# WestlyPark/StyleRenderer

Measured on AMD Instinct MI355X. Metric: generator fwd+bwd images/sec at 256^2, higher is better.
Workload: dtype f32

## Files before the change

### include/stylerenderer_amd.h

```cpp
#ifndef STYLERENDERER_AMD_H_
#define STYLERENDERER_AMD_H_

#include <stddef.h>
#include <stdint.h>

#ifdef __cplusplus
extern "C" {
#endif

typedef void* sr_stream_t;

#define SR_OK 0
#define SR_EINVAL (-1)
#define SR_ERANGE (-2)

const char* sr_error_string(int code);
int sr_abi_version(void);

int sr_fused_bias_act(float* y, const float* x, const float* b, const float* ref, int act, int grad,
                      float alpha, float scale, int64_t size_x, int64_t step_b, int64_t size_b,
                      int use_bias, int use_ref, sr_stream_t stream);

int64_t sr_fused_act_bwd_scratch_floats(int64_t n, int64_t c, int64_t inner);
int sr_fused_act_bwd(float* gx, float* gb, const float* gy, const float* out, float alpha,
                     float scale, int64_t n, int64_t c, int64_t inner, float* partial,
                     sr_stream_t stream);

int sr_noise_bias_act(float* y, const float* x, const float* noise, const float* noise_w,
                      const float* bias, const float* ref, float alpha, float scale, int64_t n,
                      int64_t c, int64_t inner, int64_t noise_bstride, sr_stream_t stream);
int64_t sr_noise_bias_act_bwd_scratch_floats(int64_t n, int64_t c, int64_t inner);
int sr_noise_bias_act_bwd(float* gx, float* gbias, float* gnoise_w, const float* gy, const float* out,
                          const float* noise, float alpha, float scale, int64_t n, int64_t c,
                          int64_t inner, int64_t noise_bstride, float* scratch, sr_stream_t stream);
int64_t sr_noise_bias_act_bwd_dot_scratch_floats(int64_t n, int64_t c, int64_t inner);
int sr_noise_bias_act_bwd_dot(float* gx, float* gbias, float* gnoise_w, float* rowdot, const float* gy,
                              const float* out, const float* noise, const float* noise_w, const float* bias,
                              float alpha, float scale, int64_t n, int64_t c, int64_t inner,
                              int64_t noise_bstride, float* scratch, sr_stream_t stream);
int sr_noise_bias_act_affine(float* y, const float* x, const float* amap, const float* smap, int64_t map_bstride,
                             const float* noise, const float* noise_w, const float* bias, float alpha,
                             float scale, int64_t n, int64_t c, int64_t inner, int64_t noise_bstride,
                             sr_stream_t stream);
int64_t sr_noise_bias_act_affine_bwd_scratch_floats(int64_t n, int64_t c, int64_t inner);
int sr_noise_bias_act_affine_bwd(float* gx, float* gamap, float* gsmap, float* gbias, float* gnoise_w,
                                 const float* gy, const float* out, const float* x, const float* amap,
                                 int64_t map_bstride, const float* noise, float alpha, float scale, int64_t n,
                                 int64_t c, int64_t inner, int64_t noise_bstride, float* scratch,
                                 sr_stream_t stream);
int64_t sr_noise_bias_act_affine_bwd2_scratch_floats(int64_t n, int64_t c, int64_t inner);
int sr_noise_bias_act_affine_bwd2(float* d_gy, float* d_x, float* d_amap, int64_t d_amap_bstride, const float* Gx,
                                  const float* Gmap, int64_t gmap_bstride, const float* Gb, const float* Gnw,
                                  const float* gy, const float* out, const float* x, const float* amap,
                                  int64_t map_bstride, const float* noise, float alpha, float scale, int64_t n,
                                  int64_t c, int64_t inner, int64_t noise_bstride, float* scratch, sr_stream_t stream);

int sr_adam_flat(float* p, const float* g, float* m, float* v, int64_t n, float lr, float beta1, float beta2,
                 float eps, const float* step, sr_stream_t stream);
int sr_adam_flat_guarded(float* p, const float* g, float* m, float* v, int64_t n, float lr, float beta1, float beta2,
                         float eps, float* step, const int64_t* guard_offs, int n_guards,
                         int32_t* skipped_host, sr_stream_t stream);

int64_t sr_rowdot_scratch_floats(int64_t rows, int64_t inner);
int sr_rowdot(float* dots, float* out_scaled, const float* a, const float* b, const float* scale,
              int64_t rows, int64_t inner, float* scratch, sr_stream_t stream);
int sr_rowdot_div(float* dots, const float* a, const float* b, const float* rdiv, int64_t rows, int64_t inner,
                  float* scratch, sr_stream_t stream);
int sr_rowdot_bwd(float* ga, float* gb, float* gs, const float* a, const float* b, const float* gd, const float* go,
                  const float* scale, int64_t rows, int64_t inner, float* scratch, sr_stream_t stream);

int sr_smallconv_fwd(float* out, const float* x, const float* ws, const float* bias, int64_t B, int64_t C,
                     int64_t N, int64_t hw, sr_stream_t stream);
int sr_smallconv_dx(float* dx, const float* g, const float* ws, int64_t B, int64_t C, int64_t N, int64_t hw,
                    sr_stream_t stream);
int sr_smallconv_dx_add(float* dx, const float* g, const float* ws, const float* addend, int64_t B, int64_t C, int64_t N,
                        int64_t hw, sr_stream_t stream);
int64_t sr_smallconv_dw_scratch_floats(int64_t B, int64_t C, int64_t N, int64_t hw);
int sr_smallconv_dw(float* dws, const float* g, const float* x, int64_t B, int64_t C, int64_t N, int64_t hw,
                    float* scratch, sr_stream_t stream);
int sr_smallconv_dw_bias(float* dws, float* gb, const float* g, const float* x, int64_t B, int64_t C, int64_t N, int64_t hw,
                         float* scratch, sr_stream_t stream);
int sr_modrows_fwd(float* ws, const float* w, const float* s, float scale, int64_t B, int64_t N, int64_t C,
                   sr_stream_t stream);
int sr_modrows_bwd(float* gs, float* gw, const float* dws, const float* w, const float* s, float scale, int64_t B,
                   int64_t N, int64_t C, sr_stream_t stream);

int sr_vertex_normals_f32(float* vn, float* norm_out, const float* v, const int64_t* tri, const int32_t* adj_off,
                          const int32_t* adj, int64_t B, int64_t nv, int64_t nf, float eps, sr_stream_t stream);

int sr_affine3_fwd(float* out, const float* v, const float* m, const float* t, int64_t B, int64_t nv,
                   int64_t v_bstride, sr_stream_t stream);
int sr_affine3_bwd(float* gm, float* gt, const float* v, const float* g, int64_t B, int64_t nv, int64_t v_bstride,
                   sr_stream_t stream);

int sr_morph_fwd(float* v, float* vs, float* reg, const float* w, const float* bias, const float* coeff, const float* lin,
                 const float* pose, const float* sigma, float lam, int64_t B, int64_t nv, int64_t d, sr_stream_t stream);
int sr_vertex_normals_bwd_f32(float* gvs, const float* gv, const float* gn, const float* lin, const float* rot,
                              const float* v, const float* ns, const float* normc, const int64_t* tri,
                              const int32_t* adj_off, const int32_t* adj, int64_t B, int64_t nv, int64_t nf, float eps,
                              sr_stream_t stream);
int64_t sr_morph_gcoeff_scratch_floats(int64_t rows, int64_t B, int64_t d);
int sr_morph_gcoeff(float* gcoeff, float* scratch, const float* w, const float* gvs, const float* coeff,
                    const float* sigma, float lam, const float* greg, int64_t B, int64_t rows, int64_t d,
                    sr_stream_t stream);
int sr_morph_pose_bwd(float* gpose, const float* glin, const float* grot, const float* gt, const float* pose, int64_t B,
                      sr_stream_t stream);

int sr_skin_joints_fwd(float* cx, float* G, float* chain, float* reg, const float* coeff, const float* pose,
                       const float* j0, const float* js, const int32_t* parent, const float* sigma, const float* pose_inv,
                       float lam, int64_t B, int64_t nj, int64_t nroot, int64_t ds, sr_stream_t stream);
int sr_skin_fwd(float* v, float* vp, const float* st, const float* vt, const float* cx, const float* wts, const float* G,
                int64_t B, int64_t nv, int64_t D, int64_t nj, sr_stream_t stream);
int64_t sr_skin_bwd_scratch_floats(int64_t nv, int64_t B, int64_t nj);
int sr_skin_bwd(float* gvp, float* part, const float* gv, const float* gvn, const float* vp, const float* wts,
                const float* G, int64_t B, int64_t nv, int64_t nj, sr_stream_t stream);
int sr_skin_joints_bwd(float* gcoeff, float* gpose, const float* gcx, const float* part, const float* coeff,
                       const float* pose, const float* chain, const float* js, const int32_t* parent, const float* sigma,
                       const float* pose_inv, float lam, const float* greg, int64_t B, int64_t nblk, int64_t nj,
                       int64_t nroot, int64_t ds, sr_stream_t stream);

int64_t sr_blend_z_floats(int64_t B, int64_t ds, int64_t de);
int sr_blend_head(float* xs, float* xe, float* prior, float* z, const float* x, const float* beta, float lam, int64_t B,
                  int64_t ds, int64_t de, sr_stream_t stream);
int sr_blend_fwd(float* v, float* vs, float* reg, const float* w, const float* z, const float* prior, const float* lin,
                 const float* pose, int64_t B, int64_t nv, int64_t ds, int64_t de, sr_stream_t stream);
int sr_blend_gz(float* gz, const float* w, const float* gvs, int64_t B, int64_t nv, int64_t ds, int64_t de,
                sr_stream_t stream);
int sr_blend_tail(float* gcoeff, const float* gz, const float* xs, const float* xe, const float* beta, float lam,
                  const float* greg, int64_t B, int64_t ds, int64_t de, sr_stream_t stream);

int sr_pose_fwd(float* lin, float* rot, const float* pose, sr_stream_t stream);
int sr_pose_bwd(float* gpose, const float* glin, const float* grot, const float* pose, sr_stream_t stream);
int sr_pose_batch_fwd(float* lin, float* rot, const float* pose, int64_t B, sr_stream_t stream);

int sr_linear_fwd(float* y, const float* x, const float* w, const float* bias, int64_t B, int64_t K, int64_t N,
                  int64_t ldx, float wscale, float bscale, int act, float alpha, float gain, sr_stream_t stream);
int sr_linear_bwd_x(float* gx, const float* gy, const float* y, const float* w, int64_t B, int64_t K, int64_t N,
                    float wscale, int act, float alpha, float gain, sr_stream_t stream);
int sr_linear_bwd_w(float* gw, float* gbias, const float* gy, const float* y, const float* x, int64_t B,
                    int64_t K, int64_t N, int64_t ldx, float wscale, float bscale, int act, float alpha,
                    float gain, sr_stream_t stream);
int sr_demod_fwd(float* d, const float* s, const float* wsq, int64_t B, int64_t Ci, int64_t Co, float eps,
                 sr_stream_t stream);
int sr_demod_bwd(float* gs, float* gwsq, const float* gd, const float* gs_add, const float* s, const float* d,
                 const float* wsq, int64_t B, int64_t Ci, int64_t Co, sr_stream_t stream);

int sr_weight_prep(float* wt, float* wsq, const float* w, float scale, int64_t Co, int64_t Ci, int ksize,
                   int64_t ld, sr_stream_t stream);
int sr_weight_prep_bwd(float* gw, const float* gwt, const float* gwsq, const float* w, float scale,
                       int64_t Co, int64_t Ci, int ksize, int64_t ldg, sr_stream_t stream);
int sr_weight_adjoint(float* out, const float* in, int64_t taps, int64_t C, int64_t N, int64_t ldn,
                      int64_t ldc, int flip, sr_stream_t stream);

int sr_weight_prep_batch(int n, float* const* wt, float* const* wsq, const float* const* w, const float* scale,
                         const int64_t* Co, const int64_t* Ci, const int* ksize, const int64_t* ld, sr_stream_t stream);
int sr_weight_adjoint_batch(int n, float* const* out, const float* const* in, const int64_t* taps, const int64_t* C,
                            const int64_t* N, const int64_t* ldn, const int64_t* ldc, const int* flip,
                            sr_stream_t stream);

#define SR_BANK_MAX 48
int sr_bank_nt(int n, float* const* out, const float* const* A, const float* const* M, const float* const* bias,
               const int64_t* lda, const int64_t* ldo, const int64_t* K, const int64_t* N, int64_t B, float alpha,
               float bscale, sr_stream_t stream);
int sr_bank_nn(int n_out, float* const* out, const int64_t* ldo, const int64_t* J, const int* n_terms,
               const float* const* A, const float* const* M, const int64_t* lda, const int64_t* I, int64_t B,
               float alpha, sr_stream_t stream);
int sr_bank_tn(int n, float* const* out, float* const* col, const float* const* A, const float* const* C,
               const int64_t* lda, const int64_t* ldc, const int64_t* I, const int64_t* J, int64_t B, float alpha,
               float bscale, sr_stream_t stream);

int sr_upfirdn2d(float* out, const float* x, const float* k, int64_t major, int in_h, int in_w,
                 int out_h, int out_w, int kh, int kw, int up_x, int up_y, int down_x, int down_y,
                 int pad_x0, int pad_x1, int pad_y0, int pad_y1, sr_stream_t stream);

int sr_upsample2_add(float* out, const float* x, const float* k, const float* addend, int64_t major, int in_h,
                     int in_w, int out_h, int out_w, int pad0, int pad1, sr_stream_t stream);

int sr_blur_noise_bias_act(float* y, const float* x, const float* k, const float* noise, const float* noise_w,
                           const float* bias, float alpha, float gain, int64_t n, int64_t c, int in_h, int in_w,
                           int out_h, int out_w, int pad0, int pad1, int64_t noise_bstride, sr_stream_t stream);

int64_t sr_blur_nba_bwd_scratch_floats(int64_t n, int64_t c, int out_h, int out_w);
int sr_blur_nba_bwd(float* gx, float* gbias, float* gnoise_w, float* rowdot, const float* gy, const float* y,
                    const float* k_flipped, const float* noise, const float* noise_w, const float* bias, float alpha,
                    float gain, int64_t n, int64_t c, int in_h, int in_w, int out_h, int out_w, int pad0,
                    int64_t noise_bstride, float* scratch, sr_stream_t stream);


#define SR_RASTER_CHW 2
#define SR_RASTER_GRAD_ACC 4
int64_t sr_rasterize_scratch_bytes(int64_t b, int64_t nf, int64_t h, int64_t w, int is_double);
int sr_rasterize_forward_f32(int64_t b, int64_t nv, int64_t nf, int64_t h, int64_t w, int repeat_v,
                             int repeat_f, int perspective, const float* v, const int64_t* tri,
                             int64_t* index, float* coeff, float* zbuf, float eps,
                             const float* tex, int64_t tex_c, float* attr, int32_t* win, int32_t* big,
                             void* work, sr_stream_t stream);
int sr_rasterize_forward_f64(int64_t b, int64_t nv, int64_t nf, int64_t h, int64_t w, int repeat_v,
                             int repeat_f, int perspective, const double* v, const int64_t* tri,
                             int64_t* index, double* coeff, double* zbuf, double eps,
                             const double* tex, int64_t tex_c, double* attr, int32_t* win, int32_t* big,
                             void* work, sr_stream_t stream);

#define SR_RASTER_MAX_LEVELS 12
int sr_rasterize_levels_supported(int n, int64_t b, int64_t nf, const int64_t* h, const int64_t* w);
int sr_rasterize_forward_levels_f32(int n, int64_t b, int64_t nv, int64_t nf, const int64_t* h, const int64_t* w,
                                    int repeat_v, int repeat_f, int perspective, const float* v, const int64_t* tri,
                                    float eps, const float* tex, int64_t tex_c, float* const* attr, int32_t* const* win,
                                    int32_t* const* big, void* const* work, sr_stream_t stream);

int sr_rasterize_grad_levels_f32(int n, int64_t b, int64_t nv, int64_t nf, const int64_t* h, const int64_t* w, int repeat_f,
                                 int perspective, const float* v, const float* tex, int64_t tex_c, const int64_t* tri,
                                 const int32_t* const* win, int32_t* const* big, const float* const* grad_out,
                                 const int32_t* adj_off, const int32_t* adj, int64_t off_bstride, int64_t adj_bstride,
                                 const int32_t* adj_slot, float* grad_v, float* grad_tex, float eps, void* const* work,
                                 sr_stream_t stream);

int sr_rasterize_backward_f32(int64_t b, int64_t n, int64_t h, int64_t w, int repeat_v,
                              int perspective, const float* v, const int64_t* index, float* dcoeff,
                              float eps, sr_stream_t stream);
int sr_rasterize_backward_f64(int64_t b, int64_t n, int64_t h, int64_t w, int repeat_v,
                              int perspective, const double* v, const int64_t* index,
                              double* dcoeff, double eps, sr_stream_t stream);

int64_t sr_rasterize_grad_scratch_bytes(int64_t b, int64_t nf, int64_t tex_c, int is_double);
int sr_rasterize_grad_f32(int64_t b, int64_t nv, int64_t nf, int64_t h, int64_t w, int repeat_f,
                          int perspective, const float* v, const float* tex, int64_t tex_c,
                          const int64_t* tri, const int32_t* win, const int32_t* big, const float* grad_out,
                          const int32_t* adj_off, const int32_t* adj, int64_t adj_off_bstride,
                          int64_t adj_bstride, const int32_t* adj_slot, float* grad_v, float* grad_tex, float eps,
                          void* work, sr_stream_t stream);
int sr_rasterize_grad_f64(int64_t b, int64_t nv, int64_t nf, int64_t h, int64_t w, int repeat_f,
                          int perspective, const double* v, const double* tex, int64_t tex_c,
                          const int64_t* tri, const int32_t* win, const int32_t* big, const double* grad_out,
                          const int32_t* adj_off, const int32_t* adj, int64_t adj_off_bstride,
                          int64_t adj_bstride, const int32_t* adj_slot, double* grad_v, double* grad_tex, double eps,
                          void* work, sr_stream_t stream);

int sr_rasterize_forward_cpu_f32(int64_t b, int64_t nv, int64_t nf, int64_t h, int64_t w, int repeat_v,
                                 int repeat_f, int perspective, const float* v, const int64_t* tri,
                                 int64_t* index, float* coeff, float* zbuf, float eps);
int sr_rasterize_forward_cpu_f64(int64_t b, int64_t nv, int64_t nf, int64_t h, int64_t w, int repeat_v,
                                 int repeat_f, int perspective, const double* v, const int64_t* tri,
                                 int64_t* index, double* coeff, double* zbuf, double eps);
int sr_rasterize_backward_cpu_f32(int64_t b, int64_t n, int64_t h, int64_t w, int perspective,
                                  const float* v, const int64_t* index, float* dcoeff, float eps);
int sr_rasterize_backward_cpu_f64(int64_t b, int64_t n, int64_t h, int64_t w, int perspective,
                                  const double* v, const int64_t* index, double* dcoeff, double eps);

int64_t sr_conv2d_scratch_floats(int64_t B, int64_t C, int64_t N, int64_t IH, int64_t IW, int64_t OH,
                                 int64_t OW, int ksize, int stride, int pad, int transposed);
int sr_conv2d_mfma(float* out, const float* in, const float* wt, const float* iscale,
                   const float* oscale, const float* obias, int64_t B, int64_t C, int64_t N,
                   int64_t wt_ld, int64_t IH, int64_t IW, int64_t OH, int64_t OW, int ksize, int stride,
                   int pad, int transposed, float* scratch, sr_stream_t stream);
int sr_conv2d_nba(float* out, const float* in, const float* wt, const float* iscale, const float* oscale,
                  const float* noise, const float* noise_w, const float* abias, float alpha, float gain, int64_t B,
                  int64_t C, int64_t N, int64_t wt_ld, int64_t H, int64_t W, int64_t noise_bstride, float* scratch,
                  sr_stream_t stream);

#define SR_CONV_U_READY 1
int sr_conv2d_uses_winograd(int64_t B, int64_t C, int64_t N, int64_t IH, int64_t IW, const float* in, const float* out);

int sr_conv2d_generic(float* y, const float* x, const float* w, const float* bias, int64_t B, int64_t C, int64_t N,
                      int64_t IH, int64_t IW, int64_t OH, int64_t OW, int kh, int kw, int sy, int sx, int py, int px,
                      sr_stream_t stream);
int sr_conv2d_generic_dgrad(float* dx, const float* g, const float* w, int64_t B, int64_t C, int64_t N, int64_t IH,
                            int64_t IW, int64_t OH, int64_t OW, int kh, int kw, int sy, int sx, int py, int px,
                            sr_stream_t stream);
int sr_conv2d_generic_wgrad(float* dw, const float* x, const float* g, int64_t B, int64_t C, int64_t N, int64_t IH,
                            int64_t IW, int64_t OH, int64_t OW, int kh, int kw, int sy, int sx, int py, int px,
                            sr_stream_t stream);
int sr_conv2d_mfma_ex(float* out, const float* in, const float* wt, const float* iscale,
                      const float* oscale, const float* obias, int64_t B, int64_t C, int64_t N,
                      int64_t wt_ld, int64_t IH, int64_t IW, int64_t OH, int64_t OW, int ksize,
                      int stride, int pad, int transposed, int flags, float* scratch, sr_stream_t stream);
int sr_conv1x1_add_supported(int64_t B, int64_t C, int64_t N, int64_t wt_ld, int64_t P, const float* in, const float* wt,
                             const float* out, const float* addend);
int sr_conv1x1_add(float* out, const float* in, const float* wt, const float* oscale, const float* addend, int64_t B,
                   int64_t C, int64_t N, int64_t wt_ld, int64_t P, sr_stream_t stream);
int sr_conv2d_nba_ex(float* out, const float* in, const float* wt, const float* iscale, const float* oscale,
                     const float* noise, const float* noise_w, const float* abias, float alpha, float gain,
                     int64_t B, int64_t C, int64_t N, int64_t wt_ld, int64_t H, int64_t W, int64_t noise_bstride,
                     int flags, float* scratch, sr_stream_t stream);

int64_t sr_conv2d_wgrad_scratch_floats(int64_t B, int64_t C, int64_t N, int64_t IH, int64_t IW,
                                       int64_t OH, int64_t OW, int ksize, int stride, int pad,
                                       int transposed);
int sr_conv2d_wgrad_mfma(float* dwt, const float* x, const float* gy, const float* xscale,
                         const float* gscale, int64_t B, int64_t C, int64_t N, int64_t IH,
                         int64_t IW, int64_t OH, int64_t OW, int ksize, int stride, int pad,
                         int transposed, float* scratch, sr_stream_t stream);

int sr_signal_bump(uint32_t* counter, sr_stream_t stream);
int sr_signal_set(uint32_t* word, const uint32_t* epoch, sr_stream_t stream);
int sr_signal_wait(const uint32_t* counter, uint32_t at_least, sr_stream_t stream);
int sr_signal_wait_timeout(const uint32_t* counter, uint32_t at_least, uint64_t timeout_us, int32_t* status_host,
                           int32_t code, sr_stream_t stream);
int sr_signal_wait_poison(const uint32_t* counter, uint32_t at_least, uint64_t timeout_us, int32_t* status_host,
                          int32_t code, float* poison, sr_stream_t stream);
int sr_signal_set_host(uint32_t* word_host, const uint32_t* epoch, sr_stream_t stream);

int sr_graph_replace_memset_nodes(void* hip_graph, int* replaced);
int sr_graph_node_count(void* graph, int* kernel_nodes, int* all_nodes);

int64_t sr_lpips_layer_scratch_floats(int64_t b, int64_t hw);
int sr_lpips_layer_fwd(float* d, const float* f0, const float* t, const float* lin, int64_t b, int64_t c, int64_t hw,
                       int64_t t_bstride, float eps, float* scratch, sr_stream_t stream);
int sr_lpips_layer_bwd(float* gf, const float* gd, const float* f0, const float* t, const float* lin, int64_t b,
                       int64_t c, int64_t hw, int64_t t_bstride, float eps, sr_stream_t stream);
int sr_ppl_endpoints(float* out, const float* a, const float* b, int64_t in_stride, const float* t, int64_t npairs,
                     int64_t d, int mode, int n_ends, float eps, sr_stream_t stream);
int sr_ppl_prep(float* out, const float* img, const float* shift, const float* scale, int64_t n, int64_t h, int64_t w,
                int64_t y0, int64_t x0, int64_t ch, int64_t cw, int64_t oh, int64_t ow, sr_stream_t stream);
int64_t sr_lpips_pair_scratch_floats(int64_t npairs, int64_t n_layers, const int64_t* hw);
int sr_lpips_pair(float* d, const float* const* f, const float* const* lin, const int64_t* c, const int64_t* hw,
                  int64_t n_layers, int64_t npairs, float div, float* scratch, sr_stream_t stream);
int sr_incep_conv(const float* in, const float* wt, const float* bias, int64_t B, int64_t C, int64_t H, int64_t W,
                  int64_t M, int kh, int kw, int stride, int ph, int pw, int nseg, float* const* seg_out,
                  const int64_t* seg_m0, const int64_t* seg_coff, const int64_t* seg_ctot, sr_stream_t stream);
int sr_incep_pool(float* out, const float* in, int64_t B, int64_t C, int64_t H, int64_t W, int mode, int64_t coff,
                  int64_t ctot, sr_stream_t stream);
int sr_incep_gap(float* out, const float* in, int64_t planes, int64_t hw, sr_stream_t stream);
int sr_fstats_update(double* sum, double* gram, double* shift, const float* f, int64_t n, int64_t d, int first,
                     sr_stream_t stream);
int sr_fstats_finalize(double* mean, double* cov, const double* sum, const double* gram, const double* shift,
                       int64_t count, int64_t d, sr_stream_t stream);
int sr_mse_fwd(float* out, const float* a, const float* b, int64_t n, sr_stream_t stream);
int sr_mse_bwd(float* ga, const float* gout, const float* a, const float* b, int64_t n, sr_stream_t stream);
int64_t sr_mse_rows_scratch_floats(int64_t B, int64_t n);
int sr_mse_rows_fwd(float* out, const float* a, const float* t, int64_t B, int64_t n, float* scratch,
                    sr_stream_t stream);
int sr_mse_rows_bwd(float* ga, const float* gout, const float* a, const float* t, int64_t B, int64_t n,
                    sr_stream_t stream);
int sr_fit_loss_rows(float* rows, float* total, const float* d0, const float* d1, const float* d2, const float* d3,
                     const float* d4, const float* mse, float pixel_weight, const float* coeff, const float* sigma,
                     float shape_reg, int64_t B, int64_t d, sr_stream_t stream);
int sr_fit_loss_rows_bwd(float* gd, float* gmse, const float* gtotal, float pixel_weight, int64_t B, sr_stream_t stream);
int sr_maxpool2_fwd(float* out, const float* x, int64_t planes, int64_t ih, int64_t iw, sr_stream_t stream);
int sr_maxpool2_bwd(float* gx, const float* gy, const float* x, int64_t planes, int64_t ih, int64_t iw, sr_stream_t stream);

#define SR_ADA_NDRAW 11
#define SR_ADA_REC 28
int sr_ada_params(float* rec, const float* draws, int64_t B, const float* pose_p, const float* color_p, const double* p_dev,
                  double p_host, int64_t H, int64_t W, sr_stream_t stream);
int sr_ada_apply(float* out, const float* img, const float* rec, int64_t B, int64_t H, int64_t W, int with_bias,
                 sr_stream_t stream);
int sr_ada_apply_grad(float* gin, const float* gout, const float* rec, int64_t B, int64_t H, int64_t W, sr_stream_t stream);
int sr_ada_update(double* state, const float* stat, double target, double length, sr_stream_t stream);

int64_t sr_resample_u8_scratch_bytes(int64_t N, int64_t H, int64_t W, int64_t C, int64_t oh, int64_t ow,
                                     const int32_t* bounds_v_host, int64_t oy0, int64_t ox0, int64_t ohw, int64_t oww);
int sr_resample_u8(void* out, const uint8_t* in, int64_t N, int64_t H, int64_t W, int64_t C, int64_t oh, int64_t ow,
                   const int32_t* coeffs_h_t, const int32_t* bounds_h, const int32_t* bounds_h_host, int64_t ksize_h,
                   const int32_t* coeffs_v, const int32_t* bounds_v, const int32_t* bounds_v_host, int64_t ksize_v,
                   int64_t oy0, int64_t ox0, int64_t ohw, int64_t oww, int out_form, int mul24, uint8_t* scratch,
                   sr_stream_t stream);

int sr_warp_affine_u8(void* out, const uint8_t* in, const double* matrix, int64_t matrix_stride, int64_t N, int64_t H,
                      int64_t W, int64_t C, int64_t oh, int64_t ow, int border, int fill, int out_form,
                      sr_stream_t stream);

#ifdef __cplusplus
}
#endif
#endif
```

### stylerenderer_amd/_lib.py

```python
import ctypes
import os

_HERE = os.path.dirname(os.path.abspath(__file__))
LIB_PATH = os.environ.get("STYLERENDERER_AMD_LIB") or os.path.join(_HERE, "libstylerenderer_hip.so")

_i = ctypes.c_int
_l = ctypes.c_int64
_f = ctypes.c_float
_d = ctypes.c_double
_p = ctypes.c_void_p

SIGNATURES = {
    "sr_error_string": (ctypes.c_char_p, [_i]),
    "sr_abi_version": (_i, []),
    "sr_fused_bias_act": (_i, [_p, _p, _p, _p, _i, _i, _f, _f, _l, _l, _l, _i, _i, _p]),
    "sr_fused_act_bwd_scratch_floats": (_l, [_l, _l, _l]),
    "sr_fused_act_bwd": (_i, [_p, _p, _p, _p, _f, _f, _l, _l, _l, _p, _p]),
    "sr_noise_bias_act": (_i, [_p] * 6 + [_f, _f] + [_l] * 4 + [_p]),
    "sr_noise_bias_act_bwd_scratch_floats": (_l, [_l, _l, _l]),
    "sr_noise_bias_act_bwd": (_i, [_p] * 6 + [_f, _f] + [_l] * 4 + [_p, _p]),
    "sr_noise_bias_act_bwd_dot_scratch_floats": (_l, [_l, _l, _l]),
    "sr_noise_bias_act_bwd_dot": (_i, [_p] * 9 + [_f, _f] + [_l] * 4 + [_p, _p]),
    "sr_conv2d_nba": (_i, [_p] * 8 + [_f, _f] + [_l] * 7 + [_p, _p]),
    "sr_conv2d_nba_ex": (_i, [_p] * 8 + [_f, _f] + [_l] * 7 + [_i, _p, _p]),
    "sr_noise_bias_act_affine": (_i, [_p] * 4 + [_l] + [_p] * 3 + [_f, _f] + [_l] * 4 + [_p]),
    "sr_noise_bias_act_affine_bwd_scratch_floats": (_l, [_l, _l, _l]),
    "sr_noise_bias_act_affine_bwd": (_i, [_p] * 9 + [_l, _p, _f, _f] + [_l] * 4 + [_p, _p]),
    "sr_noise_bias_act_affine_bwd2_scratch_floats": (_l, [_l, _l, _l]),
    "sr_noise_bias_act_affine_bwd2": (_i, [_p, _p, _p, _l, _p, _p, _l] + [_p] * 6 + [_l, _p, _f, _f] + [_l] * 4 + [_p, _p]),
    "sr_adam_flat": (_i, [_p] * 4 + [_l] + [_f] * 4 + [_p, _p]),
    "sr_adam_flat_guarded": (_i, [_p] * 4 + [_l] + [_f] * 4 + [_p, ctypes.POINTER(_l), _i, _p, _p]),
    "sr_rowdot_scratch_floats": (_l, [_l, _l]),
    "sr_rowdot": (_i, [_p] * 5 + [_l, _l, _p, _p]),
    "sr_rowdot_div": (_i, [_p] * 4 + [_l, _l, _p, _p]),
    "sr_rowdot_bwd": (_i, [_p] * 8 + [_l, _l, _p, _p]),
    "sr_smallconv_fwd": (_i, [_p] * 4 + [_l] * 4 + [_p]),
    "sr_smallconv_dx": (_i, [_p] * 3 + [_l] * 4 + [_p]),
    "sr_smallconv_dx_add": (_i, [_p] * 4 + [_l] * 4 + [_p]),
    "sr_smallconv_dw_scratch_floats": (_l, [_l] * 4),
    "sr_smallconv_dw": (_i, [_p] * 3 + [_l] * 4 + [_p, _p]),
    "sr_smallconv_dw_bias": (_i, [_p] * 4 + [_l] * 4 + [_p, _p]),
    "sr_modrows_fwd": (_i, [_p] * 3 + [_f] + [_l] * 3 + [_p]),
    "sr_modrows_bwd": (_i, [_p] * 5 + [_f] + [_l] * 3 + [_p]),
    "sr_vertex_normals_f32": (_i, [_p] * 6 + [_l] * 3 + [_f, _p]),
    "sr_linear_fwd": (_i, [_p] * 4 + [_l] * 4 + [_f, _f, _i, _f, _f, _p]),
    "sr_linear_bwd_x": (_i, [_p] * 4 + [_l] * 3 + [_f, _i, _f, _f, _p]),
    "sr_linear_bwd_w": (_i, [_p] * 5 + [_l] * 4 + [_f, _f, _i, _f, _f, _p]),
    "sr_demod_fwd": (_i, [_p] * 3 + [_l] * 3 + [_f, _p]),
    "sr_demod_bwd": (_i, [_p] * 7 + [_l] * 3 + [_p]),
    "sr_weight_prep": (_i, [_p, _p, _p, _f, _l, _l, _i, _l, _p]),
    "sr_weight_prep_bwd": (_i, [_p, _p, _p, _p, _f, _l, _l, _i, _l, _p]),
    "sr_weight_adjoint": (_i, [_p, _p, _l, _l, _l, _l, _l, _i, _p]),
    "sr_bank_nt": (_i, [_i] + [_p] * 8 + [_l, _f, _f, _p]),
    "sr_bank_nn": (_i, [_i] + [_p] * 8 + [_l, _f, _p]),
    "sr_bank_tn": (_i, [_i] + [_p] * 8 + [_l, _f, _f, _p]),
    "sr_weight_prep_batch": (_i, [_i] + [_p] * 9),
    "sr_weight_adjoint_batch": (_i, [_i] + [_p] * 9),
    "sr_lpips_layer_scratch_floats": (_l, [_l, _l]),
    "sr_lpips_layer_fwd": (_i, [_p] * 4 + [_l] * 4 + [_f, _p, _p]),
    "sr_lpips_layer_bwd": (_i, [_p] * 5 + [_l] * 4 + [_f, _p]),
    "sr_ppl_endpoints": (_i, [_p, _p, _p, _l, _p, _l, _l, _i, _i, _f, _p]),
    "sr_ppl_prep": (_i, [_p] * 4 + [_l] * 9 + [_p]),
    "sr_lpips_pair_scratch_floats": (_l, [_l, _l, _p]),
    "sr_lpips_pair": (_i, [_p] * 5 + [_l, _l, _f, _p, _p]),
    "sr_incep_conv": (_i, [_p] * 3 + [_l] * 5 + [_i] * 6 + [_p] * 5),
    "sr_incep_pool": (_i, [_p] * 2 + [_l] * 4 + [_i, _l, _l, _p]),
    "sr_incep_gap": (_i, [_p] * 2 + [_l] * 2 + [_p]),
    "sr_fstats_update": (_i, [_p] * 4 + [_l, _l, _i, _p]),
    "sr_fstats_finalize": (_i, [_p] * 5 + [_l, _l, _p]),
    "sr_mse_fwd": (_i, [_p] * 3 + [_l, _p]),
    "sr_mse_bwd": (_i, [_p] * 4 + [_l, _p]),
    "sr_mse_rows_scratch_floats": (_l, [_l, _l]),
    "sr_mse_rows_fwd": (_i, [_p] * 3 + [_l, _l, _p, _p]),
    "sr_mse_rows_bwd": (_i, [_p] * 4 + [_l, _l, _p]),
    "sr_fit_loss_rows": (_i, [_p] * 8 + [_f, _p, _p, _f, _l, _l, _p]),
    "sr_fit_loss_rows_bwd": (_i, [_p] * 3 + [_f, _l, _p]),
    "sr_maxpool2_fwd": (_i, [_p] * 2 + [_l] * 3 + [_p]),
    "sr_maxpool2_bwd": (_i, [_p] * 3 + [_l] * 3 + [_p]),
    "sr_ada_params": (_i, [_p, _p, _l, _p, _p, _p, _d, _l, _l, _p]),
    "sr_ada_apply": (_i, [_p] * 3 + [_l] * 3 + [_i, _p]),
    "sr_ada_apply_grad": (_i, [_p] * 3 + [_l] * 3 + [_p]),
    "sr_ada_update": (_i, [_p, _p, _d, _d, _p]),
    "sr_upfirdn2d": (_i, [_p, _p, _p, _l] + [_i] * 14 + [_p]),
    "sr_upsample2_add": (_i, [_p] * 4 + [_l] + [_i] * 6 + [_p]),
    "sr_blur_noise_bias_act": (_i, [_p] * 6 + [_f, _f, _l, _l] + [_i] * 6 + [_l, _p]),
    "sr_conv2d_generic": (_i, [_p] * 4 + [_l] * 7 + [_i] * 6 + [_p]),
    "sr_conv2d_generic_dgrad": (_i, [_p] * 3 + [_l] * 7 + [_i] * 6 + [_p]),
    "sr_conv2d_generic_wgrad": (_i, [_p] * 3 + [_l] * 7 + [_i] * 6 + [_p]),
    "sr_blur_nba_bwd_scratch_floats": (_l, [_l, _l, _i, _i]),
    "sr_blur_nba_bwd": (_i, [_p] * 10 + [_f, _f, _l, _l] + [_i] * 5 + [_l, _p, _p]),
    "sr_rasterize_scratch_bytes": (_l, [_l, _l, _l, _l, _i]),
    "sr_rasterize_forward_f32": (_i, [_l] * 5 + [_i] * 3 + [_p] * 5 + [_f, _p, _l, _p, _p, _p, _p, _p]),
    "sr_rasterize_levels_supported": (_i, [_i, _l, _l, _p, _p]),
    "sr_rasterize_forward_levels_f32": (_i, [_i, _l, _l, _l, _p, _p, _i, _i, _i, _p, _p, _f, _p, _l, _p, _p, _p, _p, _p]),
    "sr_rasterize_grad_levels_f32": (_i, [_i, _l, _l, _l, _p, _p, _i, _i, _p, _p, _l] + [_p] * 6 + [_l, _l] + [_p] * 3 + [_f, _p, _p]),
    "sr_rasterize_forward_f64": (_i, [_l] * 5 + [_i] * 3 + [_p] * 5 + [_d, _p, _l, _p, _p, _p, _p, _p]),
    "sr_rasterize_grad_scratch_bytes": (_l, [_l, _l, _l, _i]),
    "sr_rasterize_forward_cpu_f32": (_i, [_l] * 5 + [_i] * 3 + [_p] * 5 + [_f]),
    "sr_rasterize_forward_cpu_f64": (_i, [_l] * 5 + [_i] * 3 + [_p] * 5 + [_d]),
    "sr_rasterize_backward_cpu_f32": (_i, [_l] * 4 + [_i] + [_p] * 3 + [_f]),
    "sr_rasterize_backward_cpu_f64": (_i, [_l] * 4 + [_i] + [_p] * 3 + [_d]),
    "sr_rasterize_backward_f32": (_i, [_l] * 4 + [_i] * 2 + [_p] * 3 + [_f, _p]),
    "sr_rasterize_backward_f64": (_i, [_l] * 4 + [_i] * 2 + [_p] * 3 + [_d, _p]),
    "sr_rasterize_grad_f32": (_i, [_l] * 5 + [_i] * 2 + [_p, _p, _l] + [_p] * 6 + [_l, _l, _p, _p, _p, _f, _p, _p]),
    "sr_conv2d_wgrad_scratch_floats": (_l, [_l] * 7 + [_i] * 4),
    "sr_conv2d_wgrad_mfma": (_i, [_p] * 5 + [_l] * 7 + [_i] * 4 + [_p, _p]),
    "sr_conv2d_scratch_floats": (_l, [_l] * 7 + [_i] * 4),
    "sr_conv2d_mfma": (_i, [_p] * 6 + [_l] * 8 + [_i] * 4 + [_p, _p]),
    "sr_conv2d_uses_winograd": (_i, [_l] * 5 + [_p, _p]),
    "sr_conv2d_mfma_ex": (_i, [_p] * 6 + [_l] * 8 + [_i] * 5 + [_p, _p]),
    "sr_conv1x1_add_supported": (_i, [_l] * 5 + [_p] * 4),
    "sr_conv1x1_add": (_i, [_p] * 5 + [_l] * 5 + [_p]),
    "sr_rasterize_grad_f64": (_i, [_l] * 5 + [_i] * 2 + [_p, _p, _l] + [_p] * 6 + [_l, _l, _p, _p, _p, _d, _p, _p]),
    "sr_pose_fwd": (_i, [_p, _p, _p, _p]),
    "sr_pose_bwd": (_i, [_p, _p, _p, _p, _p]),
    "sr_pose_batch_fwd": (_i, [_p, _p, _p, _l, _p]),
    "sr_affine3_fwd": (_i, [_p, _p, _p, _p, _l, _l, _l, _p]),
    "sr_affine3_bwd": (_i, [_p, _p, _p, _p, _l, _l, _l, _p]),
    "sr_morph_fwd": (_i, [_p] * 9 + [_f, _l, _l, _l, _p]),
    "sr_vertex_normals_bwd_f32": (_i, [_p] * 11 + [_l, _l, _l, _f, _p]),
    "sr_morph_gcoeff_scratch_floats": (_l, [_l, _l, _l]),
    "sr_morph_gcoeff": (_i, [_p] * 6 + [_f, _p, _l, _l, _l, _p]),
    "sr_morph_pose_bwd": (_i, [_p] * 5 + [_l, _p]),
    "sr_skin_joints_fwd": (_i, [_p] * 11 + [_f] + [_l] * 4 + [_p]),
    "sr_skin_fwd": (_i, [_p] * 7 + [_l] * 4 + [_p]),
    "sr_skin_bwd_scratch_floats": (_l, [_l, _l, _l]),
    "sr_skin_bwd": (_i, [_p] * 7 + [_l] * 3 + [_p]),
    "sr_skin_joints_bwd": (_i, [_p] * 11 + [_f, _p] + [_l] * 5 + [_p]),
    "sr_blend_z_floats": (_l, [_l, _l, _l]),
    "sr_blend_head": (_i, [_p] * 6 + [_f] + [_l] * 3 + [_p]),
    "sr_blend_fwd": (_i, [_p] * 8 + [_l] * 4 + [_p]),
    "sr_blend_gz": (_i, [_p] * 3 + [_l] * 4 + [_p]),
    "sr_blend_tail": (_i, [_p] * 5 + [_f, _p] + [_l] * 3 + [_p]),
    "sr_resample_u8_scratch_bytes": (_l, [_l] * 6 + [ctypes.POINTER(ctypes.c_int32)] + [_l] * 4),
    "sr_resample_u8": (_i, [_p, _p] + [_l] * 6 + [_p, _p, ctypes.POINTER(ctypes.c_int32), _l] * 2 + [_l] * 4
                       + [_i, _i, _p, _p]),
    "sr_warp_affine_u8": (_i, [_p, _p, _p] + [_l] * 7 + [_i, _i, _i, _p]),
    "sr_signal_bump": (_i, [_p, _p]),
    "sr_signal_wait": (_i, [_p, ctypes.c_uint32, _p]),
    "sr_signal_set": (_i, [_p, _p, _p]),
    "sr_signal_set_host": (_i, [_p, _p, _p]),
    "sr_signal_wait_timeout": (_i, [_p, ctypes.c_uint32, ctypes.c_uint64, _p, _i, _p]),
    "sr_signal_wait_poison": (_i, [_p, ctypes.c_uint32, ctypes.c_uint64, _p, _i, _p, _p]),
    "sr_graph_replace_memset_nodes": (_i, [_p, ctypes.POINTER(_i)]),
    "sr_graph_node_count": (_i, [_p, ctypes.POINTER(_i), ctypes.POINTER(_i)]),
}

_lib = None


class NativeLibraryError(RuntimeError):
    pass


def lib():
    global _lib
    if _lib is not None:
        return _lib
    if not os.path.isfile(LIB_PATH):
        raise NativeLibraryError(
            "stylerenderer_amd: %s not found. Build it with `python -c 'import __graft_entry__ as g; "
            "g.build()'` (hipcc --offload-arch=gfx950). There is no CPU/PyTorch fallback for device "
            "tensors." % LIB_PATH)
    try:
        handle = ctypes.CDLL(LIB_PATH)
    except OSError as e:
        raise NativeLibraryError("stylerenderer_amd: cannot load %s: %s" % (LIB_PATH, e))
    for name, (res, args) in SIGNATURES.items():
        try:
            fn = getattr(handle, name)
        except AttributeError:
            raise NativeLibraryError("stylerenderer_amd: %s does not export %s" % (LIB_PATH, name))
        fn.restype = res
        fn.argtypes = args
    _lib = handle
    return _lib


def check(rc, what=""):
    if rc != 0:
        msg = lib().sr_error_string(rc)
        raise RuntimeError("%s failed: %s (code %d)" % (what or "stylerenderer_amd call",
                                                        msg.decode() if msg else "?", rc))


def ptr(t):
    if t is None or t.numel() == 0:
        return None
    return t.data_ptr()


def current_stream(device=None):
    import torch

    return torch.cuda.current_stream(device).cuda_stream
```

### stylerenderer_amd/csrc/conv_mfma.hip

```cpp
#include "common.h"
#include "conv1x1_gemm.h"
#include "conv_s2_bf16x3.h"
#include "conv_wgrad_bf16x3.h"
#include "conv_wino.h"

#include <cstdlib>

namespace {

typedef float f32x16 __attribute__((ext_vector_type(16)));
typedef const void __attribute__((address_space(1)))* gptr_t;
typedef void __attribute__((address_space(3)))* lptr_t;

constexpr int BN = 128;
constexpr int BM = 128;

__device__ __attribute__((aligned(16))) const float g_zero_line[4] = {0.f, 0.f, 0.f, 0.f};
__device__ __attribute__((aligned(16))) const float g_ones_line[4] = {1.f, 1.f, 1.f, 1.f};

struct ConvParams {
    const float* in;
    const float* wt;
    const float* iscale;
    const float* oscale;
    const float* obias;
    float* out;
    int B, C, N, ldw;
    int IH, IW;
    int GH, GW;
    int gy_base, gx_base;
    int OH, OW;
    int osy, osx, ooy, oox;
    int dy0, dx0;
    int wmap[9];
    int tiles_x, tiles_y, tiles_b, tiles_n;
    float* partial;
    int64_t partial_floats;
    int ks, c_per_slice;
    int tap_first, tap_step, tap_count;
};

template <int IS, int TY, int TX, int PW, int PH, int PB, bool V4, bool TAP9 = false>
struct Geo {
    static constexpr bool ROT = V4 && IS == 2;
    static constexpr int NT = TY * TX;
    static constexpr int KC = NT >= 9 ? 4 : (NT >= 4 ? 8 : 16);
    static constexpr int EH = (PH - 1) * IS + TY;
    static constexpr int EW = (PW - 1) * IS + TX;
    static constexpr int LEAD = (V4 && !ROT) ? (TAP9 ? 4 : (TX > 1 ? 3 : 0)) : 0;
    static constexpr int EWP = ROT ? (EW + 3 + 3) / 4 * 4
                                   : (V4 ? (LEAD + EW + 3) / 4 * 4 : EW + ((EW % 2 == 0) ? 1 : 0));
    static constexpr int PLANE = PB * EH * EWP;
    static constexpr int W_FLOATS = NT * KC * BN;
    static constexpr int W_INSTR = W_FLOATS / 256;
    static constexpr int IMG_INSTR = V4 ? (KC * PLANE + 255) / 256 : 0;
    static constexpr int ST_INSTR = V4 ? (KC * PB + 63) / 64 : 0;
    static constexpr int IN_FLOATS = KC * PLANE + KC * PB;
    static constexpr int IN_INSTR = V4 ? IMG_INSTR + ST_INSTR : (IN_FLOATS + 63) / 64;
    static constexpr int S_BASE = V4 ? W_FLOATS + IMG_INSTR * 256 : W_FLOATS + KC * PLANE;
    static constexpr int BUF = V4 ? S_BASE + ST_INSTR * 64 : W_FLOATS + IN_INSTR * 64;
    static constexpr int W_PER_WAVE = (W_INSTR + 3) / 4;
    static constexpr int IN_PER_WAVE = (IN_INSTR + 3) / 4;
    static constexpr int LDS_BYTES = 2 * BUF * 4;
};

template <int IS, int TY, int TX, int PW, int PH, int PB, bool V4, bool FAST, bool TAP9 = false>
__global__ __launch_bounds__(256) void k_conv_mfma(const ConvParams p) {
    using G = Geo<IS, TY, TX, PW, PH, PB, V4, TAP9>;
    static_assert(PW * PH * PB == BM, "patch must hold 128 pixels");
    static_assert(!TAP9 || (IS == 1 && TY == 1 && TX == 1), "tap-split mode is a shifted 1x1 convolution");
    extern __shared__ __attribute__((aligned(16))) float smem[];

    const int nwg = gridDim.x;
    int bid = blockIdx.x;
    {
        const int q = nwg / SR_NUM_XCD, r = nwg % SR_NUM_XCD, xcd = bid % SR_NUM_XCD;
        bid = (xcd < r ? xcd * (q + 1) : r * (q + 1) + (xcd - r) * q) + bid / SR_NUM_XCD;
    }
    int tap = 0, g_dy0 = p.dy0, g_dx0 = p.dx0, g_gh = p.GH, g_gw = p.GW, g_ooy = p.ooy, g_oox = p.oox, g_slab = p.wmap[0];
    int tap_local = 0;
    if (TAP9) {
        tap_local = bid % p.tap_count;
        bid /= p.tap_count;
        tap = p.tap_first + tap_local * p.tap_step;
        const int ky = tap / 3, kx = tap - 3 * ky;
        g_dy0 = -(ky >> 1); g_dx0 = -(kx >> 1);
        g_ooy = ky & 1; g_oox = kx & 1;
        g_gh = min(g_ooy ? p.IH : p.IH + 1, p.GH); g_gw = min(g_oox ? p.IW : p.IW + 1, p.GW);
        g_slab = tap;
    }
    const int n_t = bid % p.tiles_n;
    bid /= p.tiles_n;
    const int tx_i = bid % p.tiles_x;
    bid /= p.tiles_x;
    const int ty_i = bid % p.tiles_y;
    bid /= p.tiles_y;
    const int tb_i = bid % p.tiles_b;
    const int slice = bid / p.tiles_b;
    const int c_beg = slice * p.c_per_slice;
    const int c_end = min(p.C, c_beg + p.c_per_slice);
    const int n0 = n_t * BN, gy0 = p.gy_base + ty_i * PH, gx0 = p.gx_base + tx_i * PW, b0 = tb_i * PB;
    const int iy0 = gy0 * IS + g_dy0, ix0 = gx0 * IS + g_dx0;

    const int tid = threadIdx.x, lane = tid & 63;
    const int wave = __builtin_amdgcn_readfirstlane(tid >> 6);
    const int half = lane >> 5, l31 = lane & 31;
    const int wco = wave & 1, wpx = wave >> 1;

    int a_off[2], b_off[2], s_off[2];
    int b_rot[2][4];
#pragma unroll
    for (int t = 0; t < 2; ++t) {
        a_off[t] = half * BN + wco * 64 + t * 32 + l31;
        const int m = wpx * 64 + t * 32 + l31;
        const int px = m % PW, py = (m / PW) % PH, pb = m / (PW * PH);
        b_off[t] = G::W_FLOATS + half * G::PLANE + (pb * G::EH + py * IS) * G::EWP + px * IS + G::LEAD +
                   ((TAP9 && V4) ? g_dx0 : 0);
        s_off[t] = G::S_BASE + pb * G::KC + half;
        const int l0 = half + iy0 + py * IS + ix0;
#pragma unroll
        for (int k = 0; k < 4; ++k) b_rot[t][k] = b_off[t] + ((l0 + k) & 3);
    }

    int w_src[G::W_PER_WAVE];
    int w_cl[G::W_PER_WAVE];
#pragma unroll
    for (int i = 0; i < G::W_PER_WAVE; ++i) {
        const int j = wave + 4 * i;
        const int row = 2 * j + half;
        const int t = row / G::KC, c = row % G::KC;
        const int col = min(n0 + l31 * 4, p.ldw - 4);
        w_cl[i] = (j < G::W_INSTR) ? c : -1;
        int slab = 0;
#pragma unroll
        for (int k = 0; k < G::NT; ++k)
            if (t == k) slab = p.wmap[k];
        if (TAP9) slab = g_slab;
        w_src[i] = (slab * p.C + c) * p.ldw + col;
    }
    int i_src[G::IN_PER_WAVE];
    int i_cl[G::IN_PER_WAVE];
#pragma unroll
    for (int i = 0; i < G::IN_PER_WAVE; ++i) {
        const int j = wave + 4 * i;
        int src = -1, c = 0, pb = 0;
        if (V4) {
            const int f = (j * 64 + lane) * 4;
            if (j < G::IMG_INSTR && f < G::KC * G::PLANE) {
                c = f / G::PLANE;
                const int q = f % G::PLANE;
                const int cola = q % G::EWP, r = (q / G::EWP) % G::EH;
                pb = q / (G::EWP * G::EH);
                const int gy = iy0 + r;
                int gx = ((TAP9 && V4) ? gx0 : ix0) - G::LEAD + cola;
                bool ok = gy >= 0 && gy < p.IH && b0 + pb < p.B;
                if (G::ROT) {
                    gx = ix0 - ((c * (p.IH * p.IW) + gy * p.IW + ix0) & 3) + cola;
                } else {
                    ok = ok && gx >= 0 && gx + 3 < p.IW;
                }
                if (ok) src = (pb * p.C + c) * p.IH * p.IW + gy * p.IW + gx;
            } else if (j >= G::IMG_INSTR && j < G::IN_INSTR) {
                const int e = (j - G::IMG_INSTR) * 64 + lane;
                if (e < G::KC * PB) {
                    pb = e / G::KC;
                    c = e % G::KC;
                    src = -2;
                }
            }
        } else {
            const int f = j * 64 + lane;
            if (j < G::IN_INSTR && f < G::KC * G::PLANE) {
                c = f / G::PLANE;
                const int q = f % G::PLANE;
                const int colp = q % G::EWP, r = (q / G::EWP) % G::EH;
                pb = q / (G::EWP * G::EH);
                const int gy = iy0 + r, gx = ix0 + colp;
                if (colp < G::EW && gy >= 0 && gy < p.IH && gx >= 0 && gx < p.IW && b0 + pb < p.B)
                    src = (pb * p.C + c) * p.IH * p.IW + gy * p.IW + gx;
            } else if (j < G::IN_INSTR && f < G::IN_FLOATS) {
                const int e = f - G::KC * G::PLANE;
                pb = e / G::KC;
                c = e % G::KC;
                src = -2;
            }
        }
        i_src[i] = src;
        i_cl[i] = c | (pb << 8);
    }
    const float* in_base = p.in + (int64_t)b0 * p.C * p.IH * p.IW;
    const int plane_in = p.IH * p.IW;

    const char* f_wp[G::W_PER_WAVE];
    const char* f_ip[G::IN_PER_WAVE];
    unsigned f_is[G::IN_PER_WAVE];
    if (FAST) {
#pragma unroll
        for (int i = 0; i < G::W_PER_WAVE; ++i) f_wp[i] = reinterpret_cast<const char*>(p.wt + w_src[i]);
#pragma unroll
        for (int i = 0; i < G::IN_PER_WAVE; ++i) {
            const int c = i_cl[i] & 255, pb = i_cl[i] >> 8;
            const char* ptr = reinterpret_cast<const char*>(g_zero_line);
            unsigned str = 0;
            if (i_src[i] >= 0) {
                ptr = reinterpret_cast<const char*>(in_base + i_src[i]);
                str = (unsigned)plane_in * 4u;
            } else if (i_src[i] == -2) {
                const bool ok = p.iscale && b0 + pb < p.B;
                ptr = ok ? reinterpret_cast<const char*>(p.iscale + (int64_t)(b0 + pb) * p.C + c)
                         : reinterpret_cast<const char*>(g_ones_line);
                str = ok ? 4u : 0u;
            }
            f_ip[i] = ptr;
            f_is[i] = str;
        }
    }
    const unsigned w_chunk_stride = (unsigned)p.ldw * 4u;

    auto dma = [&](int c0, int buf) {
        float* dst = smem + buf * G::BUF;
        if (FAST) {
#pragma unroll
            for (int i = 0; i < G::W_PER_WAVE; ++i) {
                const int j = wave + 4 * i;
                if (j < G::W_INSTR)
                    __builtin_amdgcn_global_load_lds((gptr_t)(f_wp[i] + (uint64_t)(unsigned)c0 * w_chunk_stride),
                                                     (lptr_t)(dst + j * 256), 16, 0, 0);
            }
#pragma unroll
            for (int i = 0; i < G::IN_PER_WAVE; ++i) {
                const int j = wave + 4 * i;
                if (j < G::IN_INSTR) {
                    const char* src = f_ip[i] + (uint64_t)(unsigned)c0 * f_is[i];
                    if (V4 && j < G::IMG_INSTR)
                        __builtin_amdgcn_global_load_lds((gptr_t)src, (lptr_t)(dst + G::W_FLOATS + j * 256), 16, 0, 0);
                    else if (V4)
                        __builtin_amdgcn_global_load_lds((gptr_t)src,
                                                         (lptr_t)(dst + G::S_BASE + (j - G::IMG_INSTR) * 64), 4, 0, 0);
                    else
                        __builtin_amdgcn_global_load_lds((gptr_t)src, (lptr_t)(dst + G::W_FLOATS + j * 64), 4, 0, 0);
                }
            }
            return;
        }
#pragma unroll
        for (int i = 0; i < G::W_PER_WAVE; ++i) {
            const int j = wave + 4 * i;
            if (j < G::W_INSTR) {
                const float* src = (c0 + w_cl[i] < p.C) ? p.wt + w_src[i] + (int64_t)c0 * p.ldw : g_zero_line;
                __builtin_amdgcn_global_load_lds((gptr_t)src, (lptr_t)(dst + j * 256), 16, 0, 0);
            }
        }
#pragma unroll
        for (int i = 0; i < G::IN_PER_WAVE; ++i) {
            const int j = wave + 4 * i;
            if (j < G::IN_INSTR) {
                const int c = i_cl[i] & 255, pb = i_cl[i] >> 8;
                const bool c_ok = c0 + c < p.C;
                const float* src = g_zero_line;
                if (i_src[i] >= 0 && c_ok) src = in_base + i_src[i] + (int64_t)c0 * plane_in;
                if (i_src[i] == -2)
                    src = (p.iscale && c_ok && b0 + pb < p.B) ? p.iscale + (int64_t)(b0 + pb) * p.C + c0 + c
                                                              : g_ones_line;
                if (V4 && j < G::IMG_INSTR)
                    __builtin_amdgcn_global_load_lds((gptr_t)src, (lptr_t)(dst + G::W_FLOATS + j * 256), 16, 0, 0);
                else if (V4)
                    __builtin_amdgcn_global_load_lds((gptr_t)src,
                                                     (lptr_t)(dst + G::S_BASE + (j - G::IMG_INSTR) * 64), 4, 0, 0);
                else
                    __builtin_amdgcn_global_load_lds((gptr_t)src, (lptr_t)(dst + G::W_FLOATS + j * 64), 4, 0, 0);
            }
        }
    };

    f32x16 acc[2][2];
#pragma unroll
    for (int i = 0; i < 2; ++i)
#pragma unroll
        for (int j = 0; j < 2; ++j)
#pragma unroll
            for (int r = 0; r < 16; ++r) acc[i][j][r] = 0.0f;

    dma(c_beg, 0);
    int buf = 0;
    for (int c0 = c_beg; c0 < c_end; c0 += G::KC) {
        __syncthreads();
        if (c0 + G::KC < c_end) dma(c0 + G::KC, buf ^ 1);
        const float* sb = smem + buf * G::BUF;
#pragma unroll
        for (int cp = 0; cp < G::KC / 2; ++cp) {
            const float sc0 = sb[s_off[0] + 2 * cp];
            const float sc1 = (PB > 1) ? sb[s_off[1] + 2 * cp] : sc0;
#pragma unroll
            for (int ty = 0; ty < TY; ++ty)
#pragma unroll
                for (int tx = 0; tx < TX; ++tx) {
                    const int w_tap = ((ty * TX + tx) * G::KC + 2 * cp) * BN;
                    const int i_tap = (2 * cp) * G::PLANE + ty * G::EWP + tx;
                    float a0 = sb[w_tap + a_off[0]];
                    float a1 = sb[w_tap + a_off[1]];
                    float x0 = sb[i_tap + (G::ROT ? b_rot[0][(2 * cp + ty) & 3] : b_off[0])];
                    float x1 = sb[i_tap + (G::ROT ? b_rot[1][(2 * cp + ty) & 3] : b_off[1])];
                    if (PB == 1) { a0 *= sc0; a1 *= sc0; }
                    else { x0 *= sc0; x1 *= sc1; }
                    acc[0][0] = __builtin_amdgcn_mfma_f32_32x32x2f32(a0, x0, acc[0][0], 0, 0, 0);
                    acc[0][1] = __builtin_amdgcn_mfma_f32_32x32x2f32(a0, x1, acc[0][1], 0, 0, 0);
                    acc[1][0] = __builtin_amdgcn_mfma_f32_32x32x2f32(a1, x0, acc[1][0], 0, 0, 0);
                    acc[1][1] = __builtin_amdgcn_mfma_f32_32x32x2f32(a1, x1, acc[1][1], 0, 0, 0);
                }
        }
        buf ^= 1;
    }

    const int64_t plane_out = (int64_t)p.OH * p.OW;
#pragma unroll
    for (int pt = 0; pt < 2; ++pt) {
        const int m = wpx * 64 + pt * 32 + l31;
        const int px = m % PW, py = (m / PW) % PH, pb = m / (PW * PH);
        const int gy = gy0 + py, gx = gx0 + px, b = b0 + pb;
        if (gy >= g_gh || gx >= g_gw || b >= p.B) continue;
        const int64_t pix = (int64_t)(gy * p.osy + g_ooy) * p.OW + (gx * p.osx + g_oox);
#pragma unroll
        for (int ct = 0; ct < 2; ++ct)
#pragma unroll
            for (int r = 0; r < 16; ++r) {
                const int n = n0 + wco * 64 + ct * 32 + (r & 3) + 8 * (r >> 2) + 4 * half;
                if (n < p.N) {
                    float v = acc[ct][pt][r];
                    if (TAP9) {
                        const int rw = p.GW - p.gx_base, rh = p.GH - p.gy_base;
                        p.partial[((((int64_t)slice * p.tap_count + tap_local) * p.B + b) * p.N + n) * (rh * rw) +
                                  (gy - p.gy_base) * rw + (gx - p.gx_base)] = v;
                    } else if (p.ks > 1) {
                        const int rw = p.GW - p.gx_base, rh = p.GH - p.gy_base;
                        p.partial[(((int64_t)slice * p.B + b) * p.N + n) * (rh * rw) +
                                  (gy - p.gy_base) * rw + (gx - p.gx_base)] = v;
                    } else {
                        if (p.oscale) v *= p.oscale[(int64_t)b * p.N + n];
                        if (p.obias) v += p.obias[n];
                        p.out[((int64_t)b * p.N + n) * plane_out + pix] = v;
                    }
                }
            }
    }
}

template <int IS, int TY, int TX, int PW, int PH, int PB, bool V4, bool FAST, bool TAP9 = false>
int launch_fast(const ConvParams& p, dim3 grid, hipStream_t st) {
    using G = Geo<IS, TY, TX, PW, PH, PB, V4, TAP9>;
    auto kern = k_conv_mfma<IS, TY, TX, PW, PH, PB, V4, FAST, TAP9>;
    static bool configured = false;
    if (!configured) {
        (void)hipFuncSetAttribute(reinterpret_cast<const void*>(kern),
                                  hipFuncAttributeMaxDynamicSharedMemorySize, G::LDS_BYTES);
        configured = true;
    }
    hipLaunchKernelGGL(kern, grid, dim3(256), G::LDS_BYTES, st, p);
    return sr_launch_status();
}

template <int IS, int TY, int TX, int PW, int PH, int PB, bool V4, bool TAP9 = false>
int launch_one(const ConvParams& p, dim3 grid, hipStream_t st) {
    using G = Geo<IS, TY, TX, PW, PH, PB, V4, TAP9>;
    if (p.C % G::KC == 0 && p.c_per_slice % G::KC == 0)
        return launch_fast<IS, TY, TX, PW, PH, PB, V4, true, TAP9>(p, grid, st);
    return launch_fast<IS, TY, TX, PW, PH, PB, V4, false, TAP9>(p, grid, st);
}

struct TFused {
    static constexpr int KC = 8;
    static constexpr int PW = 32, PH = 4;
    static constexpr int LEAD = 3;
    static constexpr int EWP = 36;
    static constexpr int EH = PH + 1;
    static constexpr int PLANE = EH * EWP;
    static constexpr int W_FLOATS = 9 * KC * BN;
    static constexpr int W_INSTR = W_FLOATS / 256;
    static constexpr int I_INSTR = (KC * PLANE / 4 + 63) / 64;
    static constexpr int I_FLOATS = I_INSTR * 256;
    static constexpr int BUF = W_FLOATS + I_FLOATS;
    static constexpr int W_PER_WAVE = 9, I_PER_WAVE = 2;
    static constexpr int PAD = 2 * BUF;
    static constexpr int STY = PAD + 4 * 256;
};

#ifdef CONVT_TIMING
__device__ long long g_convt_stamps[8 * 16384];
#define CONVT_STAMP(i) do { if (threadIdx.x == 0) { g_convt_stamps[(blockIdx.x & 16383) * 8 + (i)] = wall_clock64(); } } while (0)
#else
#define CONVT_STAMP(i)
#endif

template <bool KS>
__global__ __launch_bounds__(256) void k_convt_fused(const ConvParams p) {
#if __HIP_DEVICE_COMPILE__
    using G = TFused;
    CONVT_STAMP(0);
#ifdef CONVT_TIMING
    const long long convt_c0 = clock64();
#endif
    extern __shared__ __attribute__((aligned(16))) float smem[];
    float* const sty = smem + G::STY;

    const int nwg = gridDim.x;
    int bid = blockIdx.x;
    {
        const int q = nwg / SR_NUM_XCD, r = nwg % SR_NUM_XCD, xcd = bid % SR_NUM_XCD;
        bid = (xcd < r ? xcd * (q + 1) : r * (q + 1) + (xcd - r) * q) + bid / SR_NUM_XCD;
    }
    const int n_t = bid % p.tiles_n;
    bid /= p.tiles_n;
    const int tx_i = bid % p.tiles_x;
    bid /= p.tiles_x;
    const int ty_i = bid % p.tiles_y;
    bid /= p.tiles_y;
    const int b = KS ? bid % p.B : bid;
    const int slice = KS ? bid / p.B : 0;
    const int c_beg = KS ? slice * p.c_per_slice : 0;
    const int c_cnt = KS ? p.c_per_slice : p.C;
    const int n0 = n_t * BN, j0 = ty_i * G::PH, i0 = tx_i * G::PW;

    const int tid = threadIdx.x, lane = tid & 63;
    const int wave = __builtin_amdgcn_readfirstlane(tid >> 6);
    const int half = lane >> 5, l31 = lane & 31;
    const int wco = wave & 1, wpx = wave >> 1;

    constexpr int OOB = 0x7FFFFFF0;
    int w_off[G::W_PER_WAVE];
#pragma unroll
    for (int i = 0; i < G::W_PER_WAVE; ++i) {
        const int j = wave + 4 * i;
        const int row = 2 * j + half;
        const int t = row / G::KC, c = row % G::KC;
        const int col = min(n0 + l31 * 4, p.ldw - 4);
        w_off[i] = j < G::W_INSTR ? ((t * p.C + c) * p.ldw + col) * 4 : OOB;
    }
    int i_off[G::I_PER_WAVE];
#pragma unroll
    for (int i = 0; i < G::I_PER_WAVE; ++i) {
        const int j = wave + 4 * i;
        const int f = (j * 64 + lane) * 4;
        int off = OOB;
        if (j < G::I_INSTR && f < G::KC * G::PLANE) {
            const int c = f / G::PLANE, q = f % G::PLANE;
            const int r = q / G::EWP, cola = q % G::EWP;
            const int gy = j0 - 1 + r, gx = i0 - 4 + cola;
            if (gy >= 0 && gy < p.IH && gx >= 0 && gx + 3 < p.IW) off = ((c * p.IH + gy) * p.IW + gx) * 4;
        }
        i_off[i] = off;
    }
    const int plane_in = p.IH * p.IW;
    const __amdgpu_buffer_rsrc_t r_w = uniform_rsrc(p.wt + (int64_t)c_beg * p.ldw, (9 * p.C - c_beg) * p.ldw * 4);
    const __amdgpu_buffer_rsrc_t r_in = uniform_rsrc(p.in + ((int64_t)b * p.C + c_beg) * plane_in, c_cnt * plane_in * 4);
    const int nchunks = c_cnt / G::KC;

    auto dma1 = [&](int k, int i) {
        const int kc = min(k, nchunks - 1), c0 = kc * G::KC;
        float* dst = smem + (k & 1) * G::BUF;
        if (i < G::I_PER_WAVE) {
            const int j = wave + 4 * i;
            __builtin_amdgcn_raw_ptr_buffer_load_lds(
                r_in, (lptr_t)(j < G::I_INSTR ? dst + G::W_FLOATS + j * 256 : smem + G::PAD + wave * 256), 16, i_off[i],
                c0 * plane_in * 4, 0, 0);
        } else {
            const int ii = i - G::I_PER_WAVE, j = wave + 4 * ii;
            __builtin_amdgcn_raw_ptr_buffer_load_lds(r_w, (lptr_t)(j < G::W_INSTR ? dst + j * 256 : smem + G::PAD + wave * 256),
                                                     16, w_off[ii], c0 * p.ldw * 4, 0, 0);
        }
    };
    constexpr int N_DMA = G::W_PER_WAVE + G::I_PER_WAVE;

    f32x16 acc[4][2][2];
#pragma unroll
    for (int ph = 0; ph < 4; ++ph)
#pragma unroll
        for (int i = 0; i < 2; ++i)
#pragma unroll
            for (int j = 0; j < 2; ++j)
#pragma unroll
                for (int r = 0; r < 16; ++r) acc[ph][i][j][r] = 0.0f;

    int a_off[2], b_off[2];
#pragma unroll
    for (int t = 0; t < 2; ++t) {
        a_off[t] = half * BN + wco * 64 + t * 32 + l31;
        const int py = wpx * 2 + t;
        b_off[t] = G::W_FLOATS + half * G::PLANE + (py + 1) * G::EWP + l31 + G::LEAD + 1;
    }

#pragma unroll
    for (int i = 0; i < N_DMA; ++i) dma1(0, i);
#pragma unroll
    for (int i = 0; i < 4; ++i) dma1(1, i);
    for (int c = tid; c < c_cnt; c += 256) sty[c] = p.iscale ? p.iscale[(int64_t)b * p.C + c_beg + c] : 1.0f;
    __builtin_amdgcn_s_waitcnt(0x0F70);
    __syncthreads();

    float A[2][9][2], X[2][4][2];
    float sc_next;
    auto load_set = [&](const float* sb, int c0, int cp, int set) {
#pragma unroll
        for (int sh = 0; sh < 4; ++sh)
#pragma unroll
            for (int t = 0; t < 2; ++t)
                X[set][sh][t] = sb[(2 * cp) * G::PLANE + b_off[t] - (sh >> 1) * G::EWP - (sh & 1)];
#pragma unroll
        for (int tap = 0; tap < 9; ++tap)
#pragma unroll
            for (int t = 0; t < 2; ++t) A[set][tap][t] = sb[(tap * G::KC + 2 * cp) * BN + a_off[t]];
        sc_next = sty[c0 + 2 * cp + half];
    };
    load_set(smem, 0, 0, 0);
#pragma unroll
    for (int sh = 0; sh < 4; ++sh) { X[0][sh][0] *= sc_next; X[0][sh][1] *= sc_next; }
    CONVT_STAMP(1);

    for (int k = 0; k < nchunks; ++k) {
        const float* sb = smem + (k & 1) * G::BUF;
        const float* sbn = smem + ((k + 1) & 1) * G::BUF;
        const int c0 = k * G::KC, c0n = min(k + 1, nchunks - 1) * G::KC;
#pragma unroll
        for (int cp = 0; cp < G::KC / 2; ++cp) {
            const int cur = cp & 1, nxt = cur ^ 1;
            if (cp == G::KC / 2 - 1) {
                __builtin_amdgcn_s_waitcnt(0x0F70);
                __syncthreads();
                load_set(sbn, c0n, 0, nxt);
            } else {
                load_set(sb, c0, cp + 1, nxt);
            }
            __builtin_amdgcn_sched_barrier(0);
#pragma unroll
            for (int ky = 0; ky < 3; ++ky)
#pragma unroll
                for (int kx = 0; kx < 3; ++kx) {
                    const int tap = ky * 3 + kx, ph = (ky & 1) * 2 + (kx & 1), sh = (ky >> 1) * 2 + (kx >> 1);
                    acc[ph][0][0] = __builtin_amdgcn_mfma_f32_32x32x2f32(A[cur][tap][0], X[cur][sh][0], acc[ph][0][0], 0, 0, 0);
                    acc[ph][0][1] = __builtin_amdgcn_mfma_f32_32x32x2f32(A[cur][tap][0], X[cur][sh][1], acc[ph][0][1], 0, 0, 0);
                    acc[ph][1][0] = __builtin_amdgcn_mfma_f32_32x32x2f32(A[cur][tap][1], X[cur][sh][0], acc[ph][1][0], 0, 0, 0);
                    acc[ph][1][1] = __builtin_amdgcn_mfma_f32_32x32x2f32(A[cur][tap][1], X[cur][sh][1], acc[ph][1][1], 0, 0, 0);
                    if (tap >= 1) X[nxt][(tap - 1) >> 1][(tap - 1) & 1] *= sc_next;
                    if ((tap & 1) == 1) {
                        const int u = tap >> 1;
                        if (cp == 0) dma1(k + 1, 4 + u);
                        else if (cp == 1 && 8 + u < N_DMA) dma1(k + 1, 8 + u);
                        else if (cp == G::KC / 2 - 1) dma1(k + 2, u);
                    }
                    __builtin_amdgcn_sched_barrier(0);
                }
        }
    }
    __builtin_amdgcn_s_waitcnt(0x0F70);
    CONVT_STAMP(2);

    const int64_t plane_out = (int64_t)p.OH * p.OW;
#pragma unroll
    for (int pt = 0; pt < 2; ++pt) {
        const int j = j0 + wpx * 2 + pt, i = i0 + l31;
#pragma unroll
        for (int ct = 0; ct < 2; ++ct)
#pragma unroll
            for (int r = 0; r < 16; ++r) {
                const int n = n0 + wco * 64 + ct * 32 + (r & 3) + 8 * (r >> 2) + 4 * half;
                if (n < p.N) {
                    const float os = (!KS && p.oscale) ? p.oscale[(int64_t)b * p.N + n] : 1.0f;
                    const float ob = (!KS && p.obias) ? p.obias[n] : 0.0f;
                    float* o = (KS ? p.partial + (int64_t)slice * p.B * p.N * plane_out : p.out) +
                               ((int64_t)b * p.N + n) * plane_out + (int64_t)(2 * j) * p.OW + 2 * i;
                    o[0] = acc[0][ct][pt][r] * os + ob;
                    o[1] = acc[1][ct][pt][r] * os + ob;
                    o[p.OW] = acc[2][ct][pt][r] * os + ob;
                    o[p.OW + 1] = acc[3][ct][pt][r] * os + ob;
                }
            }
    }
    CONVT_STAMP(3);
#ifdef CONVT_TIMING
    if (threadIdx.x == 0) g_convt_stamps[(blockIdx.x & 16383) * 8 + 5] = clock64() - convt_c0;
#endif
#endif
}

#ifdef CONVT_TIMING
extern "C" int sr_debug_convt_stamps(long long* host, int n) {
    return (int)hipMemcpyFromSymbol(host, HIP_SYMBOL(g_convt_stamps), (size_t)n * sizeof(long long));
}
#endif

bool convt_fused_eligible(const ConvParams& p) {
    if ((int64_t)p.C * p.IH * p.IW >= (1LL << 29) - 4 || 9LL * p.C * p.ldw >= (1LL << 29) - 4) return false;
    return p.IH % TFused::PH == 0 && p.IW % TFused::PW == 0 && p.C % TFused::KC == 0 && p.C <= 2048 &&
           (reinterpret_cast<uintptr_t>(p.in) & 15) == 0;
}

__global__ __launch_bounds__(256) void k_convt_fused_reduce(const ConvParams p) {
    const int iw2 = 2 * p.IW, ih2 = 2 * p.IH;
    const int64_t plane_out = (int64_t)p.OH * p.OW, planes = (int64_t)p.B * p.N;
    const int64_t total = planes * ih2 * (iw2 / 4);
    for (int64_t i = (int64_t)blockIdx.x * blockDim.x + threadIdx.x; i < total; i += (int64_t)gridDim.x * blockDim.x) {
        const int64_t row = i / ((int64_t)ih2 * (iw2 / 4));
        const int q = (int)(i - row * (int64_t)ih2 * (iw2 / 4));
        const int Y = q / (iw2 / 4), X = (q - Y * (iw2 / 4)) * 4;
        const int64_t at = row * plane_out + (int64_t)Y * p.OW + X;
        float acc[4] = {0.0f, 0.0f, 0.0f, 0.0f};
        for (int s = 0; s < p.ks; ++s) {
            const float* src = p.partial + (int64_t)s * planes * plane_out + at;
#pragma unroll
            for (int k = 0; k < 4; ++k) acc[k] += src[k];
        }
        const float os = p.oscale ? p.oscale[row] : 1.0f, ob = p.obias ? p.obias[row % p.N] : 0.0f;
#pragma unroll
        for (int k = 0; k < 4; ++k) p.out[at + k] = acc[k] * os + ob;
    }
}

int convt_fused_slices(int64_t fused_blocks, int C) {
    for (int ks = 2; ks <= 4; ks *= 2)
        if (C % (ks * TFused::KC) == 0 && C / ks >= 64 && fused_blocks * ks >= 192) return ks;
    return 1;
}

int64_t convt_fused_split_floats(int64_t B, int64_t C, int64_t N, int64_t IH, int64_t IW) {
    const int64_t blocks = (IW / TFused::PW) * (IH / TFused::PH) * ((N + BN - 1) / BN) * B;
    if (IW % TFused::PW || IH % TFused::PH || blocks >= 192 || C <= 256) return 0;
    const int ks = convt_fused_slices(blocks, (int)C);
    return ks > 1 ? ks * B * N * (2 * IH + 1) * (2 * IW + 1) : 0;
}

int launch_convt_fused(ConvParams p, hipStream_t st) {
    p.tiles_x = p.IW / TFused::PW;
    p.tiles_y = p.IH / TFused::PH;
    p.tiles_n = (p.N + BN - 1) / BN;
    const int64_t blocks = (int64_t)p.tiles_x * p.tiles_y * p.tiles_n * p.B * p.ks;
    if (blocks > 0x7FFFFFFFLL) return SR_ERANGE;
    if (p.ks > 1) {
        const int lds = (TFused::STY + p.c_per_slice) * 4;
        hipLaunchKernelGGL(k_convt_fused<true>, dim3((unsigned)blocks), dim3(256), lds, st, p);
        const int64_t total = (int64_t)p.B * p.N * 2 * p.IH * (2 * p.IW / 4);
        hipLaunchKernelGGL(k_convt_fused_reduce, dim3(sr_stream_grid(total, 256)), dim3(256), 0, st, p);
        return sr_launch_status();
    }
    const int lds = (TFused::STY + p.C) * 4;
    hipLaunchKernelGGL(k_convt_fused<false>, dim3((unsigned)blocks), dim3(256), lds, st, p);
    return sr_launch_status();
}

void patch_shape(int GW, int& pw, int& ph, int& pb) {
    if (GW > 16) { pw = 32; ph = 4; pb = 1; }
    else if (GW > 8) { pw = 16; ph = 8; pb = 1; }
    else if (GW > 4) { pw = 8; ph = 8; pb = 2; }
    else { pw = 4; ph = 4; pb = 8; }
}

void choose_split(int GH, int GW, int B, int N, int C, int& ks, int& c_per_slice) {
    int pw, ph, pb;
    patch_shape(GW, pw, ph, pb);
    const int64_t blocks = (int64_t)((GW + pw - 1) / pw) * ((GH + ph - 1) / ph) * ((B + pb - 1) / pb) *
                           ((N + BN - 1) / BN);
    ks = 1;
    c_per_slice = (C + 15) / 16 * 16;
    if (blocks >= SR_NUM_CU || C < 64) return;
    int want = (int)((2 * SR_NUM_CU + blocks - 1) / blocks);
    if (want > 16) want = 16;
    int per = (C + want - 1) / want;
    per = (per + 15) / 16 * 16;
    if (per < 32) per = 32;
    c_per_slice = per;
    ks = (C + per - 1) / per;
}

__global__ __launch_bounds__(256) void k_conv_reduce(const ConvParams p, int rh, int rw) {
    const int64_t region = (int64_t)rh * rw, total = (int64_t)p.B * p.N * region;
    const int64_t plane_out = (int64_t)p.OH * p.OW;
    for (int64_t i = (int64_t)blockIdx.x * blockDim.x + threadIdx.x; i < total;
         i += (int64_t)gridDim.x * blockDim.x) {
        float acc = 0.0f;
#pragma unroll 8
        for (int s = 0; s < p.ks; ++s) acc += p.partial[s * total + i];
        const int64_t row = i / region;
        const int q = (int)(i - row * region);
        const int gy = p.gy_base + q / rw, gx = p.gx_base + q % rw;
        if (p.oscale) acc *= p.oscale[row];
        if (p.obias) acc += p.obias[row % p.N];
        p.out[row * plane_out + (int64_t)(gy * p.osy + p.ooy) * p.OW + (gx * p.osx + p.oox)] = acc;
    }
}

__global__ __launch_bounds__(256) void k_convt_tap_reduce(const ConvParams p) {
    const int rh = p.GH, rw = p.GW;
    const int64_t region = (int64_t)rh * rw, plane_out = (int64_t)p.OH * p.OW;
    const int64_t total = (int64_t)p.B * p.N * plane_out, slab = (int64_t)p.B * p.N * region;
    for (int64_t i = (int64_t)blockIdx.x * blockDim.x + threadIdx.x; i < total;
         i += (int64_t)gridDim.x * blockDim.x) {
        const int64_t row = i / plane_out;
        const int q = (int)(i - row * plane_out);
        const int Y = q / p.OW, X = q - Y * p.OW;
        const int py = Y & 1, px = X & 1;
        const int64_t at = row * region + (int64_t)(Y >> 1) * rw + (X >> 1);
        float acc = 0.0f;
        for (int s = 0; s < p.ks; ++s)
            for (int ky = py; ky < 3; ky += 2)
                for (int kx = px; kx < 3; kx += 2) acc += p.partial[((int64_t)s * 9 + ky * 3 + kx) * slab + at];
        if (p.oscale) acc *= p.oscale[row];
        if (p.obias) acc += p.obias[row % p.N];
        p.out[i] = acc;
    }
}

int convt_taps_mode() {
    const char* e = std::getenv("SR_CONVT_TAPS");
    return !e ? 2 : (e[0] == '0' ? 0 : 1);
}

void convt_taps_plan(int IH, int IW, int B, int N, int C, int& ks, int& c_per_slice) {
    if (sr_convt_taps_gemm_eligible(B, C, N, IW, 4, 16, nullptr)) {
        const int64_t tiles = sr_ceil_div((int64_t)B * (IH + 1) * (IW + 1), 128) * (N / 128) * 9;
        static const int per_cu = [] {
            const char* e = std::getenv("SR_TAPS_WGS");
            const int v = e ? std::atoi(e) : 0;
            return v >= 1 && v <= 8 ? v : 2;
        }();
        int want = (int)sr_ceil_div((int64_t)per_cu * SR_NUM_CU, tiles);
        if (want > 8) want = 8;
        if (want < 1) want = 1;
        int per = (C + want - 1) / want;
        per = (per + 15) / 16 * 16;
        if (per < 64) per = 64;
        if (per > C) per = C;
        c_per_slice = per;
        ks = (C + per - 1) / per;
        return;
    }
    int pw, ph, pb;
    patch_shape(IW + 1, pw, ph, pb);
    const int64_t blocks = (int64_t)((IW + pw) / pw) * ((IH + ph) / ph) * ((B + pb - 1) / pb) * ((N + BN - 1) / BN) * 9;
    ks = 1;
    c_per_slice = (C + 15) / 16 * 16;
    if (blocks >= 2 * SR_NUM_CU || C < 64) return;
    int want = (int)((2 * SR_NUM_CU + blocks - 1) / blocks);
    if (want > 8) want = 8;
    int per = (C + want - 1) / want;
    per = (per + 15) / 16 * 16;
    if (per < 32) per = 32;
    c_per_slice = per;
    ks = (C + per - 1) / per;
}

int64_t convt_taps_floats(int64_t B, int64_t C, int64_t N, int64_t IH, int64_t IW) {
    int ks, per;
    convt_taps_plan((int)IH, (int)IW, (int)B, (int)N, (int)C, ks, per);
    return (int64_t)ks * 9 * B * N * (IH + 1) * (IW + 1);
}

bool convt_taps_wanted(int64_t B, int64_t C, int64_t N, int64_t IH, int64_t IW) {
    const int mode = convt_taps_mode();
    return mode == 1 || (mode == 2 && 18.0 * (double)B * (double)C * (double)N * (double)IH * (double)IW < 1.05e10);
}

bool taps_v4(const ConvParams& p) {
    const char* e = std::getenv("SR_CONVT_TAPS_V4");
    return !(e && e[0] == '0') && p.IW % 4 == 0 && p.gx_base % 4 == 0 && (reinterpret_cast<uintptr_t>(p.in) & 15) == 0;
}

int launch_convt_taps(ConvParams p, hipStream_t st) {
    p.GH = p.IH + 1; p.GW = p.IW + 1;
    p.gy_base = p.gx_base = 0;
    p.osy = p.osx = 2; p.ooy = p.oox = 0;
    p.dy0 = p.dx0 = 0;
    p.tap_first = 0; p.tap_step = 1; p.tap_count = 9;
    convt_taps_plan(p.IH, p.IW, p.B, p.N, p.C, p.ks, p.c_per_slice);
    int pw, ph, pb;
    patch_shape(p.GW, pw, ph, pb);
    p.tiles_x = (p.GW + pw - 1) / pw;
    p.tiles_y = (p.GH + ph - 1) / ph;
    p.tiles_b = (p.B + pb - 1) / pb;
    p.tiles_n = (p.N + BN - 1) / BN;
    const int64_t blocks = (int64_t)p.tiles_x * p.tiles_y * p.tiles_b * p.tiles_n * p.ks * 9;
    if (blocks > 0x7FFFFFFFLL) return SR_ERANGE;
    const dim3 grid((unsigned)blocks);
    const bool v4 = taps_v4(p);
    int rc;
    if (sr_convt_taps_gemm_eligible(p.B, p.C, p.N, p.IW, p.ldw, p.c_per_slice, p.wt))
        rc = sr_convt_taps_gemm_launch(p.partial, p.in, p.wt, p.ldw, p.iscale, p.B, p.C, p.N, p.IH, p.IW, p.ks, p.c_per_slice, st);
    else if (pw == 32) rc = v4 ? launch_one<1, 1, 1, 32, 4, 1, true, true>(p, grid, st)
                          : launch_one<1, 1, 1, 32, 4, 1, false, true>(p, grid, st);
    else if (pw == 16) rc = v4 ? launch_one<1, 1, 1, 16, 8, 1, true, true>(p, grid, st)
                               : launch_one<1, 1, 1, 16, 8, 1, false, true>(p, grid, st);
    else if (pw == 8) rc = launch_one<1, 1, 1, 8, 8, 2, false, true>(p, grid, st);
    else rc = launch_one<1, 1, 1, 4, 4, 8, false, true>(p, grid, st);
    if (rc != SR_OK) return rc;
    const int64_t total = (int64_t)p.B * p.N * p.OH * p.OW;
    hipLaunchKernelGGL(k_convt_tap_reduce, dim3(sr_stream_grid(total, 256)), dim3(256), 0, st, p);
    return sr_launch_status();
}

__global__ __launch_bounds__(256) void k_convt_strip_reduce(const ConvParams p, const float* __restrict__ prow,
                                                            const float* __restrict__ pcol, int ks_row, int ks_col) {
    const int rw = p.IW + 1, ch = p.IH, OW = p.OW, OH = p.OH;
    const int per_row = OW + OH - 1;
    const int64_t planes = (int64_t)p.B * p.N, total = planes * per_row;
    for (int64_t i = (int64_t)blockIdx.x * blockDim.x + threadIdx.x; i < total;
         i += (int64_t)gridDim.x * blockDim.x) {
        const int64_t row = i / per_row;
        const int q = (int)(i - row * per_row);
        float acc;
        int64_t o;
        acc = 0.0f;
        if (q < OW) {
            const int g = q >> 1;
            const float* t = prow + row * rw + g;
            for (int s = 0; s < ks_row; ++s, t += 3 * planes * rw)
                acc += (q & 1) ? t[planes * rw] : t[0] + t[2 * planes * rw];
            o = (int64_t)(OH - 1) * OW + q;
        } else {
            const int Y = q - OW, g = Y >> 1;
            const float* t = pcol + row * ch + g;
            for (int s = 0; s < ks_col; ++s, t += 3 * planes * ch)
                acc += (Y & 1) ? t[planes * ch] : t[0] + t[2 * planes * ch];
            o = (int64_t)Y * OW + (OW - 1);
        }
        if (p.oscale) acc *= p.oscale[row];
        if (p.obias) acc += p.obias[row % p.N];
        p.out[row * (int64_t)OH * OW + o] = acc;
    }
}

constexpr int STRIP_KS = 4;
int64_t convt_strip_floats(int64_t B, int64_t N, int64_t IH, int64_t IW) { return STRIP_KS * 3 * B * N * (IW + 1 + IH); }

template <int PW, int PH, int PB>
int launch_strip_part(ConvParams& p, hipStream_t st) {
    p.tiles_x = (p.GW - p.gx_base + PW - 1) / PW;
    p.tiles_y = (p.GH - p.gy_base + PH - 1) / PH;
    p.tiles_b = (p.B + PB - 1) / PB;
    p.tiles_n = (p.N + BN - 1) / BN;
    int64_t blocks = (int64_t)p.tiles_x * p.tiles_y * p.tiles_b * p.tiles_n * p.tap_count;
    p.ks = 1; p.c_per_slice = (p.C + 15) / 16 * 16;
    for (int ks = STRIP_KS; ks >= 2; ks /= 2)
        if (p.C % (16 * ks) == 0 && p.C / ks >= 64 && blocks * ks <= 4 * SR_NUM_CU) {
            p.ks = ks;
            p.c_per_slice = p.C / ks;
            break;
        }
    blocks *= p.ks;
    if (blocks > 0x7FFFFFFFLL) return SR_ERANGE;
    if (PB == 1 && taps_v4(p)) return launch_one<1, 1, 1, PW, PH, PB, PB == 1, true>(p, dim3((unsigned)blocks), st);
    return launch_one<1, 1, 1, PW, PH, PB, false, true>(p, dim3((unsigned)blocks), st);
}

int launch_convt_strips(ConvParams p, hipStream_t st) {
    float* prow = p.partial;
    float* pcol = p.partial + STRIP_KS * 3 * (int64_t)p.B * p.N * (p.IW + 1);
    p.osy = p.osx = 2; p.ooy = p.oox = 0;
    p.dy0 = p.dx0 = 0;
    p.ks = 1; p.c_per_slice = (p.C + 15) / 16 * 16;
    p.gy_base = p.IH; p.GH = p.IH + 1; p.gx_base = 0; p.GW = p.IW + 1;
    p.tap_first = 6; p.tap_step = 1; p.tap_count = 3;
    p.partial = prow;
    int rc = launch_strip_part<32, 4, 1>(p, st);
    if (rc != SR_OK) return rc;
    const int ks_row = p.ks;
    p.gy_base = 0; p.GH = p.IH; p.gx_base = p.IW; p.GW = p.IW + 1;
    p.tap_first = 2; p.tap_step = 3; p.tap_count = 3;
    p.partial = pcol;
    rc = launch_strip_part<4, 4, 8>(p, st);
    if (rc != SR_OK) return rc;
    const int ks_col = p.ks;
    const int64_t total = (int64_t)p.B * p.N * (p.OW + p.OH - 1);
    hipLaunchKernelGGL(k_convt_strip_reduce, dim3(sr_stream_grid(total, 256)), dim3(256), 0, st, p, prow, pcol, ks_row,
                       ks_col);
    return sr_launch_status();
}

bool wino_enabled() {
    const char* e = std::getenv("SR_WINOGRAD");
    return !(e && e[0] == '0');
}

bool rot_enabled() {
    const char* e = std::getenv("SR_CONV_ROT");
    return !(e && e[0] == '0');
}

template <int IS, int TY, int TX>
int launch_by_patch(ConvParams& p, hipStream_t st) {
    int pw, ph, pb;
    const int ext_w = p.GW - p.gx_base, ext_h = p.GH - p.gy_base;
    if (ext_w <= 0 || ext_h <= 0) return SR_OK;
    choose_split(ext_h, ext_w, p.B, p.N, p.C, p.ks, p.c_per_slice);
    if (!p.partial || (int64_t)p.ks * p.B * p.N * ext_h * ext_w > p.partial_floats) {
        p.ks = 1;
        p.c_per_slice = (p.C + 15) / 16 * 16;
    }
    patch_shape(ext_w, pw, ph, pb);
    p.tiles_x = (ext_w + pw - 1) / pw;
    p.tiles_y = (ext_h + ph - 1) / ph;
    p.tiles_b = (p.B + pb - 1) / pb;
    p.tiles_n = (p.N + BN - 1) / BN;
    const int64_t blocks = (int64_t)p.tiles_x * p.tiles_y * p.tiles_b * p.tiles_n * p.ks;
    if (blocks <= 0) return SR_OK;
    if (blocks > 0x7FFFFFFFLL) return SR_ERANGE;
    const dim3 grid((unsigned)blocks);
    const bool v4 = IS == 1 && pb == 1 && p.IW % 4 == 0 && (reinterpret_cast<uintptr_t>(p.in) & 15) == 0 &&
                    p.gx_base % 4 == 0 && p.dx0 == (TX > 1 ? -1 : 0);
    const bool rot = IS == 2 && pb == 1 && (p.IW & 3) == 1 && ((p.IH * p.IW) & 3) == 1 && p.C % 4 == 0 &&
                     (reinterpret_cast<uintptr_t>(p.in) & 15) == 0 && p.dx0 >= 0 && p.dy0 >= 0 && p.gx_base == 0 &&
                     p.gy_base == 0 && (p.GW - 1) * 2 + p.dx0 + TX <= p.IW && (p.GH - 1) * 2 + p.dy0 + TY <= p.IH &&
                     ext_w % pw == 0 && ext_h % ph == 0 && rot_enabled();
    int rc;
    if (IS == 1 && v4) {
        if (pw == 32) rc = launch_one<1, TY, TX, 32, 4, 1, true>(p, grid, st);
        else rc = launch_one<1, TY, TX, 16, 8, 1, true>(p, grid, st);
    } else if (IS == 2 && rot && TY == 3 && TX == 3) {
        if (pw == 32) rc = launch_one<2, 3, 3, 32, 4, 1, true>(p, grid, st);
        else rc = launch_one<2, 3, 3, 16, 8, 1, true>(p, grid, st);
    } else if (pw == 32) rc = launch_one<IS, TY, TX, 32, 4, 1, false>(p, grid, st);
    else if (pw == 16) rc = launch_one<IS, TY, TX, 16, 8, 1, false>(p, grid, st);
    else if (pw == 8) rc = launch_one<IS, TY, TX, 8, 8, 2, false>(p, grid, st);
    else rc = launch_one<IS, TY, TX, 4, 4, 8, false>(p, grid, st);
    if (rc != SR_OK || p.ks <= 1) return rc;
    const int64_t total = (int64_t)p.B * p.N * ext_h * ext_w;
    hipLaunchKernelGGL(k_conv_reduce, dim3(sr_stream_grid(total, 256)), dim3(256), 0, st, p, ext_h, ext_w);
    return sr_launch_status();
}

}

extern "C" int64_t sr_conv2d_scratch_floats(int64_t B, int64_t C, int64_t N, int64_t IH, int64_t IW,
                                            int64_t OH, int64_t OW, int ksize, int stride, int pad,
                                            int transposed) {
    (void)ksize; (void)stride; (void)pad;
    if (B <= 0 || C <= 0 || N <= 0 || OH <= 0 || OW <= 0) return 0;
    int ks, per;
    int64_t need = 0;
    auto consider = [&](int64_t gh, int64_t gw) {
        if (gh <= 0 || gw <= 0) return;
        choose_split((int)gh, (int)gw, (int)B, (int)N, (int)C, ks, per);
        if (ks > 1) need = need > ks * B * N * gh * gw ? need : ks * B * N * gh * gw;
    };
    if (!transposed) {
        consider(OH, OW);
        if (ksize == 3 && stride == 2 && pad == 0 && sr_wgrad_bf16x3_enabled('c') &&
            sr_conv_s2_bf16x3_eligible(B, C, N, IH, IW, OH, OW)) {
            const int64_t w = sr_conv_s2_bf16x3_scratch_floats(C, N);
            need = need > w ? need : w;
        }
        if (ksize == 3 && stride == 1 && pad == 1 && wino_enabled() &&
            sr_wino_eligible(B, C, N, IH, IW, nullptr, nullptr)) {
            const int64_t w = sr_wino_scratch_floats(C, N) + sr_wino_partial_floats(B, C, N, IH, IW);
            need = need > w ? need : w;
        }
    } else {
        consider(IH + 1, IW + 1);
        consider(IH, IW);
        consider(1, IW + 1);
        consider(IH, 1);
        if (ksize == 3 && stride == 2 && pad == 0 && convt_taps_wanted(B, C, N, IH, IW)) {
            const int64_t w = convt_taps_floats(B, C, N, IH, IW);
            need = need > w ? need : w;
        }
        if (ksize == 3 && stride == 2 && pad == 0) {
            const int64_t w = convt_strip_floats(B, N, IH, IW), f = convt_fused_split_floats(B, C, N, IH, IW);
            need = need > w ? need : w;
            need = need > f ? need : f;
        }
        if (ksize == 3 && stride == 2 && pad == 0 && sr_wgrad_bf16x3_enabled('t') && sr_convt_bf16x3_eligible(B, C, N, IH, IW)) {
            const int64_t w = sr_convt_bf16x3_scratch_floats(C, N);
            need = need > w ? need : w;
        }
    }
    return need;
}

extern "C" int sr_conv2d_uses_winograd(int64_t B, int64_t C, int64_t N, int64_t IH, int64_t IW, const float* in,
                                       const float* out) {
    return (wino_enabled() && sr_wino_eligible(B, C, N, IH, IW, in, out)) ? 1 : 0;
}

extern "C" int sr_conv2d_mfma_ex(float* out, const float* in, const float* wt, const float* iscale,
                              const float* oscale, const float* obias, int64_t B, int64_t C,
                              int64_t N, int64_t wt_ld, int64_t IH, int64_t IW, int64_t OH, int64_t OW,
                              int ksize, int stride, int pad, int transposed, int flags, float* scratch,
                              sr_stream_t stream) {
    if (B < 0 || C <= 0 || N <= 0 || IH <= 0 || IW <= 0 || OH <= 0 || OW <= 0) return SR_EINVAL;
    if (wt_ld < N || wt_ld % 4 != 0 || (reinterpret_cast<uintptr_t>(wt) & 15)) return SR_EINVAL;
    if (B == 0) return SR_OK;
    if (!out || !in || !wt) return SR_EINVAL;
    if (B * C * IH * IW >= (1LL << 31) || B * N * OH * OW >= (1LL << 40) ||
        (int64_t)ksize * ksize * C * wt_ld >= (1LL << 31))
        return SR_ERANGE;
    hipStream_t st = sr_stream(stream);
    ConvParams p;
    p.in = in; p.wt = wt; p.iscale = iscale; p.oscale = oscale; p.obias = obias; p.out = out;
    p.B = (int)B; p.C = (int)C; p.N = (int)N; p.ldw = (int)wt_ld;
    p.IH = (int)IH; p.IW = (int)IW; p.OH = (int)OH; p.OW = (int)OW;
    p.partial = scratch;
    p.partial_floats = scratch ? sr_conv2d_scratch_floats(B, C, N, IH, IW, OH, OW, ksize, stride, pad, transposed) : 0;
    for (int i = 0; i < 9; ++i) p.wmap[i] = 0;
    p.ks = 1; p.c_per_slice = (p.C + 15) / 16 * 16;
    p.tap_first = 0; p.tap_step = 1; p.tap_count = 9;
    if (!transposed) {
        if (OH != (IH + 2 * pad - ksize) / stride + 1 || OW != (IW + 2 * pad - ksize) / stride + 1)
            return SR_EINVAL;
        p.GH = p.OH; p.GW = p.OW;
        p.gy_base = p.gx_base = 0;
        p.osy = p.osx = 1; p.ooy = p.oox = 0;
        p.dy0 = p.dx0 = -pad;
        for (int i = 0; i < ksize * ksize; ++i) p.wmap[i] = i;
        int rc;
        if (ksize == 3 && stride == 1 && pad == 1 && scratch && wino_enabled() &&
            sr_wino_eligible(B, C, N, IH, IW, in, out))
            return sr_wino_conv3x3(out, in, wt, wt_ld, iscale, oscale, obias, B, C, N, IH, IW, scratch, st, nullptr,
                                   (flags & SR_CONV_U_READY) != 0);
        if (ksize == 3 && stride == 2 && pad == 0 && scratch && sr_wgrad_bf16x3_enabled('c') &&
            sr_conv_s2_bf16x3_eligible(B, C, N, IH, IW, OH, OW))
            return sr_conv_s2_bf16x3_launch(out, in, wt, wt_ld, iscale, oscale, obias, B, C, N, IH, IW, OH, OW, scratch, st);
        if (ksize == 3 && stride == 1) rc = launch_by_patch<1, 3, 3>(p, st);
        else if (ksize == 3 && stride == 2) rc = launch_by_patch<2, 3, 3>(p, st);
        else if (ksize == 1 && stride == 1) {
            if (pad == 0 && sr_conv1x1_gemm_eligible(B, C, N, wt_ld, IH * IW, in, wt, out))
                return sr_conv1x1_gemm_launch(out, in, wt, wt_ld, iscale, oscale, obias, B, C, N, IH * IW, st);
            rc = launch_by_patch<1, 1, 1>(p, st);
        }
        else if (ksize == 1 && stride == 2) rc = launch_by_patch<2, 1, 1>(p, st);
        else return SR_EINVAL;
        return rc;
    }
    if (ksize != 3 || stride != 2 || pad != 0 || OH != 2 * IH + 1 || OW != 2 * IW + 1) return SR_EINVAL;
    if (scratch && convt_taps_wanted(B, C, N, IH, IW) && convt_taps_floats(B, C, N, IH, IW) <= p.partial_floats &&
        !(sr_wgrad_bf16x3_enabled('t') && sr_convt_bf16x3_eligible(B, C, N, IH, IW)))
        return launch_convt_taps(p, st);
    bool fused_ok = false;
    {
        const char* e = std::getenv("SR_CONVT_FUSED");
        const int64_t fused_blocks = (int64_t)(p.IW / TFused::PW) * (p.IH / TFused::PH) * ((p.N + BN - 1) / BN) * p.B;
        bool fused_pays = fused_blocks >= 192 || p.C <= 256;
        if (!fused_pays && scratch && !(e && e[0] == '0')) {
            const char* k = std::getenv("SR_CONVT_FUSED_KS");
            const int ks = (k && k[0] == '0') ? 1 : convt_fused_slices(fused_blocks, p.C);
            if (ks > 1 && convt_fused_eligible(p) && (int64_t)ks * B * N * OH * OW <= p.partial_floats) {
                p.ks = ks;
                p.c_per_slice = p.C / ks;
                fused_pays = true;
            }
        }
        if (scratch && sr_wgrad_bf16x3_enabled('t') && sr_convt_bf16x3_eligible(B, C, N, IH, IW)) {
            const int rc = sr_convt_bf16x3_launch(out, in, wt, wt_ld, iscale, oscale, obias, B, C, N, IH, IW, scratch, st);
            if (rc != SR_OK) return rc;
            fused_ok = true;
        } else if (!(e && e[0] == '0') && p.IW >= 16 && convt_fused_eligible(p) && (fused_pays || (e && e[0] == '1'))) {
            for (int i = 0; i < 9; ++i) p.wmap[i] = i;
            const int rc = launch_convt_fused(p, st);
            p.ks = 1; p.c_per_slice = (p.C + 15) / 16 * 16;
            if (rc != SR_OK) return rc;
            fused_ok = true;
        }
    }
    if (fused_ok && scratch && convt_strip_floats(B, N, IH, IW) <= p.partial_floats) {
        const char* e = std::getenv("SR_CONVT_STRIPS");
        if (!(e && e[0] == '0')) return launch_convt_strips(p, st);
    }
    for (int py = 0; py < 2; ++py)
        for (int px = 0; px < 2; ++px) {
            const int TYp = py == 0 ? 2 : 1, TXp = px == 0 ? 2 : 1;
            p.osy = p.osx = 2; p.ooy = py; p.oox = px;
            p.dy0 = -(TYp - 1); p.dx0 = -(TXp - 1);
            for (int ty = 0; ty < TYp; ++ty)
                for (int tx = 0; tx < TXp; ++tx) {
                    const int ky = py + 2 * (TYp - 1 - ty), kx = px + 2 * (TXp - 1 - tx);
                    p.wmap[ty * TXp + tx] = ky * 3 + kx;
                }
            const int gh_full = py == 0 ? p.IH + 1 : p.IH, gw_full = px == 0 ? p.IW + 1 : p.IW;
            int regions[3][4] = {{0, p.IH, 0, p.IW},
                                 {p.IH, gh_full, 0, gw_full},
                                 {0, p.IH, p.IW, gw_full}};
            const bool split_border = p.IW >= 16;
            if (!split_border) {
                regions[0][1] = gh_full;
                regions[0][3] = gw_full;
            }
            const bool fused = split_border && fused_ok;
            for (int rg = fused ? 1 : 0; rg < (split_border ? 3 : 1); ++rg) {
                p.gy_base = regions[rg][0]; p.GH = regions[rg][1];
                p.gx_base = regions[rg][2]; p.GW = regions[rg][3];
                if (p.GH <= p.gy_base || p.GW <= p.gx_base) continue;
                int rc;
                if (py == 0 && px == 0) rc = launch_by_patch<1, 2, 2>(p, st);
                else if (py == 0) rc = launch_by_patch<1, 2, 1>(p, st);
                else if (px == 0) rc = launch_by_patch<1, 1, 2>(p, st);
                else rc = launch_by_patch<1, 1, 1>(p, st);
                if (rc != SR_OK) return rc;
            }
        }
    return SR_OK;
}

extern "C" int sr_conv2d_mfma(float* out, const float* in, const float* wt, const float* iscale,
                              const float* oscale, const float* obias, int64_t B, int64_t C,
                              int64_t N, int64_t wt_ld, int64_t IH, int64_t IW, int64_t OH, int64_t OW,
                              int ksize, int stride, int pad, int transposed, float* scratch,
                              sr_stream_t stream) {
    return sr_conv2d_mfma_ex(out, in, wt, iscale, oscale, obias, B, C, N, wt_ld, IH, IW, OH, OW, ksize, stride, pad,
                             transposed, 0, scratch, stream);
}

extern "C" int sr_conv2d_nba_ex(float* out, const float* in, const float* wt, const float* iscale, const float* oscale,
                                const float* noise, const float* noise_w, const float* abias, float alpha, float gain,
                                int64_t B, int64_t C, int64_t N, int64_t wt_ld, int64_t H, int64_t W,
                                int64_t noise_bstride, int flags, float* scratch, sr_stream_t stream) {
    if (B < 0 || C <= 0 || N <= 0 || H <= 0 || W <= 0) return SR_EINVAL;
    if (wt_ld < N || wt_ld % 4 != 0 || (reinterpret_cast<uintptr_t>(wt) & 15)) return SR_EINVAL;
    if (B == 0) return SR_OK;
    if (!out || !in || !wt || !scratch || (noise && !noise_w)) return SR_EINVAL;
    if (!wino_enabled() || !sr_wino_eligible(B, C, N, H, W, in, out)) return SR_EINVAL;
    const WinoNba nba{noise, noise_w, abias, noise_bstride, alpha, gain};
    return sr_wino_conv3x3(out, in, wt, wt_ld, iscale, oscale, nullptr, B, C, N, H, W, scratch, sr_stream(stream), &nba,
                           (flags & SR_CONV_U_READY) != 0);
}

extern "C" int sr_conv2d_nba(float* out, const float* in, const float* wt, const float* iscale, const float* oscale,
                             const float* noise, const float* noise_w, const float* abias, float alpha, float gain,
                             int64_t B, int64_t C, int64_t N, int64_t wt_ld, int64_t H, int64_t W,
                             int64_t noise_bstride, float* scratch, sr_stream_t stream) {
    return sr_conv2d_nba_ex(out, in, wt, iscale, oscale, noise, noise_w, abias, alpha, gain, B, C, N, wt_ld, H, W,
                            noise_bstride, 0, scratch, stream);
}
```

### stylerenderer_amd/csrc/conv_wino.h

```cpp
#pragma once
#include <hip/hip_runtime.h>
#include <stdint.h>

struct WinoParams {
    const float* in;
    const float* u;
    const float* iscale;
    const float* oscale;
    const float* obias;
    float* out;
    int B, C, N, H, W;
    int tiles_x, tiles_y, tiles_n;
    int nba;
    const float* nz;
    const float* nz_w;
    const float* abias;
    int64_t nz_bstride;
    float alpha, gain;
    int ks, kchunks;
    float* partial;
};

struct WinoNba {
    const float* nz;
    const float* nz_w;
    const float* abias;
    int64_t nz_bstride;
    float alpha, gain;
};

bool sr_wino_eligible(int64_t B, int64_t C, int64_t N, int64_t H, int64_t W, const void* in, const void* out);
int64_t sr_wino_scratch_floats(int64_t C, int64_t N);
int sr_wino_split(int64_t B, int64_t C, int64_t N, int64_t H, int64_t W);
int64_t sr_wino_partial_floats(int64_t B, int64_t C, int64_t N, int64_t H, int64_t W);
int sr_wino_conv3x3(float* out, const float* in, const float* wt, int64_t ldw, const float* iscale,
                    const float* oscale, const float* obias, int64_t B, int64_t C, int64_t N, int64_t H, int64_t W,
                    float* u_scratch, hipStream_t st, const WinoNba* nba = nullptr, bool u_ready = false);

bool sr_wgrad_wino_eligible(int64_t B, int64_t C, int64_t N, int64_t H, int64_t W, const void* x, const void* gy);
int64_t sr_wgrad_wino_scratch_floats(int64_t B, int64_t C, int64_t N, int64_t H, int64_t W);
int sr_wgrad_wino_3x3(float* dwt, const float* x, const float* gy, const float* xscale, const float* gscale,
                      int64_t B, int64_t C, int64_t N, int64_t H, int64_t W, float* scratch, hipStream_t st);
```

### stylerenderer_amd/csrc/conv_wino.hip

```cpp
#include <type_traits>
#include "common.h"
#include "conv_wino.h"
#include <cstdlib>

namespace {

typedef float f32x16 __attribute__((ext_vector_type(16)));
typedef const void __attribute__((address_space(1)))* gptr_t;
typedef void __attribute__((address_space(3)))* lptr_t;

__device__ __attribute__((aligned(16))) const float g_wino_zero[4] = {0.f, 0.f, 0.f, 0.f};

constexpr int TW = 16, TH = 4;
constexpr int NB = 64;
constexpr int EH = 2 * TH + 2;
constexpr int LEAD = 3;
constexpr int EWP = 40;
constexpr int PLANE = EH * EWP;

#ifdef WINO_TIMING
__device__ long long g_wino_stamps[8 * 16384];
#define WINO_STAMP(i) do { if (tid == 0) { g_wino_stamps[(blockIdx.x & 16383) * 8 + (i)] = wall_clock64(); } } while (0)
#else
#define WINO_STAMP(i)
#endif

template <int KC>
struct WG {
    static constexpr int CQ = KC / 4;
    static constexpr int PPS = CQ * 512;
    static constexpr int UV = 8 * PPS;
    static constexpr int U_INSTR = UV / 256;
    static constexpr int D_FLOATS = KC * PLANE;
    static constexpr int D_INSTR = (D_FLOATS / 4 + 63) / 64;
    static constexpr int D_BUF = D_INSTR * 256;
    static constexpr int D_PER_WAVE = (D_INSTR + 3) / 4;
    static constexpr int PAD = 4 * UV + 2 * D_BUF;
    static constexpr int STY = PAD + 3 * 256;
};

template <int KC>
__global__ __launch_bounds__(256) void k_conv_wino(const WinoParams p) {
#if __HIP_DEVICE_COMPILE__
    using G = WG<KC>;
    extern __shared__ __attribute__((aligned(16))) float smem[];
    float* const ubuf = smem;
    float* const vbuf = smem + 2 * G::UV;
    float* const dbuf = smem + 4 * G::UV + 1;
    float* const sty = smem + G::STY;

    const int nwg = gridDim.x;
    int bid = blockIdx.x;
    {
        const int q = nwg / SR_NUM_XCD, r = nwg % SR_NUM_XCD, xcd = bid % SR_NUM_XCD;
        bid = (xcd < r ? xcd * (q + 1) : r * (q + 1) + (xcd - r) * q) + bid / SR_NUM_XCD;
    }
    const int slice = bid % p.ks;
    bid /= p.ks;
    const int n_t = bid % p.tiles_n;
    bid /= p.tiles_n;
    const int tx_i = bid % p.tiles_x;
    bid /= p.tiles_x;
    const int ty_i = bid % p.tiles_y;
    const int b = bid / p.tiles_y;
    const int oy0 = ty_i * (2 * TH), ox0 = tx_i * (2 * TW), n0 = n_t * NB;

    const int tid = threadIdx.x, lane = tid & 63;
    const int wave = __builtin_amdgcn_readfirstlane(tid >> 6);
    const int half = lane >> 5, l31 = lane & 31;
    const int wn = wave & 1, wt = wave >> 1;
    const int nchunks = p.kchunks;
    const int k_lo = slice * p.kchunks;
    const int all_chunks = p.C / KC;
    WINO_STAMP(0);
#ifdef WINO_TIMING
    const long long wino_c0 = clock64();
    if (tid == 0) {
        g_wino_stamps[(blockIdx.x & 16383) * 8 + 6] = __builtin_amdgcn_s_getreg((31 << 11) | 4);
        g_wino_stamps[(blockIdx.x & 16383) * 8 + 7] = __builtin_amdgcn_s_getreg((31 << 11) | 20);
    }
#endif

    int d_off[G::D_PER_WAVE];
#pragma unroll
    for (int i = 0; i < G::D_PER_WAVE; ++i) {
        const int j = wave + 4 * i;
        const int f = (j * 64 + lane) * 4;
        int off = 0x7FFFFFF0;
        if (j < G::D_INSTR && f < G::D_FLOATS) {
            const int c = f / PLANE, q = f % PLANE;
            const int r = q / EWP, cola = q % EWP;
            const int gy = oy0 - 1 + r, gx = ox0 - 4 + cola;
            if (gy >= 0 && gy < p.H && gx >= 0 && gx + 3 < p.W) off = ((c * p.H + gy) * p.W + gx) * 4;
        }
        d_off[i] = off;
    }
    const int chunk_in_bytes = KC * p.H * p.W * 4;
    const __amdgpu_buffer_rsrc_t r_in = __builtin_amdgcn_make_buffer_rsrc(
        const_cast<float*>(p.in + ((int64_t)b * p.C + (int64_t)k_lo * KC) * p.H * p.W), 0, nchunks * chunk_in_bytes,
        0x00020000);
    const __amdgpu_buffer_rsrc_t r_u = __builtin_amdgcn_make_buffer_rsrc(
        const_cast<float*>(p.u + ((int64_t)n_t * all_chunks + k_lo) * G::UV), 0, nchunks * G::UV * 4, 0x00020000);
    const int u_voff = lane * 16;

    auto dma_d1 = [&](int k, int buf, int i) {
        const int j = wave + 4 * i;
        float* dst = j < G::D_INSTR ? dbuf + buf * G::D_BUF + j * 256 : smem + G::PAD + (wave - 1) * 256;
        __builtin_amdgcn_raw_ptr_buffer_load_lds(r_in, (lptr_t)dst, 16, d_off[i], k * chunk_in_bytes, 0, 0);
    };
    auto dma_u1 = [&](int k, int buf, int i) {
        const int j = wave + 4 * i;
        __builtin_amdgcn_raw_ptr_buffer_load_lds(r_u, (lptr_t)(ubuf + buf * G::UV + j * 256), 16, u_voff,
                                                 (k * G::UV + j * 256) * 4, 0, 0);
    };
    auto dma_d = [&](int k, int buf) {
#pragma unroll
        for (int i = 0; i < G::D_PER_WAVE; ++i) dma_d1(k, buf, i);
    };
    auto dma_u = [&](int k, int buf) {
#pragma unroll
        for (int i = 0; i < G::U_INSTR / 4; ++i) dma_u1(k, buf, i);
    };

    static_assert(KC == 8, "two channel quads per chunk");
    const int t_cq = wave & 1, t_h = wave >> 1;
    const int t_ca = 4 * t_cq + t_h;
    const int t_rd = t_ca * PLANE + (2 * (lane >> 4)) * EWP + LEAD + 2 * (lane & 15);
    const int t_wr = t_cq * 512 + t_h * 128 + lane * 2;

    typedef float f2 __attribute__((ext_vector_type(2)));
    auto ld2 = [](const float* q) { return *reinterpret_cast<const f2*>(q); };
    auto st2 = [](float* q, f2 v) { *reinterpret_cast<f2*>(q) = v; };
    auto pk_add = [](f2 x, f2 y) { f2 r; asm("v_pk_add_f32 %0, %1, %2" : "=v"(r) : "v"(x), "v"(y)); return r; };
    auto pk_sub = [](f2 x, f2 y) {
        f2 r;
        asm("v_pk_add_f32 %0, %1, %2 neg_lo:[0,1] neg_hi:[0,1]" : "=v"(r) : "v"(x), "v"(y));
        return r;
    };
    auto pk_mul_s = [](f2 x, f2 sv, int ch) {
        f2 r;
        if (ch == 0) asm("v_pk_mul_f32 %0, %1, %2 op_sel:[0,0] op_sel_hi:[1,0]" : "=v"(r) : "v"(x), "v"(sv));
        else asm("v_pk_mul_f32 %0, %1, %2 op_sel:[0,1] op_sel_hi:[1,1]" : "=v"(r) : "v"(x), "v"(sv));
        return r;
    };
    auto pk_fms_s = [](f2 x, f2 sv, f2 y, int ch) {
        f2 r;
        if (ch == 0)
            asm("v_pk_fma_f32 %0, %1, %2, %3 op_sel:[0,0,0] op_sel_hi:[1,0,1] neg_lo:[0,0,1] neg_hi:[0,0,1]"
                : "=v"(r) : "v"(x), "v"(sv), "v"(y));
        else
            asm("v_pk_fma_f32 %0, %1, %2, %3 op_sel:[0,1,0] op_sel_hi:[1,1,1] neg_lo:[0,0,1] neg_hi:[0,0,1]"
                : "=v"(r) : "v"(x), "v"(sv), "v"(y));
        return r;
    };
    auto pk_fnma_s = [](f2 x, f2 sv, f2 y, int ch) {
        f2 r;
        if (ch == 0)
            asm("v_pk_fma_f32 %0, %1, %2, %3 op_sel:[0,0,0] op_sel_hi:[1,0,1] neg_lo:[1,0,0] neg_hi:[1,0,0]"
                : "=v"(r) : "v"(x), "v"(sv), "v"(y));
        else
            asm("v_pk_fma_f32 %0, %1, %2, %3 op_sel:[0,1,0] op_sel_hi:[1,1,1] neg_lo:[1,0,0] neg_hi:[1,0,0]"
                : "=v"(r) : "v"(x), "v"(sv), "v"(y));
        return r;
    };
    auto col01 = [](f2 tp, f2 tq) {
        f2 r;
        asm("v_pk_add_f32 %0, %1, %2 op_sel:[0,0] op_sel_hi:[1,0] neg_lo:[0,1] neg_hi:[0,0]" : "=v"(r) : "v"(tp), "v"(tq));
        return r;
    };
    auto col23 = [](f2 tp, f2 tq) {
        f2 r;
        asm("v_pk_add_f32 %0, %1, %2 op_sel:[0,1] op_sel_hi:[1,1] neg_lo:[0,1] neg_hi:[1,0]" : "=v"(r) : "v"(tq), "v"(tp));
        return r;
    };
    struct XF {
        f2 P[2][4], Q[2][4];
        f2 sp[2][2], sq[2][2];
        f2 tp[2][4], tq[2][4];
        f2 o01[2][4], o23[2][4];
    };
    auto xf_read = [&](XF& x, const float* d0, int r) {
#pragma unroll
        for (int ch = 0; ch < 2; ++ch) {
            x.P[ch][r] = ld2(d0 + ch * 2 * PLANE + r * EWP);
            x.Q[ch][r] = ld2(d0 + ch * 2 * PLANE + r * EWP + 2);
        }
    };
    auto xf_step = [&](XF& x, int step, f2 sv) {
#pragma unroll
        for (int ch = 0; ch < 2; ++ch) {
            if (step == 0) {
                x.sp[ch][0] = pk_mul_s(x.P[ch][1], sv, ch);
                x.sp[ch][1] = pk_mul_s(x.P[ch][2], sv, ch);
                x.sq[ch][0] = pk_mul_s(x.Q[ch][1], sv, ch);
                x.sq[ch][1] = pk_mul_s(x.Q[ch][2], sv, ch);
                x.tp[ch][0] = pk_fms_s(x.P[ch][0], sv, x.sp[ch][1], ch);
                x.tq[ch][0] = pk_fms_s(x.Q[ch][0], sv, x.sq[ch][1], ch);
            } else if (step == 1) {
                x.tp[ch][1] = pk_add(x.sp[ch][0], x.sp[ch][1]);
                x.tq[ch][1] = pk_add(x.sq[ch][0], x.sq[ch][1]);
                x.tp[ch][2] = pk_sub(x.sp[ch][1], x.sp[ch][0]);
                x.tq[ch][2] = pk_sub(x.sq[ch][1], x.sq[ch][0]);
                x.tp[ch][3] = pk_fnma_s(x.P[ch][3], sv, x.sp[ch][0], ch);
                x.tq[ch][3] = pk_fnma_s(x.Q[ch][3], sv, x.sq[ch][0], ch);
            } else {
#pragma unroll
                for (int q = 2 * (step - 2); q < 2 * (step - 2) + 2; ++q) {
                    x.o01[ch][q] = col01(x.tp[ch][q], x.tq[ch][q]);
                    x.o23[ch][q] = col23(x.tp[ch][q], x.tq[ch][q]);
                }
            }
        }
    };
    auto xf_write = [&](const XF& x, float* vout, int q) {
#pragma unroll
        for (int ch = 0; ch < 2; ++ch) {
            st2(vout + (2 * q) * G::PPS + ch * 256, x.o01[ch][q]);
            st2(vout + (2 * q + 1) * G::PPS + ch * 256, x.o23[ch][q]);
        }
    };
    auto transform = [&](int k, int dsel, int vsel) {
        const float* d0 = dbuf + dsel * G::D_BUF + t_rd;
        float* v = vbuf + vsel * G::UV + t_wr;
        f2 sv;
        sv.x = sty[k * KC + t_ca];
        sv.y = sty[k * KC + t_ca + 2];
        XF x;
#pragma unroll
        for (int r = 0; r < 4; ++r) xf_read(x, d0, r);
#pragma unroll
        for (int st = 0; st < 4; ++st) xf_step(x, st, sv);
#pragma unroll
        for (int q = 0; q < 4; ++q) xf_write(x, v, q);
    };

    f32x16 acc[16];
#pragma unroll
    for (int pos = 0; pos < 16; ++pos)
#pragma unroll
        for (int r = 0; r < 16; ++r) acc[pos][r] = 0.0f;

    const int a_off = (half * 64 + wn * 32 + l31) * 2;
    const int b_off = (half * 64 + wt * 32 + l31) * 2;

    dma_d(0, 0);
    dma_u(0, 0);
    if (nchunks > 1) dma_d(1, 1);
    for (int c = tid; c < nchunks * KC; c += 256)
        sty[c] = p.iscale ? p.iscale[(int64_t)b * p.C + k_lo * KC + c] : 1.0f;
    __builtin_amdgcn_s_waitcnt(0x0F70);
    __syncthreads();
    WINO_STAMP(1);
    transform(0, 0, 0);
    WINO_STAMP(2);

    static_assert(KC == 8, "the slot schedule below is written for two channel quads per chunk");
    f2 au[2][2][8], bv[2][2][8];
    auto mfma_step = [&](int cq, int m) {
        const int e = m >> 4, pos = m & 15, pp = pos >> 1;
        if (pos & 1) acc[pos] = __builtin_amdgcn_mfma_f32_32x32x2f32(au[cq][e][pp].y, bv[cq][e][pp].y, acc[pos], 0, 0, 0);
        else acc[pos] = __builtin_amdgcn_mfma_f32_32x32x2f32(au[cq][e][pp].x, bv[cq][e][pp].x, acc[pos], 0, 0, 0);
    };
    auto body = [&](int k, auto first_tag) {
        constexpr bool FIRST = decltype(first_tag)::value;
        __builtin_amdgcn_s_waitcnt(0x0F70);
        __syncthreads();
        const int kd = min(k + 2, nchunks - 1), ku = min(k + 1, nchunks - 1);
        const float* ub = ubuf + (k & 1) * G::UV + a_off;
        const float* vb_ = vbuf + (k & 1) * G::UV + b_off;
        const int kn = (k + 1 < nchunks) ? k + 1 : k;
        const float* d0 = dbuf + ((k + 1) & 1) * G::D_BUF + t_rd;
        float* vout = vbuf + ((k + 1) & 1) * G::UV + t_wr;
        f2 sab;
        sab.x = sty[kn * KC + t_ca];
        sab.y = sty[kn * KC + t_ca + 2];
        XF x;
        auto load_ops = [&](int cq, int pp) {
#pragma unroll
            for (int e = 0; e < 2; ++e) {
                au[cq][e][pp] = ld2(ub + pp * G::PPS + cq * 512 + e * 256);
                bv[cq][e][pp] = ld2(vb_ + pp * G::PPS + cq * 512 + e * 256);
            }
        };
#ifndef WINO_RD
#define WINO_RD "0123"
#define WINO_ST "4567"
#define WINO_WR "CDEF"
#define WINO_L0 "4567"
#define WINO_L1 "89AB"
#define WINO_DD "45"
#define WINO_DU "89AB"
#endif
        constexpr char RD[] = WINO_RD, ST[] = WINO_ST, WR[] = WINO_WR, L0[] = WINO_L0, L1[] = WINO_L1, DD[] = WINO_DD,
                       DU[] = WINO_DU;
        static_assert(sizeof(RD) == 5 && sizeof(ST) == 5 && sizeof(WR) == 5 && sizeof(L0) == 5 && sizeof(L1) == 5 &&
                      sizeof(DD) == 3 && sizeof(DU) == 5, "schedule strings");
        static_assert(G::D_PER_WAVE == 4 && G::U_INSTR / 4 == 8, "4 halo + 8 weight DMA instructions per wave");
#pragma unroll
        for (int s = 0; s < 16; ++s) {
            const int cq = (s < 8) ? 1 : 0, j = s & 7;
            const char d = s < 10 ? '0' + s : 'A' + (s - 10);
            if (!(FIRST && s < 8)) {
#pragma unroll
                for (int u = 0; u < 4; ++u) mfma_step(cq, 4 * j + u);
            }
#pragma unroll
            for (int i = 0; i < 4; ++i) {
                if (L0[i] == d) { load_ops(0, 2 * i); load_ops(0, 2 * i + 1); }
                if (L1[i] == d) { load_ops(1, 2 * i); load_ops(1, 2 * i + 1); }
            }
#ifndef WINO_NO_DMA
#pragma unroll
            for (int i = 0; i < 4; ++i) {
                if (i < 2 && DD[i] == d) { dma_d1(kd, k & 1, 2 * i); dma_d1(kd, k & 1, 2 * i + 1); }
                if (DU[i] == d) { dma_u1(ku, (k + 1) & 1, 2 * i); dma_u1(ku, (k + 1) & 1, 2 * i + 1); }
            }
#endif
#ifndef WINO_NO_XFORM
#pragma unroll
            for (int i = 0; i < 4; ++i) if (RD[i] == d) xf_read(x, d0, i);
#pragma unroll
            for (int i = 0; i < 4; ++i) if (ST[i] == d) xf_step(x, i, sab);
#pragma unroll
            for (int i = 0; i < 4; ++i) if (WR[i] == d) xf_write(x, vout, i);
#endif
            __builtin_amdgcn_sched_barrier(0);
        }
    };
    body(0, std::true_type{});
    for (int k = 1; k < nchunks; ++k) body(k, std::false_type{});
#pragma unroll
    for (int m = 0; m < 32; ++m) mfma_step(1, m);

    __builtin_amdgcn_s_waitcnt(0x0F70);
    WINO_STAMP(3);

    const int tile = wt * 32 + l31;
    const int oy = oy0 + 2 * (tile >> 4), ox = ox0 + 2 * (tile & 15);
    const int64_t plane = (int64_t)p.H * p.W;
    float nzv[2][2] = {{0.0f, 0.0f}, {0.0f, 0.0f}};
    if (p.nba && p.nz) {
#pragma clang fp contract(off)
        const float nw = p.nz_w[0];
        const float* nzp = p.nz + b * p.nz_bstride + (int64_t)oy * p.W + ox;
#pragma unroll
        for (int a = 0; a < 2; ++a) {
            nzv[a][0] = nw * nzp[a * p.W];
            nzv[a][1] = nw * nzp[a * p.W + 1];
        }
    }
#pragma unroll
    for (int r = 0; r < 16; ++r) {
        const int n = n0 + wn * 32 + (r & 3) + 8 * (r >> 2) + 4 * half;
        float s[2][4];
#pragma unroll
        for (int j = 0; j < 4; ++j) {
            const float m0 = acc[j][r], m1 = acc[4 + j][r], m2 = acc[8 + j][r], m3 = acc[12 + j][r];
            s[0][j] = (m0 + m1) + m2;
            s[1][j] = (m1 - m2) - m3;
        }
        if (p.ks > 1) {
            float* o = p.partial + (((int64_t)slice * p.B + b) * p.N + n) * plane + (int64_t)oy * p.W + ox;
            *reinterpret_cast<float2*>(o) = make_float2((s[0][0] + s[0][1]) + s[0][2], (s[0][1] - s[0][2]) - s[0][3]);
            *reinterpret_cast<float2*>(o + p.W) = make_float2((s[1][0] + s[1][1]) + s[1][2], (s[1][1] - s[1][2]) - s[1][3]);
            continue;
        }
        const float os = p.oscale ? p.oscale[(int64_t)b * p.N + n] : 1.0f;
        const float ob = p.obias ? p.obias[n] : 0.0f;
        float* o = p.out + ((int64_t)b * p.N + n) * plane + (int64_t)oy * p.W + ox;
        const float ab = (p.nba && p.abias) ? p.abias[n] : 0.0f;
        float y[2][2];
#pragma unroll
        for (int a = 0; a < 2; ++a) {
            const float y0 = (s[a][0] + s[a][1]) + s[a][2];
            const float y1 = (s[a][1] - s[a][2]) - s[a][3];
            float v0 = y0 * os + ob, v1 = y1 * os + ob;
            if (p.nba) {
#pragma clang fp contract(off)
                v0 = v0 + nzv[a][0];
                v1 = v1 + nzv[a][1];
                v0 = v0 + ab;
                v1 = v1 + ab;
                v0 = ((v0 > 0.0f) ? v0 : v0 * p.alpha) * p.gain;
                v1 = ((v1 > 0.0f) ? v1 : v1 * p.alpha) * p.gain;
            }
            y[a][0] = v0;
            y[a][1] = v1;
        }
        *reinterpret_cast<float2*>(o) = make_float2(y[0][0], y[0][1]);
        *reinterpret_cast<float2*>(o + p.W) = make_float2(y[1][0], y[1][1]);
    }
    WINO_STAMP(4);
#ifdef WINO_TIMING
    if (tid == 0) g_wino_stamps[(blockIdx.x & 16383) * 8 + 5] = clock64() - wino_c0;
#endif
#endif
}

__global__ __launch_bounds__(256) void k_wino_reduce(const WinoParams p) {
    const int64_t plane = (int64_t)p.H * p.W, total4 = (int64_t)p.B * p.N * plane / 4;
    const int64_t slab4 = total4;
    for (int64_t i = (int64_t)blockIdx.x * 256 + threadIdx.x; i < total4; i += (int64_t)gridDim.x * 256) {
        const float4* src = reinterpret_cast<const float4*>(p.partial) + i;
        float4 a = src[0];
        for (int s = 1; s < p.ks; ++s) {
            const float4 q = src[s * slab4];
            a.x += q.x; a.y += q.y; a.z += q.z; a.w += q.w;
        }
        const int64_t row = (i * 4) / plane;
        const int n = (int)(row % p.N), b = (int)(row / p.N);
        const int64_t pix = i * 4 - row * plane;
        const float os = p.oscale ? p.oscale[row] : 1.0f;
        const float ob = p.obias ? p.obias[n] : 0.0f;
        float v[4] = {a.x * os + ob, a.y * os + ob, a.z * os + ob, a.w * os + ob};
        if (p.nba) {
#pragma clang fp contract(off)
            const float ab = p.abias ? p.abias[n] : 0.0f;
            float nz[4] = {0.0f, 0.0f, 0.0f, 0.0f};
            if (p.nz) {
                const float nw = p.nz_w[0];
                const float4 q = *reinterpret_cast<const float4*>(p.nz + b * p.nz_bstride + pix);
                nz[0] = nw * q.x; nz[1] = nw * q.y; nz[2] = nw * q.z; nz[3] = nw * q.w;
            }
#pragma unroll
            for (int j = 0; j < 4; ++j) {
                float t = v[j] + nz[j];
                t = t + ab;
                v[j] = ((t > 0.0f) ? t : t * p.alpha) * p.gain;
            }
        }
        reinterpret_cast<float4*>(p.out)[i] = make_float4(v[0], v[1], v[2], v[3]);
    }
}

template <int KC>
__global__ __launch_bounds__(64) void k_wino_weights(float* __restrict__ u, const float* __restrict__ wt, int C,
                                                     int N, int ldw) {
    using G = WG<KC>;
    const int n = blockIdx.x * 64 + threadIdx.x, c = blockIdx.y;
    float g[3][3];
#pragma unroll
    for (int t = 0; t < 9; ++t) g[t / 3][t % 3] = wt[((int64_t)t * C + c) * ldw + n];
    float h[4][3];
#pragma unroll
    for (int j = 0; j < 3; ++j) {
        h[0][j] = g[0][j];
        h[1][j] = 0.5f * ((g[0][j] + g[2][j]) + g[1][j]);
        h[2][j] = 0.5f * ((g[0][j] + g[2][j]) - g[1][j]);
        h[3][j] = g[2][j];
    }
    const int cl = c % KC, cq = cl / 4, e = (cl % 4) / 2, hh = cl % 2;
    float* dst = u + ((int64_t)blockIdx.x * (C / KC) + c / KC) * G::UV + cq * 512 + e * 256 + hh * 128 + threadIdx.x * 2;
#pragma unroll
    for (int i = 0; i < 4; ++i) {
        *reinterpret_cast<float2*>(dst + (2 * i) * G::PPS) = make_float2(h[i][0], 0.5f * ((h[i][0] + h[i][2]) + h[i][1]));
        *reinterpret_cast<float2*>(dst + (2 * i + 1) * G::PPS) = make_float2(0.5f * ((h[i][0] + h[i][2]) - h[i][1]), h[i][2]);
    }
}

template <int KC>
int launch(const WinoParams& p, float* u, const float* wt, int ldw, hipStream_t st, bool u_ready) {
    using G = WG<KC>;
    const int lds = (G::STY + p.kchunks * KC) * 4;
    auto kern = k_conv_wino<KC>;
    static bool configured = false;
    if (!configured) {
        if (hipFuncSetAttribute(reinterpret_cast<const void*>(kern), hipFuncAttributeMaxDynamicSharedMemorySize,
                                160 * 1024) != hipSuccess) {
            (void)hipGetLastError();
            return SR_EINVAL;
        }
        configured = true;
    }
    if (!u_ready) hipLaunchKernelGGL(k_wino_weights<KC>, dim3(p.N / 64, p.C), dim3(64), 0, st, u, wt, p.C, p.N, ldw);
    const int64_t blocks = (int64_t)p.tiles_n * p.tiles_x * p.tiles_y * p.B * p.ks;
    hipLaunchKernelGGL(kern, dim3((unsigned)blocks), dim3(256), lds, st, p);
    if (p.ks > 1) {
        const int64_t total4 = (int64_t)p.B * p.N * p.H * p.W / 4;
        int64_t grid = (total4 + 255) / 256;
        if (grid > 8192) grid = 8192;
        hipLaunchKernelGGL(k_wino_reduce, dim3((unsigned)grid), dim3(256), 0, st, p);
    }
    return sr_launch_status();
}

}

#ifdef WINO_TIMING
extern "C" int sr_debug_wino_stamps(long long* host, int n) {
    return (int)hipMemcpyFromSymbol(host, HIP_SYMBOL(g_wino_stamps), (size_t)n * sizeof(long long));
}
#endif

bool sr_wino_eligible(int64_t B, int64_t C, int64_t N, int64_t H, int64_t W, const void* in, const void* out) {
    if (B <= 0 || C % 8 != 0 || N % 64 != 0 || H % 8 != 0 || W % 32 != 0) return false;
    if (C > 512 || B * ((W / 32) * (H / 8)) * (N / 64) > 0x7FFFFFFFLL) return false;
    if (C * H * W >= (1LL << 29) - 4 || 16 * C * 64 >= (1LL << 29)) return false;
    return ((reinterpret_cast<uintptr_t>(in) | reinterpret_cast<uintptr_t>(out)) & 15) == 0;
}

int64_t sr_wino_scratch_floats(int64_t C, int64_t N) { return 16 * C * N; }

int sr_wino_split(int64_t B, int64_t C, int64_t N, int64_t H, int64_t W) {
    const char* e = std::getenv("SR_WINO_SPLIT");
    if (e && e[0] == '0') return 1;
    const int64_t blocks = B * (W / (2 * TW)) * (H / (2 * TH)) * (N / NB), nchunks = C / 8;
    int ks = 1;
    while (blocks * ks < 192 && ks < 8 && nchunks % (2 * ks) == 0 && nchunks / (2 * ks) >= 8) ks *= 2;
    return ks;
}
int64_t sr_wino_partial_floats(int64_t B, int64_t C, int64_t N, int64_t H, int64_t W) {
    const int ks = sr_wino_split(B, C, N, H, W);
    return ks > 1 ? (int64_t)ks * B * N * H * W : 0;
}

int sr_wino_conv3x3(float* out, const float* in, const float* wt, int64_t ldw, const float* iscale,
                    const float* oscale, const float* obias, int64_t B, int64_t C, int64_t N, int64_t H, int64_t W,
                    float* u_scratch, hipStream_t st, const WinoNba* nba, bool u_ready) {
    WinoParams p;
    p.in = in; p.u = u_scratch; p.iscale = iscale; p.oscale = oscale; p.obias = obias; p.out = out;
    p.nba = nba ? 1 : 0;
    p.nz = nba ? nba->nz : nullptr; p.nz_w = nba ? nba->nz_w : nullptr; p.abias = nba ? nba->abias : nullptr;
    p.nz_bstride = nba ? nba->nz_bstride : 0; p.alpha = nba ? nba->alpha : 0.0f; p.gain = nba ? nba->gain : 1.0f;
    p.B = (int)B; p.C = (int)C; p.N = (int)N; p.H = (int)H; p.W = (int)W;
    p.tiles_x = (int)(W / (2 * TW)); p.tiles_y = (int)(H / (2 * TH)); p.tiles_n = (int)(N / NB);
    p.ks = sr_wino_split(B, C, N, H, W);
    p.kchunks = (int)(C / 8) / p.ks;
    p.partial = u_scratch + sr_wino_scratch_floats(C, N);
    return launch<8>(p, u_scratch, wt, (int)ldw, st, u_ready);
}
```

### stylerenderer_amd/op/conv.py

```python
import os

import torch

from .. import _lib
from ._dispatch import hold_for_capture, mark_inputs, on_device_of, require_f32, stream_of, wanted
from . import weight_prep as _wp
from .fused_elem import rowdot, rowdot_div


PROFILE = None


def _timed(kind, geom, flops, launch):
    if PROFILE is None:
        return launch()
    e0, e1 = torch.cuda.Event(enable_timing=True), torch.cuda.Event(enable_timing=True)
    e0.record()
    rc = launch()
    e1.record()
    PROFILE.append((kind, geom, flops, e0, e1))
    return rc


def conv_out_size(ih, iw, ksize, stride, pad, transposed):
    if transposed:
        return (ih - 1) * stride + ksize - 2 * pad, (iw - 1) * stride + ksize - 2 * pad
    return (ih + 2 * pad - ksize) // stride + 1, (iw + 2 * pad - ksize) // stride + 1


def conv2d_mfma(x, wt, iscale=None, oscale=None, obias=None, ksize=3, stride=1, pad=1,
                transposed=False):
    require_f32(x, "conv2d_mfma")
    require_f32(wt, "conv2d_mfma weight")
    x = x.contiguous()
    b, c, ih, iw = x.shape
    taps, cw, n = wt.shape
    if (wt.stride(2) == 1 and wt.stride(1) % 4 == 0 and wt.stride(1) >= n and wt.stride(0) == cw * wt.stride(1)
            and wt.data_ptr() % 16 == 0):
        ldw = wt.stride(1)
    else:
        ldw = (n + 3) // 4 * 4
        wt = torch.nn.functional.pad(wt, (0, ldw - n)) if ldw != n else wt.contiguous()
    if taps != ksize * ksize or cw != c:
        raise RuntimeError("conv2d_mfma: weight must be [k*k, C, N]; got %s for C=%d k=%d"
                           % (tuple(wt.shape), c, ksize))
    oh, ow = conv_out_size(ih, iw, ksize, stride, pad, transposed)
    for t, shape, name in ((iscale, (b, c), "iscale"), (oscale, (b, n), "oscale"), (obias, (n,), "obias")):
        if t is not None:
            require_f32(t, "conv2d_mfma " + name)
            if tuple(t.shape) != shape or not t.is_contiguous():
                raise RuntimeError("conv2d_mfma: %s must be contiguous %s" % (name, shape))
    out = torch.empty((b, n, oh, ow), dtype=x.dtype, device=x.device)
    gh, gw = (ih, iw) if transposed else (oh, ow)
    flops = 2.0 * b * gh * gw * c * n * ksize * ksize
    L = _lib.lib()
    nscr = L.sr_conv2d_scratch_floats(b, c, n, ih, iw, oh, ow, ksize, stride, pad, int(bool(transposed)))
    scratch, flags, entry = _conv_scratch(wt, nscr, (b, c, n, ih, iw, ksize, stride, pad, bool(transposed)), x)
    with on_device_of(x):
        rc = _timed("conv", (ksize, stride, int(bool(transposed)), b, c, n, gh, gw), flops,
                    lambda: L.sr_conv2d_mfma_ex(
                        _lib.ptr(out), _lib.ptr(x), _lib.ptr(wt), _lib.ptr(iscale), _lib.ptr(oscale),
                        _lib.ptr(obias), b, c, n, ldw, ih, iw, oh, ow, ksize, stride, pad,
                        int(bool(transposed)), flags, _lib.ptr(scratch), stream_of(x)))
    _lib.check(rc, "sr_conv2d_mfma")
    _scratch_written(entry, b, c, n, ih, iw, x, out)
    return out


class _Scratch:
    __slots__ = ("buf", "ready")

    def __init__(self, buf):
        self.buf, self.ready = buf, False


def _conv_scratch(wt, nscr, key, like):
    if nscr <= 0:
        return None, 0, None
    if not (getattr(wt, "_sr_frozen", False) and key[5:] == (3, 1, 1, False)) or os.environ.get("SR_U_CACHE", "1") == "0":
        return torch.empty(nscr, dtype=like.dtype, device=like.device), 0, None
    cache = wt.__dict__.setdefault("_sr_scratch", {})
    k = key + (os.environ.get("SR_WINOGRAD", "1"), os.environ.get("SR_WINO_SPLIT", "1"), wt._version, wt.data_ptr())
    hit = cache.get(k)
    if hit is None or hit.buf.numel() < nscr:
        if len(cache) >= 6:
            cache.clear()
        hit = cache[k] = _Scratch(torch.empty(nscr, dtype=like.dtype, device=like.device))
    hold_for_capture(hit.buf)
    return hit.buf, (1 if hit.ready else 0), hit


def _scratch_written(entry, b, c, n, h, w, x, out):
    if entry is None or entry.ready:
        return
    if x.is_cuda and torch.cuda.is_current_stream_capturing():
        return
    if _lib.lib().sr_conv2d_uses_winograd(b, c, n, h, w, _lib.ptr(x), _lib.ptr(out)):
        entry.ready = True


def conv2d_wgrad_mfma(x, gy, xscale=None, gscale=None, ksize=3, stride=1, pad=1, transposed=False):
    require_f32(x, "conv2d_wgrad_mfma")
    require_f32(gy, "conv2d_wgrad_mfma grad")
    x = x.contiguous()
    gy = gy.contiguous()
    b, c, ih, iw = x.shape
    b2, n, oh, ow = gy.shape
    if b2 != b or (oh, ow) != conv_out_size(ih, iw, ksize, stride, pad, transposed):
        raise RuntimeError("conv2d_wgrad_mfma: shape mismatch x %s gy %s" % (tuple(x.shape), tuple(gy.shape)))
    for t, shape, name in ((xscale, (b, c), "xscale"), (gscale, (b, n), "gscale")):
        if t is not None and (tuple(t.shape) != shape or not t.is_contiguous() or t.dtype != torch.float32):
            raise RuntimeError("conv2d_wgrad_mfma: %s must be contiguous float32 %s" % (name, shape))
    if (ksize == 1 and stride == 1 and pad == 0 and not transposed and c <= 4 and xscale is None and gscale is None
            and (ih * iw) % 4 == 0 and b * n <= 65535 and n <= 4096 and os.environ.get("SR_WGRAD_SMALL", "1") != "0"):
        from .smallconv import _dw

        return _dw(x, gy).sum(0).view(1, c, n)
    L = _lib.lib()
    nfl = L.sr_conv2d_wgrad_scratch_floats(b, c, n, ih, iw, oh, ow, ksize, stride, pad, int(bool(transposed)))
    if nfl < 0:
        raise RuntimeError("conv2d_wgrad_mfma: unsupported geometry")
    scratch = torch.empty(nfl, dtype=torch.float32, device=x.device)
    dwt = torch.empty((ksize * ksize, c, n), dtype=torch.float32, device=x.device)
    gh, gw = (ih, iw) if transposed else (oh, ow)
    flops = 2.0 * b * gh * gw * c * n * ksize * ksize
    with on_device_of(x):
        rc = _timed("wgrad", (ksize, stride, int(bool(transposed)), b, c, n, gh, gw), flops,
                    lambda: L.sr_conv2d_wgrad_mfma(
                        _lib.ptr(dwt), _lib.ptr(x), _lib.ptr(gy), _lib.ptr(xscale), _lib.ptr(gscale),
                        b, c, n, ih, iw, oh, ow, ksize, stride, pad, int(bool(transposed)),
                        _lib.ptr(scratch), stream_of(x)))
    _lib.check(rc, "sr_conv2d_wgrad_mfma")
    return dwt


_ADJOINT = {"c3": "c3", "c3s2": "t3s2", "t3s2": "c3s2", "c1": "c1"}
_GEOM = {
    "c3": (3, 1, 1, False), "c3s2": (3, 2, 0, False), "t3s2": (3, 2, 0, True), "c1": (1, 1, 0, False),
    "c1s2": (1, 2, 0, False),
}


def adjoint_weight(wt, geom, frozen=False, banked=None):
    if banked is not None and banked[0] == (geom == "c3") and not torch.is_grad_enabled():
        return banked[1]
    if frozen and not wt.requires_grad and not torch.is_grad_enabled():
        return _wp.adjoint_cached(wt, geom == "c3")
    return _wp.adjoint(wt, geom == "c3")


def _bc(s):
    return s[:, :, None, None]


class ConvFn(torch.autograd.Function):
    @staticmethod
    def forward(ctx, x, wt, iscale, oscale, bias, geom):
        mark_inputs(ctx, x, wt, iscale, oscale, bias, geom)
        k, stride, pad, tr = _GEOM[geom]
        out = conv2d_mfma(x, wt, iscale, oscale, bias, k, stride, pad, tr)
        ctx.frozen = bool(getattr(wt, "_sr_frozen", False))
        ctx.adj = getattr(wt, "_sr_adj", None)
        ctx.geom = geom
        ctx.has = (iscale is not None, oscale is not None, bias is not None)
        ctx.save_for_backward(x, wt, iscale, oscale, bias, out if oscale is not None else None)
        return out

    @staticmethod
    def backward(ctx, g):
        x, wt, iscale, oscale, bias, out = ctx.saved_tensors
        need_x, need_w, need_is, need_os, need_b = wanted(ctx)[:5]
        geom = ctx.geom
        g = g.contiguous()
        gx = gw = gis = gos = gb = None
        if need_x or need_is:
            if geom == "c1s2":
                inner = ConvFn.apply(g, adjoint_weight(wt, "c1", ctx.frozen, ctx.adj), oscale, None, None, "c1")
                dxu = torch.zeros_like(x)
                dxu[:, :, ::2, ::2] = inner
            else:
                dxu = ConvFn.apply(g, adjoint_weight(wt, geom, ctx.frozen, ctx.adj), oscale, None, None, _ADJOINT[geom])
            if need_is and need_x and iscale is not None:
                gis, gx = rowdot(x, dxu, iscale)
            else:
                if need_is:
                    gis = rowdot(x, dxu)
                if need_x:
                    gx = dxu * _bc(iscale) if iscale is not None else dxu
        if need_w:
            gw = WgradFn.apply(x, g, iscale, oscale, geom)
        if need_os:
            y0 = out - bias[None, :, None, None] if bias is not None else out
            gos = rowdot_div(g, y0, oscale)
        if need_b:
            gb = g.sum((0, 2, 3))
        return gx, gw, gis, gos, gb, None


class WgradFn(torch.autograd.Function):
    @staticmethod
    def forward(ctx, x, g, iscale, oscale, geom):
        mark_inputs(ctx, x, g, iscale, oscale, geom)
        k, stride, pad, tr = _GEOM[geom]
        ctx.geom = geom
        ctx.save_for_backward(x, g, iscale, oscale)
        return conv2d_wgrad_mfma(x, g, iscale, oscale, k, stride, pad, tr)

    @staticmethod
    def backward(ctx, gg):
        x, g, iscale, oscale = ctx.saved_tensors
        need_x, need_g, need_is, need_os = wanted(ctx)[:4]
        geom = ctx.geom
        gg = gg.contiguous()
        gx = g_g = gis = gos = None
        if need_x or need_is:
            if geom == "c1s2":
                inner = ConvFn.apply(g, adjoint_weight(gg, "c1"), oscale, None, None, "c1")
                dxu = torch.zeros_like(x)
                dxu[:, :, ::2, ::2] = inner
            else:
                dxu = ConvFn.apply(g, adjoint_weight(gg, geom), oscale, None, None, _ADJOINT[geom])
            if need_is:
                gis = rowdot(x, dxu)
            if need_x:
                gx = dxu * _bc(iscale) if iscale is not None else dxu
        if need_g or need_os:
            dgu = ConvFn.apply(x, gg, iscale, None, None, geom)
            if need_os:
                gos = rowdot(g, dgu)
            if need_g:
                g_g = dgu * _bc(oscale) if oscale is not None else dgu
        return gx, g_g, gis, gos, None


def _aliases(*tensors):
    return [t.view_as(t) if t is not None else None for t in tensors]


def conv_nba_shape_ok(x, n, noise):
    import os

    if os.environ.get("SR_WINOGRAD", "1") == "0" or x.device.type != "cuda" or x.dtype != torch.float32:
        return False
    b, c, h, w = x.shape
    ok = (h % 8 == 0 and w % 32 == 0 and c % 8 == 0 and c <= 512 and n % 64 == 0
          and b * n <= 65535 and x.is_contiguous() and x.data_ptr() % 16 == 0)
    if noise is not None:
        ok = ok and noise.dtype == torch.float32 and noise.numel() in (h * w, b * h * w) and noise.data_ptr() % 16 == 0
    return ok


def conv_nba_supported(x, wt, noise):
    return wt.shape[0] == 9 and conv_nba_shape_ok(x, wt.shape[2], noise)


def _wt_pitch(wt):
    taps, cw, n = wt.shape
    if (wt.stride(2) == 1 and wt.stride(1) % 4 == 0 and wt.stride(1) >= n and wt.stride(0) == cw * wt.stride(1)
            and wt.data_ptr() % 16 == 0):
        return wt, wt.stride(1)
    ldw = (n + 3) // 4 * 4
    return (torch.nn.functional.pad(wt, (0, ldw - n)) if ldw != n else wt.contiguous()), ldw


class ConvNBAFn(torch.autograd.Function):
    @staticmethod
    def forward(ctx, x, wt, iscale, oscale, noise, noise_w, abias, slope, gain):
        mark_inputs(ctx, x, wt, iscale, oscale, noise, noise_w, abias, slope, gain)
        b, c, h, w = x.shape
        n = wt.shape[2]
        wtp, ldw = _wt_pitch(wt)
        out = torch.empty((b, n, h, w), dtype=x.dtype, device=x.device)
        L = _lib.lib()
        nscr = L.sr_conv2d_scratch_floats(b, c, n, h, w, h, w, 3, 1, 1, 0)
        scratch, flags, entry = _conv_scratch(wt if wtp is wt else wtp, max(nscr, 1), (b, c, n, h, w, 3, 1, 1, False), x)
        bstride = 0 if noise is None or noise.numel() == h * w else h * w
        flops = 2.0 * b * h * w * c * n * 9
        with on_device_of(x):
            rc = _timed("conv", (3, 1, 0, b, c, n, h, w), flops,
                        lambda: L.sr_conv2d_nba_ex(_lib.ptr(out), _lib.ptr(x), _lib.ptr(wtp), _lib.ptr(iscale),
                                                   _lib.ptr(oscale), _lib.ptr(noise), _lib.ptr(noise_w), _lib.ptr(abias),
                                                   float(slope), float(gain), b, c, n, ldw, h, w, bstride, flags,
                                                   _lib.ptr(scratch), stream_of(x)))
        _lib.check(rc, "sr_conv2d_nba")
        _scratch_written(entry, b, c, n, h, w, x, out)
        ctx.save_for_backward(x, wt, iscale, oscale, noise, noise_w, abias, out)
        ctx.cfg = (float(slope), float(gain))
        ctx.frozen = bool(getattr(wt, "_sr_frozen", False))
        ctx.adj = getattr(wt, "_sr_adj", None)
        return out

    @staticmethod
    def backward(ctx, gy):
        from .fused_elem import _NBA

        x, wt, iscale, oscale, noise, noise_w, abias, out = ctx.saved_tensors
        slope, gain = ctx.cfg
        needs = wanted(ctx)
        if torch.is_grad_enabled() and oscale is not None:
            with torch.enable_grad():
                xa, wa, sa, da, nwa, aba = _aliases(x, wt, iscale, oscale, noise_w, abias)
                y0 = ConvFn.apply(xa, wa, sa, da, None, "c3")
                y = _NBA.apply(y0, noise, nwa, aba, slope, gain, out.detach())
                ins = (xa, wa, sa, da, None, nwa, aba)
                sel = [t for t, nd in zip(ins, needs[:7]) if nd and t is not None]
                got = iter(torch.autograd.grad(y, sel, gy, create_graph=True, allow_unused=True)) if sel else iter(())
                grads = [next(got) if (nd and t is not None) else None for t, nd in zip(ins, needs[:7])]
            return tuple(grads) + (None, None)
        want_p = bool(needs[6] or (noise is not None and needs[5]))
        if oscale is None:
            from .fused_elem import _NBABackward

            g, gb, gnw = _NBABackward.apply(gy, out, noise, slope, gain, want_p)
            rdot = None
        else:
            g, gb, gnw, rdot = _nba_bwd_dot(gy, out, noise, noise_w, abias, slope, gain, want_p)
        gx = gw = gis = gos = None
        if needs[0] or needs[2]:
            dxu = ConvFn.apply(g, adjoint_weight(wt, "c3", ctx.frozen, ctx.adj), oscale, None, None, "c3")
            if needs[2] and needs[0] and iscale is not None:
                gis, gx = rowdot(x, dxu, iscale)
            else:
                if needs[2] and iscale is not None:
                    gis = rowdot(x, dxu)
                if needs[0]:
                    gx = dxu * _bc(iscale) if iscale is not None else dxu
        if needs[1]:
            gw = WgradFn.apply(x, g, iscale, oscale, "c3")
        if needs[3] and oscale is not None:
            gos = rdot / oscale
        return (gx, gw, gis, gos, None, (gnw if noise is not None and want_p and needs[5] else None),
                (gb if want_p and needs[6] else None), None, None)


def _nba_bwd_dot(gy, out, noise, noise_w, abias, slope, gain, want_params=True):
    gy = gy.contiguous()
    b, n, h, w = out.shape
    inner = h * w
    L = _lib.lib()
    g = torch.empty_like(out)
    gb = (torch.zeros if out.numel() == 0 else torch.empty)(n if want_params else 0, dtype=out.dtype, device=out.device)
    gnw = (torch.empty if (noise is not None and out.numel() > 0) else torch.zeros)(1 if want_params else 0,
                                                                                        dtype=out.dtype, device=out.device)
    rdot = torch.empty((b, n), dtype=out.dtype, device=out.device)
    scratch = torch.empty(L.sr_noise_bias_act_bwd_dot_scratch_floats(b, n, inner), dtype=out.dtype, device=out.device)
    bstride = 0 if noise is None or noise.numel() == inner else inner
    with on_device_of(out):
        rc = L.sr_noise_bias_act_bwd_dot(_lib.ptr(g), _lib.ptr(gb) if want_params else None,
                                         _lib.ptr(gnw) if want_params else None, _lib.ptr(rdot), _lib.ptr(gy),
                                         _lib.ptr(out), _lib.ptr(noise), _lib.ptr(noise_w), _lib.ptr(abias), slope, gain,
                                         b, n, inner, bstride, _lib.ptr(scratch), stream_of(out))
    _lib.check(rc, "sr_noise_bias_act_bwd_dot")
    return g, gb, gnw, rdot


def _blur_bwd_fused():
    import os

    return os.environ.get("SR_BLUR_BWD_FUSED", "1") != "0"


def _blur_nba_bwd(gy, out, k_flipped, p0, shape257, noise, noise_w, abias, slope, gain, want_params=True):
    gy = gy.contiguous()
    b, n, oh, ow = out.shape
    L = _lib.lib()
    g257 = torch.empty(shape257, dtype=out.dtype, device=out.device)
    gb = torch.empty(n if want_params else 0, dtype=out.dtype, device=out.device)
    gnw = (torch.empty if noise is not None else torch.zeros)(1 if want_params else 0, dtype=out.dtype, device=out.device)
    rdot = torch.empty((b, n), dtype=out.dtype, device=out.device)
    scratch = torch.empty(L.sr_blur_nba_bwd_scratch_floats(b, n, shape257[2], shape257[3]), dtype=out.dtype,
                          device=out.device)
    bstride = 0 if noise is None or noise.numel() == oh * ow else oh * ow
    with on_device_of(out):
        rc = L.sr_blur_nba_bwd(_lib.ptr(g257), _lib.ptr(gb) if want_params else None,
                               _lib.ptr(gnw) if want_params else None, _lib.ptr(rdot), _lib.ptr(gy), _lib.ptr(out),
                               _lib.ptr(k_flipped), _lib.ptr(noise), _lib.ptr(noise_w), _lib.ptr(abias), slope, gain, b, n,
                               oh, ow, shape257[2], shape257[3], p0, bstride, _lib.ptr(scratch), stream_of(out))
    _lib.check(rc, "sr_blur_nba_bwd")
    return g257, gb, gnw, rdot


def upconv_nba_supported(x, wt, noise, oh, ow):
    b = x.shape[0]
    n = wt.shape[2]
    ok = (x.device.type == "cuda" and x.dtype == torch.float32 and wt.shape[0] == 9 and (oh * ow) % 4 == 0
          and b * n <= 65535)
    if noise is not None:
        ok = ok and noise.dtype == torch.float32 and noise.numel() in (oh * ow, b * oh * ow) and noise.data_ptr() % 16 == 0
    return ok


class UpConvNBAFn(torch.autograd.Function):

    @staticmethod
    def forward(ctx, x, wt, iscale, oscale, kernel, pad, noise, noise_w, abias, slope, gain):
        from .fused_elem import _BlurNBA

        mark_inputs(ctx, x, wt, iscale, oscale, kernel, pad, noise, noise_w, abias, slope, gain)
        y257 = conv2d_mfma(x, wt, iscale, oscale, None, 3, 2, 0, True)
        out = _BlurNBA.forward(_NoCtx(), y257, kernel, pad, noise, noise_w, abias, slope, gain)
        ctx.save_for_backward(x, wt, iscale, oscale, kernel, noise, noise_w, abias, out)
        ctx.cfg = (tuple(pad), float(slope), float(gain), tuple(y257.shape))
        ctx.frozen = bool(getattr(wt, "_sr_frozen", False))
        ctx.adj = getattr(wt, "_sr_adj", None)
        return out

    @staticmethod
    def backward(ctx, gy):
        from .fused_elem import _BlurNBA
        from .upfirdn2d import flipped, upfirdn2d_op

        x, wt, iscale, oscale, kernel, noise, noise_w, abias, out = ctx.saved_tensors
        pad, slope, gain, shape257 = ctx.cfg
        needs = wanted(ctx)
        if torch.is_grad_enabled():
            with torch.enable_grad():
                xa, wa, sa, da, nwa, aba = _aliases(x, wt, iscale, oscale, noise_w, abias)
                y = ConvFn.apply(xa, wa, sa, da, None, "t3s2")
                o = _BlurNBA.apply(y, kernel, pad, noise, nwa, aba, slope, gain, out.detach())
                ins = (xa, wa, sa, da, None, None, None, nwa, aba)
                sel = [t for t, nd in zip(ins, needs[:9]) if nd and t is not None]
                got = iter(torch.autograd.grad(o, sel, gy, create_graph=True, allow_unused=True)) if sel else iter(())
                grads = [next(got) if (nd and t is not None) else None for t, nd in zip(ins, needs[:9])]
            return tuple(grads) + (None, None)
        want_p = bool(needs[8] or (noise is not None and needs[7]))
        p0 = pad[0]
        oh, ow = out.shape[2], out.shape[3]
        if (_blur_bwd_fused() and pad[0] == pad[1] and shape257[2] == oh + 3 - 2 * p0 and shape257[3] == ow + 3 - 2 * p0
                and tuple(kernel.shape) == (4, 4)):
            g257, gb, gnw, rdot = _blur_nba_bwd(gy, out, flipped(kernel), p0, shape257, noise, noise_w, abias, slope,
                                                gain, want_p)
        else:
            g, gb, gnw, rdot = _nba_bwd_dot(gy, out, noise, noise_w, abias, slope, gain, want_p)
            g257 = upfirdn2d_op(g.reshape(-1, oh, ow, 1), flipped(kernel), 1, 1, 1, 1, 3 - p0,
                                shape257[3] - ow + p0, 3 - p0, shape257[2] - oh + p0).view(shape257)
        gx = gw = gis = gos = None
        if needs[0] or needs[2]:
            dxu = ConvFn.apply(g257, adjoint_weight(wt, "t3s2", ctx.frozen, ctx.adj), oscale, None, None, "c3s2")
            if needs[2] and needs[0] and iscale is not None:
                gis, gx = rowdot(x, dxu, iscale)
            else:
                if needs[2] and iscale is not None:
                    gis = rowdot(x, dxu)
                if needs[0]:
                    gx = dxu * _bc(iscale) if iscale is not None else dxu
        if needs[1]:
            gw = WgradFn.apply(x, g257, iscale, oscale, "t3s2")
        if needs[3] and oscale is not None:
            gos = rdot / oscale
        return (gx, gw, gis, gos, None, None, None, (gnw if noise is not None and want_p and needs[7] else None),
                (gb if want_p and needs[8] else None), None, None)


class _NoCtx:

    def save_for_backward(self, *a):
        pass


def upconv_nba(x, wt, iscale, oscale, kernel, pad, noise, noise_w, abias, slope=0.2, gain=2 ** 0.5):
    return UpConvNBAFn.apply(x, wt, iscale, oscale, kernel, tuple(pad), noise, noise_w, abias, slope, gain)


def conv2d_nba(x, wt, iscale, oscale, noise, noise_w, abias, slope=0.2, gain=2 ** 0.5):
    return ConvNBAFn.apply(x, wt, iscale, oscale, noise, noise_w, abias, slope, gain)


class Conv1x1AddFn(torch.autograd.Function):

    @staticmethod
    def forward(ctx, x, wt, oscale, addend):
        mark_inputs(ctx, x, wt, oscale, addend)
        b, c, h, w = x.shape
        n = wt.shape[2]
        out = torch.empty((b, n, h, w), dtype=x.dtype, device=x.device)
        with on_device_of(x):
            rc = _lib.lib().sr_conv1x1_add(_lib.ptr(out), _lib.ptr(x), _lib.ptr(wt), _lib.ptr(oscale), _lib.ptr(addend),
                                           b, c, n, wt.stride(1), h * w, stream_of(x))
        _lib.check(rc, "sr_conv1x1_add")
        ctx.frozen = bool(getattr(wt, "_sr_frozen", False))
        ctx.adj = getattr(wt, "_sr_adj", None)
        ctx.save_for_backward(x, wt, oscale)
        return out

    @staticmethod
    def backward(ctx, g):
        x, wt, oscale = ctx.saved_tensors
        need_x, need_w, _, need_a = wanted(ctx)[:4]
        g = g.contiguous()
        gx = gw = None
        if need_x:
            gx = ConvFn.apply(g, adjoint_weight(wt, "c1", ctx.frozen, ctx.adj), oscale, None, None, "c1")
        if need_w:
            gw = WgradFn.apply(x, g, None, oscale, "c1")
        return gx, gw, None, (g if need_a else None)


def conv1x1_add(x, wt, oscale, addend):
    ok = (x.device.type == "cuda" and x.dtype == torch.float32 and addend.dtype == torch.float32 and x.is_contiguous()
          and addend.is_contiguous() and wt.dim() == 3 and wt.shape[0] == 1 and wt.stride(2) == 1
          and wt.stride(1) % 4 == 0 and (oscale is None or (oscale.is_contiguous() and not oscale.requires_grad))
          and tuple(addend.shape) == (x.shape[0], wt.shape[2], x.shape[2], x.shape[3]))
    if ok:
        b, c, h, w = x.shape
        ok = bool(_lib.lib().sr_conv1x1_add_supported(b, c, wt.shape[2], wt.stride(1), h * w, _lib.ptr(x), _lib.ptr(wt),
                                                      _lib.ptr(addend), _lib.ptr(addend)))
    if not ok:
        return ConvFn.apply(x, wt, None, oscale, None, "c1") + addend
    return Conv1x1AddFn.apply(x, wt, oscale, addend)


def conv2d(x, wt, iscale=None, oscale=None, bias=None, geom="c3"):
    return ConvFn.apply(x, wt, iscale, oscale, bias, geom)
```

Before: 550.1.

## Fuse input-scale gradient dot product into conv data-gradient epilogue

Adds a fused dgrad+rowdot path in which the conv backward-data kernels (MFMA direct, Winograd, and the split-K reduce) compute the per-(batch,channel) dot with the input activation in their epilogue. They write partial sums per tile, and a small finish kernel reduces those into the modulation-scale gradient. This avoids materialising the unscaled dx and re-reading it plus x in a separate rowdot kernel. The cost is extra register and LDS pressure in the epilogue, more template instantiations, and a fallback path when a shape is unsupported.

Result: no change. 553.2 (median of 6 runs) (+0.6%).

```diff
diff --git a/include/stylerenderer_amd.h b/include/stylerenderer_amd.h
--- a/include/stylerenderer_amd.h
+++ b/include/stylerenderer_amd.h
@@ -260,6 +260,16 @@
 
 #define SR_CONV_U_READY 1
 int sr_conv2d_uses_winograd(int64_t B, int64_t C, int64_t N, int64_t IH, int64_t IW, const float* in, const float* out);
+
+int sr_conv2d_dgrad_dot_supported(int64_t B, int64_t C, int64_t N, int64_t IH, int64_t IW, int64_t OH, int64_t OW,
+                                  int ksize, int stride, int pad, int transposed, const float* in, const float* out,
+                                  const float* dot_x);
+int64_t sr_conv2d_dgrad_dot_scratch_floats(int64_t B, int64_t C, int64_t N, int64_t IH, int64_t IW, int64_t OH,
+                                           int64_t OW, int ksize, int stride, int pad, int transposed);
+int sr_conv2d_dgrad_dot(float* out, float* gis, const float* in, const float* wt, const float* iscale,
+                        const float* dot_x, const float* dot_scale, int64_t B, int64_t C, int64_t N, int64_t wt_ld,
+                        int64_t IH, int64_t IW, int64_t OH, int64_t OW, int ksize, int stride, int pad, int flags,
+                        float* scratch, float* dot_scratch, sr_stream_t stream);
 
 int sr_conv2d_generic(float* y, const float* x, const float* w, const float* bias, int64_t B, int64_t C, int64_t N,
                       int64_t IH, int64_t IW, int64_t OH, int64_t OW, int kh, int kw, int sy, int sx, int py, int px,
diff --git a/stylerenderer_amd/_lib.py b/stylerenderer_amd/_lib.py
--- a/stylerenderer_amd/_lib.py
+++ b/stylerenderer_amd/_lib.py
@@ -109,6 +109,9 @@
     "sr_conv2d_mfma": (_i, [_p] * 6 + [_l] * 8 + [_i] * 4 + [_p, _p]),
     "sr_conv2d_uses_winograd": (_i, [_l] * 5 + [_p, _p]),
     "sr_conv2d_mfma_ex": (_i, [_p] * 6 + [_l] * 8 + [_i] * 5 + [_p, _p]),
+    "sr_conv2d_dgrad_dot_supported": (_i, [_l] * 7 + [_i] * 4 + [_p] * 3),
+    "sr_conv2d_dgrad_dot_scratch_floats": (_l, [_l] * 7 + [_i] * 4),
+    "sr_conv2d_dgrad_dot": (_i, [_p] * 7 + [_l] * 8 + [_i] * 4 + [_p] * 3),
     "sr_conv1x1_add_supported": (_i, [_l] * 5 + [_p] * 4),
     "sr_conv1x1_add": (_i, [_p] * 5 + [_l] * 5 + [_p]),
     "sr_rasterize_grad_f64": (_i, [_l] * 5 + [_i] * 2 + [_p, _p, _l] + [_p] * 6 + [_l, _l, _p, _p, _p, _d, _p, _p]),
diff --git a/stylerenderer_amd/csrc/conv_mfma.hip b/stylerenderer_amd/csrc/conv_mfma.hip
--- a/stylerenderer_amd/csrc/conv_mfma.hip
+++ b/stylerenderer_amd/csrc/conv_mfma.hip
@@ -38,6 +38,10 @@
     int64_t partial_floats;
     int ks, c_per_slice;
     int tap_first, tap_step, tap_count;
+    const float* dot_x;
+    const float* dot_scale;
+    float* dot_partial;
+    int dot_tiles;
 };
 
 template <int IS, int TY, int TX, int PW, int PH, int PB, bool V4, bool TAP9 = false>
@@ -64,10 +68,11 @@
     static constexpr int LDS_BYTES = 2 * BUF * 4;
 };
 
-template <int IS, int TY, int TX, int PW, int PH, int PB, bool V4, bool FAST, bool TAP9 = false>
+template <int IS, int TY, int TX, int PW, int PH, int PB, bool V4, bool FAST, bool TAP9 = false, bool DOT = false>
 __global__ __launch_bounds__(256) void k_conv_mfma(const ConvParams p) {
     using G = Geo<IS, TY, TX, PW, PH, PB, V4, TAP9>;
     static_assert(PW * PH * PB == BM, "patch must hold 128 pixels");
+    static_assert(!DOT || (!TAP9 && PB <= 2), "dot epilogue: a wave's 64 pixels belong to one sample");
     static_assert(!TAP9 || (IS == 1 && TY == 1 && TX == 1), "tap-split mode is a shifted 1x1 convolution");
     extern __shared__ __attribute__((aligned(16))) float smem[];
 
@@ -313,6 +318,63 @@
     }
 
     const int64_t plane_out = (int64_t)p.OH * p.OW;
+    if constexpr (DOT) {
+        constexpr int RP = 72;
+        static_assert(BN * RP <= 2 * G::BUF, "reduction matrix fits the operand buffers");
+        float* const red = smem;
+        const int pb = (wpx * 64) / (PW * PH), b = b0 + pb;
+        bool ok[2];
+        int64_t pix[2];
+#pragma unroll
+        for (int pt = 0; pt < 2; ++pt) {
+            const int m = wpx * 64 + pt * 32 + l31;
+            const int px = m % PW, py = (m / PW) % PH;
+            const int gy = gy0 + py, gx = gx0 + px;
+            ok[pt] = gy < g_gh && gx < g_gw && b < p.B;
+            pix[pt] = (int64_t)(gy * p.osy + g_ooy) * p.OW + (gx * p.osx + g_oox);
+        }
+        __syncthreads();
+#pragma unroll
+        for (int ct = 0; ct < 2; ++ct) {
+            float xv[2][16];
+#pragma unroll
+            for (int r = 0; r < 16; ++r) {
+                const int n = n0 + wco * 64 + ct * 32 + (r & 3) + 8 * (r >> 2) + 4 * half;
+#pragma unroll
+                for (int pt = 0; pt < 2; ++pt)
+                    xv[pt][r] = (ok[pt] && n < p.N) ? p.dot_x[((int64_t)b * p.N + n) * plane_out + pix[pt]] : 0.0f;
+            }
+#pragma unroll
+            for (int r = 0; r < 16; ++r) {
+                const int cl = wco * 64 + ct * 32 + (r & 3) + 8 * (r >> 2) + 4 * half, n = n0 + cl;
+                const bool n_ok = n < p.N && b < p.B;
+                const float ds = (n_ok && p.dot_scale) ? p.dot_scale[(int64_t)b * p.N + n] : 1.0f;
+                float d = 0.0f;
+#pragma unroll
+                for (int pt = 0; pt < 2; ++pt)
+                    if (ok[pt] && n_ok) {
+                        float v = acc[ct][pt][r];
+                        if (p.oscale) v *= p.oscale[(int64_t)b * p.N + n];
+                        if (p.obias) v += p.obias[n];
+                        d += xv[pt][r] * v;
+                        p.out[((int64_t)b * p.N + n) * plane_out + pix[pt]] = v * ds;
+                    }
+                red[cl * RP + wpx * 32 + l31] = d;
+            }
+        }
+        __syncthreads();
+        {
+            const int cl = tid >> 1, part = tid & 1;
+            float sum = 0.0f;
+#pragma unroll
+            for (int i = 0; i < 32; ++i) sum += red[cl * RP + part * 32 + i];
+            if (PB == 1) sum += __shfl_xor(sum, 1, SR_WAVE);
+            const int bo = b0 + (PB == 2 ? part : 0);
+            if ((PB == 2 || part == 0) && bo < p.B && n0 + cl < p.N)
+                p.dot_partial[((int64_t)bo * p.N + n0 + cl) * p.dot_tiles + ty_i * p.tiles_x + tx_i] = sum;
+        }
+        return;
+    }
 #pragma unroll
     for (int pt = 0; pt < 2; ++pt) {
         const int m = wpx * 64 + pt * 32 + l31;
@@ -345,10 +407,10 @@
     }
 }
 
-template <int IS, int TY, int TX, int PW, int PH, int PB, bool V4, bool FAST, bool TAP9 = false>
+template <int IS, int TY, int TX, int PW, int PH, int PB, bool V4, bool FAST, bool TAP9 = false, bool DOT = false>
 int launch_fast(const ConvParams& p, dim3 grid, hipStream_t st) {
     using G = Geo<IS, TY, TX, PW, PH, PB, V4, TAP9>;
-    auto kern = k_conv_mfma<IS, TY, TX, PW, PH, PB, V4, FAST, TAP9>;
+    auto kern = k_conv_mfma<IS, TY, TX, PW, PH, PB, V4, FAST, TAP9, DOT>;
     static bool configured = false;
     if (!configured) {
         (void)hipFuncSetAttribute(reinterpret_cast<const void*>(kern),
@@ -359,12 +421,12 @@
     return sr_launch_status();
 }
 
-template <int IS, int TY, int TX, int PW, int PH, int PB, bool V4, bool TAP9 = false>
+template <int IS, int TY, int TX, int PW, int PH, int PB, bool V4, bool TAP9 = false, bool DOT = false>
 int launch_one(const ConvParams& p, dim3 grid, hipStream_t st) {
     using G = Geo<IS, TY, TX, PW, PH, PB, V4, TAP9>;
     if (p.C % G::KC == 0 && p.c_per_slice % G::KC == 0)
-        return launch_fast<IS, TY, TX, PW, PH, PB, V4, true, TAP9>(p, grid, st);
-    return launch_fast<IS, TY, TX, PW, PH, PB, V4, false, TAP9>(p, grid, st);
+        return launch_fast<IS, TY, TX, PW, PH, PB, V4, true, TAP9, DOT>(p, grid, st);
+    return launch_fast<IS, TY, TX, PW, PH, PB, V4, false, TAP9, DOT>(p, grid, st);
 }
 
 struct TFused {
@@ -684,6 +746,47 @@
         if (p.obias) acc += p.obias[row % p.N];
         p.out[row * plane_out + (int64_t)(gy * p.osy + p.ooy) * p.OW + (gx * p.osx + p.oox)] = acc;
     }
+}
+
+constexpr int DOT_SEG = 1024;
+__global__ __launch_bounds__(256) void k_dgrad_reduce_dot(float* __restrict__ out, const float* __restrict__ partial, int ks,
+                                                          int64_t slab, int plane, const float* __restrict__ dot_x,
+                                                          const float* __restrict__ dot_scale,
+                                                          float* __restrict__ dot_partial) {
+    __shared__ float wsum[4];
+    const int64_t row = blockIdx.y;
+    const float ds = dot_scale ? dot_scale[row] : 1.0f;
+    float d = 0.0f;
+#pragma unroll
+    for (int j = 0; j < DOT_SEG / 256; ++j) {
+        const int q = blockIdx.x * DOT_SEG + j * 256 + threadIdx.x;
+        if (q < plane) {
+            const int64_t at = row * plane + q;
+            float acc = 0.0f;
+#pragma unroll 8
+            for (int s = 0; s < ks; ++s) acc += partial[s * slab + at];
+            d += dot_x[at] * acc;
+            out[at] = acc * ds;
+        }
+    }
+    d = sr_wave_sum(d);
+    if ((threadIdx.x & 63) == 0) wsum[threadIdx.x >> 6] = d;
+    __syncthreads();
+    if (threadIdx.x == 0) dot_partial[row * gridDim.x + blockIdx.x] = (wsum[0] + wsum[1]) + (wsum[2] + wsum[3]);
+}
+
+__global__ __launch_bounds__(64) void k_dgrad_dot_finish(float* __restrict__ gis, const float* __restrict__ partial,
+                                                         int tiles) {
+    const int64_t row = blockIdx.x;
+    float acc = 0.0f;
+    for (int i = threadIdx.x; i < tiles; i += 64) acc += partial[row * tiles + i];
+    acc = sr_wave_sum(acc);
+    if (threadIdx.x == 0) gis[row] = acc;
+}
+
+bool dgrad_dot_enabled() {
+    const char* e = std::getenv("SR_DGRAD_DOT");
+    return !(e && e[0] == '0');
 }
 
 __global__ __launch_bounds__(256) void k_convt_tap_reduce(const ConvParams p) {
@@ -908,6 +1011,23 @@
                      p.gy_base == 0 && (p.GW - 1) * 2 + p.dx0 + TX <= p.IW && (p.GH - 1) * 2 + p.dy0 + TY <= p.IH &&
                      ext_w % pw == 0 && ext_h % ph == 0 && rot_enabled();
     int rc;
+    if (p.dot_x) {
+        if (p.osy != 1 || p.osx != 1 || ext_h != p.OH || ext_w != p.OW || p.oscale || p.obias) return SR_EINVAL;
+        if (p.ks == 1) {
+            if constexpr (IS == 2 && TY == 3 && TX == 3) {
+                if (pb > 2) return SR_EINVAL;
+                p.dot_tiles = p.tiles_x * p.tiles_y;
+                if (rot) rc = pw == 32 ? launch_one<2, 3, 3, 32, 4, 1, true, false, true>(p, grid, st)
+                                       : launch_one<2, 3, 3, 16, 8, 1, true, false, true>(p, grid, st);
+                else if (pw == 32) rc = launch_one<2, 3, 3, 32, 4, 1, false, false, true>(p, grid, st);
+                else if (pw == 16) rc = launch_one<2, 3, 3, 16, 8, 1, false, false, true>(p, grid, st);
+                else rc = launch_one<2, 3, 3, 8, 8, 2, false, false, true>(p, grid, st);
+                return rc;
+            } else {
+                return SR_EINVAL;
+            }
+        }
+    }
     if (IS == 1 && v4) {
         if (pw == 32) rc = launch_one<1, TY, TX, 32, 4, 1, true>(p, grid, st);
         else rc = launch_one<1, TY, TX, 16, 8, 1, true>(p, grid, st);
@@ -919,6 +1039,9 @@
     else if (pw == 8) rc = launch_one<IS, TY, TX, 8, 8, 2, false>(p, grid, st);
     else rc = launch_one<IS, TY, TX, 4, 4, 8, false>(p, grid, st);
     if (rc != SR_OK || p.ks <= 1) return rc;
+    if (p.dot_x)
+        return sr_dgrad_reduce_dot_launch(p.out, p.partial, p.ks, (int64_t)p.B * p.N, (int64_t)ext_h * ext_w, p.dot_x,
+                                          p.dot_scale, p.dot_partial, st);
     const int64_t total = (int64_t)p.B * p.N * ext_h * ext_w;
     hipLaunchKernelGGL(k_conv_reduce, dim3(sr_stream_grid(total, 256)), dim3(256), 0, st, p, ext_h, ext_w);
     return sr_launch_status();
@@ -977,11 +1100,71 @@
     return (wino_enabled() && sr_wino_eligible(B, C, N, IH, IW, in, out)) ? 1 : 0;
 }
 
-extern "C" int sr_conv2d_mfma_ex(float* out, const float* in, const float* wt, const float* iscale,
-                              const float* oscale, const float* obias, int64_t B, int64_t C,
-                              int64_t N, int64_t wt_ld, int64_t IH, int64_t IW, int64_t OH, int64_t OW,
-                              int ksize, int stride, int pad, int transposed, int flags, float* scratch,
-                              sr_stream_t stream) {
+int sr_dgrad_dot_segments(int64_t plane) { return (int)sr_ceil_div(plane, DOT_SEG); }
+
+int sr_dgrad_reduce_dot_launch(float* out, const float* partial, int ks, int64_t rows, int64_t plane, const float* dot_x,
+                               const float* dot_scale, float* dot_partial, hipStream_t st) {
+    if (rows <= 0 || rows > 65535 || plane <= 0 || plane >= (1LL << 31) - DOT_SEG) return SR_ERANGE;
+    hipLaunchKernelGGL(k_dgrad_reduce_dot, dim3((unsigned)sr_dgrad_dot_segments(plane), (unsigned)rows), dim3(256), 0, st, out,
+                       partial, ks, rows * plane, (int)plane, dot_x, dot_scale, dot_partial);
+    return sr_launch_status();
+}
+
+static int dgrad_dot_plan(int64_t B, int64_t C, int64_t N, int64_t IH, int64_t IW, int64_t OH, int64_t OW, int ksize,
+                          int stride, int pad, int transposed, const void* in, const void* out, const void* dot_x,
+                          bool has_scratch, int* tiles) {
+    *tiles = 0;
+    if (!dgrad_dot_enabled() || transposed || B <= 0 || C <= 0 || N <= 0 || B * N > 65535 || ksize != 3) return 0;
+    if (OH * OW >= (1LL << 31) - DOT_SEG) return 0;
+    if (stride == 1 && pad == 1) {
+        if (OH != IH || OW != IW) return 0;
+        if (has_scratch && wino_enabled() && sr_wino_eligible(B, C, N, IH, IW, in, out)) {
+            if (reinterpret_cast<uintptr_t>(dot_x) & 15) return 0;
+            *tiles = sr_wino_dot_tiles(B, C, N, IH, IW);
+            return sr_wino_split(B, C, N, IH, IW) > 1 ? 2 : 1;
+        }
+    } else if (stride == 2 && pad == 0) {
+        if (OH != (IH - 3) / 2 + 1 || OW != (IW - 3) / 2 + 1 || OH <= 0 || OW <= 0) return 0;
+        if (sr_wgrad_bf16x3_enabled('c') && sr_conv_s2_bf16x3_eligible(B, C, N, IH, IW, OH, OW)) return 0;
+    } else {
+        return 0;
+    }
+    int ks, per, pw, ph, pb;
+    choose_split((int)OH, (int)OW, (int)B, (int)N, (int)C, ks, per);
+    if (ks > 1 && has_scratch) {
+        *tiles = sr_dgrad_dot_segments(OH * OW);
+        return 2;
+    }
+    patch_shape((int)OW, pw, ph, pb);
+    if (stride != 2 || pb > 2) return 0;
+    *tiles = (int)(sr_ceil_div(OW, pw) * sr_ceil_div(OH, ph));
+    return 1;
+}
+
+extern "C" int sr_conv2d_dgrad_dot_supported(int64_t B, int64_t C, int64_t N, int64_t IH, int64_t IW, int64_t OH,
+                                             int64_t OW, int ksize, int stride, int pad, int transposed, const float* in,
+                                             const float* out, const float* dot_x) {
+    int tiles;
+    return dgrad_dot_plan(B, C, N, IH, IW, OH, OW, ksize, stride, pad, transposed, in, out, dot_x, true, &tiles);
+}
+
+extern "C" int64_t sr_conv2d_dgrad_dot_scratch_floats(int64_t B, int64_t C, int64_t N, int64_t IH, int64_t IW, int64_t OH,
+                                                      int64_t OW, int ksize, int stride, int pad, int transposed) {
+    int with = 0, without = 0;
+    const int a = dgrad_dot_plan(B, C, N, IH, IW, OH, OW, ksize, stride, pad, transposed, nullptr, nullptr, nullptr, true, &with);
+    const int b = dgrad_dot_plan(B, C, N, IH, IW, OH, OW, ksize, stride, pad, transposed, nullptr, nullptr, nullptr, false, &without);
+    if (!a && !b) return 0;
+    int64_t tiles = sr_dgrad_dot_segments(OH * OW);
+    if (with > tiles) tiles = with;
+    if (without > tiles) tiles = without;
+    return B * N * tiles;
+}
+
+static int conv2d_run(float* out, const float* in, const float* wt, const float* iscale,
+                      const float* oscale, const float* obias, int64_t B, int64_t C,
+                      int64_t N, int64_t wt_ld, int64_t IH, int64_t IW, int64_t OH, int64_t OW,
+                      int ksize, int stride, int pad, int transposed, int flags, float* scratch,
+                      sr_stream_t stream, const WinoDot* dot) {
     if (B < 0 || C <= 0 || N <= 0 || IH <= 0 || IW <= 0 || OH <= 0 || OW <= 0) return SR_EINVAL;
     if (wt_ld < N || wt_ld % 4 != 0 || (reinterpret_cast<uintptr_t>(wt) & 15)) return SR_EINVAL;
     if (B == 0) return SR_OK;
@@ -999,6 +1182,8 @@
     for (int i = 0; i < 9; ++i) p.wmap[i] = 0;
     p.ks = 1; p.c_per_slice = (p.C + 15) / 16 * 16;
     p.tap_first = 0; p.tap_step = 1; p.tap_count = 9;
+    p.dot_x = dot ? dot->x : nullptr; p.dot_scale = dot ? dot->scale : nullptr; p.dot_partial = dot ? dot->partial : nullptr;
+    p.dot_tiles = 0;
     if (!transposed) {
         if (OH != (IH + 2 * pad - ksize) / stride + 1 || OW != (IW + 2 * pad - ksize) / stride + 1)
             return SR_EINVAL;
@@ -1011,8 +1196,9 @@
         if (ksize == 3 && stride == 1 && pad == 1 && scratch && wino_enabled() &&
             sr_wino_eligible(B, C, N, IH, IW, in, out))
             return sr_wino_conv3x3(out, in, wt, wt_ld, iscale, oscale, obias, B, C, N, IH, IW, scratch, st, nullptr,
-                                   (flags & SR_CONV_U_READY) != 0);
-        if (ksize == 3 && stride == 2 && pad == 0 && scratch && sr_wgrad_bf16x3_enabled('c') &&
+                                   (flags & SR_CONV_U_READY) != 0, dot);
+        if (dot && ksize != 3) return SR_EINVAL;
+        if (!dot && ksize == 3 && stride == 2 && pad == 0 && scratch && sr_wgrad_bf16x3_enabled('c') &&
             sr_conv_s2_bf16x3_eligible(B, C, N, IH, IW, OH, OW))
             return sr_conv_s2_bf16x3_launch(out, in, wt, wt_ld, iscale, oscale, obias, B, C, N, IH, IW, OH, OW, scratch, st);
         if (ksize == 3 && stride == 1) rc = launch_by_patch<1, 3, 3>(p, st);
@@ -1026,7 +1212,7 @@
         else return SR_EINVAL;
         return rc;
     }
-    if (ksize != 3 || stride != 2 || pad != 0 || OH != 2 * IH + 1 || OW != 2 * IW + 1) return SR_EINVAL;
+    if (dot || ksize != 3 || stride != 2 || pad != 0 || OH != 2 * IH + 1 || OW != 2 * IW + 1) return SR_EINVAL;
     if (scratch && convt_taps_wanted(B, C, N, IH, IW) && convt_taps_floats(B, C, N, IH, IW) <= p.partial_floats &&
         !(sr_wgrad_bf16x3_enabled('t') && sr_convt_bf16x3_eligible(B, C, N, IH, IW)))
         return launch_convt_taps(p, st);
@@ -1095,6 +1281,33 @@
     return SR_OK;
 }
 
+extern "C" int sr_conv2d_mfma_ex(float* out, const float* in, const float* wt, const float* iscale,
+                              const float* oscale, const float* obias, int64_t B, int64_t C,
+                              int64_t N, int64_t wt_ld, int64_t IH, int64_t IW, int64_t OH, int64_t OW,
+                              int ksize, int stride, int pad, int transposed, int flags, float* scratch,
+                              sr_stream_t stream) {
+    return conv2d_run(out, in, wt, iscale, oscale, obias, B, C, N, wt_ld, IH, IW, OH, OW, ksize, stride, pad, transposed,
+                      flags, scratch, stream, nullptr);
+}
+
+extern "C" int sr_conv2d_dgrad_dot(float* out, float* gis, const float* in, const float* wt, const float* iscale,
+                                   const float* dot_x, const float* dot_scale, int64_t B, int64_t C, int64_t N,
+                                   int64_t wt_ld, int64_t IH, int64_t IW, int64_t OH, int64_t OW, int ksize, int stride,
+                                   int pad, int flags, float* scratch, float* dot_scratch, sr_stream_t stream) {
+    if (B < 0) return SR_EINVAL;
+    if (B == 0) return SR_OK;
+    if (!out || !gis || !in || !dot_x || !dot_scratch) return SR_EINVAL;
+    int tiles;
+    if (!dgrad_dot_plan(B, C, N, IH, IW, OH, OW, ksize, stride, pad, 0, in, out, dot_x, scratch != nullptr, &tiles))
+        return SR_EINVAL;
+    const WinoDot dot{dot_x, dot_scale, dot_scratch};
+    const int rc = conv2d_run(out, in, wt, iscale, nullptr, nullptr, B, C, N, wt_ld, IH, IW, OH, OW, ksize, stride, pad, 0,
+                              flags, scratch, stream, &dot);
+    if (rc != SR_OK) return rc;
+    hipLaunchKernelGGL(k_dgrad_dot_finish, dim3((unsigned)(B * N)), dim3(64), 0, sr_stream(stream), gis, dot_scratch, tiles);
+    return sr_launch_status();
+}
+
 extern "C" int sr_conv2d_mfma(float* out, const float* in, const float* wt, const float* iscale,
                               const float* oscale, const float* obias, int64_t B, int64_t C,
                               int64_t N, int64_t wt_ld, int64_t IH, int64_t IW, int64_t OH, int64_t OW,
diff --git a/stylerenderer_amd/csrc/conv_wino.h b/stylerenderer_amd/csrc/conv_wino.h
--- a/stylerenderer_amd/csrc/conv_wino.h
+++ b/stylerenderer_amd/csrc/conv_wino.h
@@ -19,6 +19,10 @@
     float alpha, gain;
     int ks, kchunks;
     float* partial;
+    const float* dot_x;
+    const float* dot_scale;
+    float* dot_partial;
+    int dot_tiles;
 };
 
 struct WinoNba {
@@ -29,13 +33,25 @@
     float alpha, gain;
 };
 
+struct WinoDot {
+    const float* x;
+    const float* scale;
+    float* partial;
+};
+
+int sr_dgrad_dot_segments(int64_t plane);
+int sr_dgrad_reduce_dot_launch(float* out, const float* partial, int ks, int64_t rows, int64_t plane, const float* dot_x,
+                               const float* dot_scale, float* dot_partial, hipStream_t st);
+
 bool sr_wino_eligible(int64_t B, int64_t C, int64_t N, int64_t H, int64_t W, const void* in, const void* out);
 int64_t sr_wino_scratch_floats(int64_t C, int64_t N);
 int sr_wino_split(int64_t B, int64_t C, int64_t N, int64_t H, int64_t W);
 int64_t sr_wino_partial_floats(int64_t B, int64_t C, int64_t N, int64_t H, int64_t W);
 int sr_wino_conv3x3(float* out, const float* in, const float* wt, int64_t ldw, const float* iscale,
                     const float* oscale, const float* obias, int64_t B, int64_t C, int64_t N, int64_t H, int64_t W,
-                    float* u_scratch, hipStream_t st, const WinoNba* nba = nullptr, bool u_ready = false);
+                    float* u_scratch, hipStream_t st, const WinoNba* nba = nullptr, bool u_ready = false,
+                    const WinoDot* dot = nullptr);
+int sr_wino_dot_tiles(int64_t B, int64_t C, int64_t N, int64_t H, int64_t W);
 
 bool sr_wgrad_wino_eligible(int64_t B, int64_t C, int64_t N, int64_t H, int64_t W, const void* x, const void* gy);
 int64_t sr_wgrad_wino_scratch_floats(int64_t B, int64_t C, int64_t N, int64_t H, int64_t W);
diff --git a/stylerenderer_amd/csrc/conv_wino.hip b/stylerenderer_amd/csrc/conv_wino.hip
--- a/stylerenderer_amd/csrc/conv_wino.hip
+++ b/stylerenderer_amd/csrc/conv_wino.hip
@@ -39,7 +39,7 @@
     static constexpr int STY = PAD + 3 * 256;
 };
 
-template <int KC>
+template <int KC, bool DOT = false>
 __global__ __launch_bounds__(256) void k_conv_wino(const WinoParams p) {
 #if __HIP_DEVICE_COMPILE__
     using G = WG<KC>;
@@ -329,11 +329,28 @@
     };
     body(0, std::true_type{});
     for (int k = 1; k < nchunks; ++k) body(k, std::false_type{});
+    constexpr int XS = 6;
+    f2 xq[XS][2];
+    const float* xb = nullptr;
+    auto ld_x = [&](int r, int slot) {
+        const float* q = xb + (int64_t)((r & 3) + 8 * (r >> 2)) * ((int64_t)p.H * p.W);
+        xq[slot][0] = ld2(q);
+        xq[slot][1] = ld2(q + p.W);
+    };
+    if constexpr (DOT) {
+        const int tile_ = wt * 32 + l31;
+        xb = p.dot_x + ((int64_t)b * p.N + n0 + wn * 32 + 4 * half) * ((int64_t)p.H * p.W) +
+             (int64_t)(oy0 + 2 * (tile_ >> 4)) * p.W + ox0 + 2 * (tile_ & 15);
+#pragma unroll
+        for (int r = 0; r < XS; ++r) ld_x(r, r);
+    }
 #pragma unroll
     for (int m = 0; m < 32; ++m) mfma_step(1, m);
 
     __builtin_amdgcn_s_waitcnt(0x0F70);
     WINO_STAMP(3);
+    float* const dsm = smem;
+    if constexpr (DOT) __syncthreads();
 
     const int tile = wt * 32 + l31;
     const int oy = oy0 + 2 * (tile >> 4), ox = ox0 + 2 * (tile & 15);
@@ -359,7 +376,7 @@
             s[0][j] = (m0 + m1) + m2;
             s[1][j] = (m1 - m2) - m3;
         }
-        if (p.ks > 1) {
+        if (!DOT && p.ks > 1) {
             float* o = p.partial + (((int64_t)slice * p.B + b) * p.N + n) * plane + (int64_t)oy * p.W + ox;
             *reinterpret_cast<float2*>(o) = make_float2((s[0][0] + s[0][1]) + s[0][2], (s[0][1] - s[0][2]) - s[0][3]);
             *reinterpret_cast<float2*>(o + p.W) = make_float2((s[1][0] + s[1][1]) + s[1][2], (s[1][1] - s[1][2]) - s[1][3]);
@@ -387,8 +404,28 @@
             y[a][0] = v0;
             y[a][1] = v1;
         }
+        if constexpr (DOT) {
+            dsm[(wave * 16 + r) * 64 + lane] = (xq[r % XS][0].x * y[0][0] + xq[r % XS][0].y * y[0][1]) +
+                                               (xq[r % XS][1].x * y[1][0] + xq[r % XS][1].y * y[1][1]);
+            if (r + XS < 16) ld_x(r + XS, r % XS);
+            const float ds = p.dot_scale ? p.dot_scale[(int64_t)b * p.N + n] : 1.0f;
+#pragma unroll
+            for (int a = 0; a < 2; ++a) { y[a][0] *= ds; y[a][1] *= ds; }
+        }
         *reinterpret_cast<float2*>(o) = make_float2(y[0][0], y[0][1]);
         *reinterpret_cast<float2*>(o + p.W) = make_float2(y[1][0], y[1][1]);
+    }
+    if constexpr (DOT) {
+        __syncthreads();
+        const int cl = tid >> 2, q = tid & 3;
+        const int c5 = cl & 31, rr = (c5 & 3) + 4 * (c5 >> 3);
+        const float* src = dsm + (((q >> 1) * 2 + (cl >> 5)) * 16 + rr) * 64 + ((c5 >> 2) & 1) * 32 + (q & 1) * 16;
+        float sum = 0.0f;
+#pragma unroll
+        for (int i = 0; i < 16; ++i) sum += src[(i + cl) & 15];
+        sum += __shfl_xor(sum, 1, SR_WAVE);
+        sum += __shfl_xor(sum, 2, SR_WAVE);
+        if (q == 0) p.dot_partial[((int64_t)b * p.N + n0 + cl) * p.dot_tiles + ty_i * p.tiles_x + tx_i] = sum;
     }
     WINO_STAMP(4);
 #ifdef WINO_TIMING
@@ -458,11 +495,11 @@
     }
 }
 
-template <int KC>
+template <int KC, bool DOT>
 int launch(const WinoParams& p, float* u, const float* wt, int ldw, hipStream_t st, bool u_ready) {
     using G = WG<KC>;
     const int lds = (G::STY + p.kchunks * KC) * 4;
-    auto kern = k_conv_wino<KC>;
+    auto kern = k_conv_wino<KC, DOT>;
     static bool configured = false;
     if (!configured) {
         if (hipFuncSetAttribute(reinterpret_cast<const void*>(kern), hipFuncAttributeMaxDynamicSharedMemorySize,
@@ -475,6 +512,9 @@
     if (!u_ready) hipLaunchKernelGGL(k_wino_weights<KC>, dim3(p.N / 64, p.C), dim3(64), 0, st, u, wt, p.C, p.N, ldw);
     const int64_t blocks = (int64_t)p.tiles_n * p.tiles_x * p.tiles_y * p.B * p.ks;
     hipLaunchKernelGGL(kern, dim3((unsigned)blocks), dim3(256), lds, st, p);
+    if (p.ks > 1 && p.dot_x)
+        return sr_dgrad_reduce_dot_launch(p.out, p.partial, p.ks, (int64_t)p.B * p.N, (int64_t)p.H * p.W, p.dot_x,
+                                          p.dot_scale, p.dot_partial, st);
     if (p.ks > 1) {
         const int64_t total4 = (int64_t)p.B * p.N * p.H * p.W / 4;
         int64_t grid = (total4 + 255) / 256;
@@ -516,7 +556,9 @@
 
 int sr_wino_conv3x3(float* out, const float* in, const float* wt, int64_t ldw, const float* iscale,
                     const float* oscale, const float* obias, int64_t B, int64_t C, int64_t N, int64_t H, int64_t W,
-                    float* u_scratch, hipStream_t st, const WinoNba* nba, bool u_ready) {
+                    float* u_scratch, hipStream_t st, const WinoNba* nba, bool u_ready, const WinoDot* dot) {
+    if (dot && (nba || oscale || obias || !dot->x || !dot->partial || (reinterpret_cast<uintptr_t>(dot->x) & 15)))
+        return SR_EINVAL;
     WinoParams p;
     p.in = in; p.u = u_scratch; p.iscale = iscale; p.oscale = oscale; p.obias = obias; p.out = out;
     p.nba = nba ? 1 : 0;
@@ -527,5 +569,13 @@
     p.ks = sr_wino_split(B, C, N, H, W);
     p.kchunks = (int)(C / 8) / p.ks;
     p.partial = u_scratch + sr_wino_scratch_floats(C, N);
-    return launch<8>(p, u_scratch, wt, (int)ldw, st, u_ready);
-}
+    p.dot_x = dot ? dot->x : nullptr; p.dot_scale = dot ? dot->scale : nullptr; p.dot_partial = dot ? dot->partial : nullptr;
+    p.dot_tiles = sr_wino_dot_tiles(B, C, N, H, W);
+    if (dot && p.ks == 1) return launch<8, true>(p, u_scratch, wt, (int)ldw, st, u_ready);
+    return launch<8, false>(p, u_scratch, wt, (int)ldw, st, u_ready);
+}
+
+int sr_wino_dot_tiles(int64_t B, int64_t C, int64_t N, int64_t H, int64_t W) {
+    if (sr_wino_split(B, C, N, H, W) > 1) return sr_dgrad_dot_segments(H * W);
+    return (int)((W / (2 * TW)) * (H / (2 * TH)));
+}
diff --git a/stylerenderer_amd/op/conv.py b/stylerenderer_amd/op/conv.py
--- a/stylerenderer_amd/op/conv.py
+++ b/stylerenderer_amd/op/conv.py
@@ -67,6 +67,42 @@
     return out
 
 
+def conv2d_dgrad_dot(g, wt, gscale, x, xscale, geom):
+    k, stride, pad, tr = _GEOM[geom]
+    if (tr or torch.is_grad_enabled() or g.device.type != "cuda" or g.dtype != torch.float32 or wt.dtype != torch.float32
+            or x.dtype != torch.float32 or not x.is_contiguous() or wt.dim() != 3):
+        return None
+    g = g.contiguous()
+    b, c, ih, iw = g.shape
+    taps, cw, n = wt.shape
+    oh, ow = conv_out_size(ih, iw, k, stride, pad, tr)
+    if taps != k * k or cw != c or tuple(x.shape) != (b, n, oh, ow):
+        return None
+    for t, shape in ((gscale, (b, c)), (xscale, (b, n))):
+        if t is not None and (tuple(t.shape) != shape or not t.is_contiguous() or t.dtype != torch.float32):
+            return None
+    L = _lib.lib()
+    args = (b, c, n, ih, iw, oh, ow, k, stride, pad, 0)
+    out = torch.empty((b, n, oh, ow), dtype=g.dtype, device=g.device)
+    if not L.sr_conv2d_dgrad_dot_supported(*args, _lib.ptr(g), _lib.ptr(out), _lib.ptr(x)):
+        return None
+    wt, ldw = _wt_pitch(wt)
+    nscr = L.sr_conv2d_scratch_floats(*args)
+    scratch, flags, entry = _conv_scratch(wt, nscr, (b, c, n, ih, iw, k, stride, pad, False), g)
+    dscr = torch.empty(L.sr_conv2d_dgrad_dot_scratch_floats(*args), dtype=g.dtype, device=g.device)
+    gis = torch.empty((b, n), dtype=g.dtype, device=g.device)
+    flops = 2.0 * b * oh * ow * c * n * k * k
+    with on_device_of(g):
+        rc = _timed("conv", (k, stride, 0, b, c, n, oh, ow), flops,
+                    lambda: L.sr_conv2d_dgrad_dot(
+                        _lib.ptr(out), _lib.ptr(gis), _lib.ptr(g), _lib.ptr(wt), _lib.ptr(gscale), _lib.ptr(x),
+                        _lib.ptr(xscale), b, c, n, ldw, ih, iw, oh, ow, k, stride, pad, flags, _lib.ptr(scratch),
+                        _lib.ptr(dscr), stream_of(g)))
+    _lib.check(rc, "sr_conv2d_dgrad_dot")
+    _scratch_written(entry, b, c, n, ih, iw, g, out)
+    return gis, out
+
+
 class _Scratch:
     __slots__ = ("buf", "ready")
 
@@ -173,13 +209,20 @@
         geom = ctx.geom
         g = g.contiguous()
         gx = gw = gis = gos = gb = None
-        if need_x or need_is:
+        fused = wadj = None
+        if (need_x or need_is) and geom != "c1s2":
+            wadj = adjoint_weight(wt, geom, ctx.frozen, ctx.adj)
+        if need_is and wadj is not None:
+            fused = conv2d_dgrad_dot(g, wadj, oscale, x, iscale, _ADJOINT[geom])
+        if fused is not None:
+            gis, gx = fused if need_x else (fused[0], None)
+        elif need_x or need_is:
             if geom == "c1s2":
                 inner = ConvFn.apply(g, adjoint_weight(wt, "c1", ctx.frozen, ctx.adj), oscale, None, None, "c1")
                 dxu = torch.zeros_like(x)
                 dxu[:, :, ::2, ::2] = inner
             else:
-                dxu = ConvFn.apply(g, adjoint_weight(wt, geom, ctx.frozen, ctx.adj), oscale, None, None, _ADJOINT[geom])
+                dxu = ConvFn.apply(g, wadj, oscale, None, None, _ADJOINT[geom])
             if need_is and need_x and iscale is not None:
                 gis, gx = rowdot(x, dxu, iscale)
             else:
@@ -316,8 +359,14 @@
         else:
             g, gb, gnw, rdot = _nba_bwd_dot(gy, out, noise, noise_w, abias, slope, gain, want_p)
         gx = gw = gis = gos = None
-        if needs[0] or needs[2]:
-            dxu = ConvFn.apply(g, adjoint_weight(wt, "c3", ctx.frozen, ctx.adj), oscale, None, None, "c3")
+        fused = None
+        wadj = adjoint_weight(wt, "c3", ctx.frozen, ctx.adj) if needs[0] or needs[2] else None
+        if needs[2] and iscale is not None:
+            fused = conv2d_dgrad_dot(g, wadj, oscale, x, iscale, "c3")
+        if fused is not None:
+            gis, gx = fused if needs[0] else (fused[0], None)
+        elif needs[0] or needs[2]:
+            dxu = ConvFn.apply(g, wadj, oscale, None, None, "c3")
             if needs[2] and needs[0] and iscale is not None:
                 gis, gx = rowdot(x, dxu, iscale)
             else:
@@ -435,8 +484,14 @@
             g257 = upfirdn2d_op(g.reshape(-1, oh, ow, 1), flipped(kernel), 1, 1, 1, 1, 3 - p0,
                                 shape257[3] - ow + p0, 3 - p0, shape257[2] - oh + p0).view(shape257)
         gx = gw = gis = gos = None
-        if needs[0] or needs[2]:
-            dxu = ConvFn.apply(g257, adjoint_weight(wt, "t3s2", ctx.frozen, ctx.adj), oscale, None, None, "c3s2")
+        fused = None
+        wadj = adjoint_weight(wt, "t3s2", ctx.frozen, ctx.adj) if needs[0] or needs[2] else None
+        if needs[2] and iscale is not None:
+            fused = conv2d_dgrad_dot(g257, wadj, oscale, x, iscale, "c3s2")
+        if fused is not None:
+            gis, gx = fused if needs[0] else (fused[0], None)
+        elif needs[0] or needs[2]:
+            dxu = ConvFn.apply(g257, wadj, oscale, None, None, "c3s2")
             if needs[2] and needs[0] and iscale is not None:
                 gis, gx = rowdot(x, dxu, iscale)
             else:
```
